# RuanJohn/Mava

Hardware: AMD Instinct MI355X
Metric: env-steps/sec (whole node), ff_mappo RWARE tiny-4ag (higher is better)
Workload: dtype f32 via 2 x f16 split operands on the MFMA (3 products, f32 accumulate); 1 GPU; ff_mappo RWARE tiny-4ag-shaped synthetic obs, 4096 envs/GPU (update_batch_size=1 x num_envs=4096), rollout_length=128, ppo_epochs=4, num_minibatches=2, agents=4, obs=70/264, actions=5, one step = one PPO update = 524288 env-steps per GPU; parallelism=dp1

## Files before the change

### include/mava_hip.h

```cpp
#ifndef MAVA_HIP_H
#define MAVA_HIP_H

#include <stddef.h>
#include <stdint.h>

#ifdef __cplusplus
extern "C" {
#endif

typedef struct ihipStream_t* mava_stream_t;

const char* mava_last_error(void);
int mava_abi_version(void);

typedef struct mava_ctx mava_ctx;
enum {
  MAVA_CTX_MATMUL_MODE = 0,
  MAVA_CTX_CRITIC_AGGREGATION = 1,
  MAVA_CTX_GAE_VARIANT = 2,
  MAVA_CTX_POLICY_VARIANT = 3,
  MAVA_CTX_H2_LAUNCHES = 4,
  MAVA_CTX_TRAIN_VARIANT = 5,
  MAVA_CTX_W8_LAUNCHES = 6,
  MAVA_CTX_W1_SPLIT_FRESH = 7,
// ... 4 lines not shown
  MAVA_CTX_W8_AHEAD_LAUNCHES = 12
};
int mava_ctx_create(mava_ctx** out);
int mava_ctx_destroy(mava_ctx* ctx);
int mava_ctx_set(mava_ctx* ctx, int key, long value);
int mava_ctx_get(const mava_ctx* ctx, int key, long* value);

int mava_gae_f32(const mava_ctx* ctx, const float* reward, const float* value, const uint8_t* done,
                 const float* last_val, const uint8_t* last_done, int T, int N, float gamma,
                 float lambda, float* adv, float* tgt, mava_stream_t s);

int mava_permutation_i32(long n, uint64_t seed, uint64_t counter, int32_t* out, mava_stream_t s);
int mava_permutation_batched_i32(long n, uint64_t seed, uint64_t counter, int n_perm, int32_t* out, long out_stride,
                                 mava_stream_t s);

int mava_clip_adam(float* p, const float* g, float* m, float* v, int32_t* count,
                   const int* seg_off, const float* seg_lr, int n_seg, float grad_scale,
                   float max_norm, int decay, int steps_per_update, int num_updates, float b1,
                   float b2, float eps, const float* loss_sums, float vf_coef, float ent_coef,
                   float* metrics_out, mava_stream_t s);

size_t mava_ppo_finish_workspace_bytes(int Pa, int Pc);
int mava_ppo_finish_f32(mava_ctx* ctx, const float* slab_a, long stride_a, const float* slab_c, long stride_c, int n_slab,
                        int Pa, int Pc, float* g, float* p, float* m, float* v, int32_t* count, float lr_a, float lr_c,
                        float grad_scale, float max_norm, int decay, int steps_per_update, int num_updates, float b1,
                        float b2, float eps, float vf_coef, float ent_coef, float* metrics_out, int critic_din,
                        void* workspace, size_t workspace_bytes, mava_stream_t s);

int mava_slab_reduce_f32(const float* slab, int n_slab, long slab_stride, int n, int accumulate,
                         float* out, mava_stream_t s);

int mava_slab_reduce2_f32(const float* slab, int n_slab, long slab_stride, int n_main,
                          float* out_main, int n_tail, float* out_tail, int accumulate,
                          mava_stream_t s);

int mava_mlp_param_count(int din, int n_out);

int mava_mlp_forward_f32(const mava_ctx* ctx, const float* params, int din, int n_out, const float* x, int x_share,
                         int rows, float* out, mava_stream_t s);

int mava_policy_step_f32(const mava_ctx* ctx, const float* actor_params, int actor_din, int n_actions,
                         const float* agents_view, const uint8_t* action_mask,
                         const float* critic_params, int critic_din, const float* critic_input,
                         int critic_share, int critic_rows, int value_broadcast, int rows,
                         uint64_t seed, uint32_t step, const uint32_t* step_base, uint32_t row_offset, int greedy,
                         const int32_t* forced_action, int32_t* action, float* log_prob,
                         float* value, float* logits, mava_stream_t s);


int mava_adv_stats_blocks(void);

int mava_adv_stats_f64(const float* advantages, const int32_t* idx, long idx_base, int Rb, int A,
                       double* partials, mava_stream_t s);
int mava_adv_stats_batched_f64(const float* advantages, const int32_t* idx, long idx_stride, int Rb, int A,
                               int n_batch, double* partials, mava_stream_t s);

int mava_ppo_actor_grad_f32(mava_ctx* ctx, const float* params, int din, int n_actions, const float* agents_view,
                            const uint8_t* action_mask, const int32_t* action, const float* old_log_prob,
                            const float* advantages, const double* adv_stats, const int32_t* idx, long idx_base, int Rb,
                            int A, float clip_eps, float ent_coef, float* slab, long slab_stride, int n_slab,
                            const uint16_t* input16, const uint32_t* input16_valid, int input16_ld, mava_stream_t s);

int mava_policy_step_continuous_f32(const mava_ctx* ctx, const float* actor_params, int actor_din, int action_dim, float min_scale,
                                    const float* agents_view, const float* critic_params, int critic_din,
                                    const float* critic_input, int critic_share, int critic_rows,
                                    int value_broadcast, int rows, uint64_t seed, uint32_t step,
                                    const uint32_t* step_base, uint32_t row_offset, int greedy,
                                    const float* forced_action, float* action, float* log_prob, float* value,
                                    float* mean, mava_stream_t s);
int mava_ppo_actor_grad_continuous_f32(const float* params, int din, int action_dim, float min_scale, const float* agents_view,
                                       const float* action, const float* old_log_prob, const float* advantages,
                                       const double* adv_stats, const int32_t* idx, long idx_base, int Rb, int A,
                                       float clip_eps, float ent_coef, uint64_t seed, uint32_t ent_step,
                                       uint32_t row_offset, float* slab, long slab_stride, int n_slab,
                                       mava_stream_t s);

int mava_ppo_critic_grad_f32(mava_ctx* ctx, const float* params, int din, const float* critic_input, int x_share,
                             const float* old_value, const float* targets, const int32_t* idx,
                             long idx_base, int Rb, int A, float clip_eps, float vf_coef,
                             float* slab, long slab_stride, int n_slab, const uint16_t* input16,
                             const uint32_t* input16_valid, int input16_ld, mava_stream_t s);


int mava_synth_rware_step(int E, int A, int O, int n_actions, int gs_tiles, int state_dim, int time_limit,
                          uint64_t seed, uint32_t t, const uint32_t* t_base, uint32_t env_offset, int is_reset,
                          int32_t* step_count, float* run_return, int32_t* run_length,
                          float* ep_return, int32_t* ep_length, float* agents_view,
                          float* global_state, uint8_t* action_mask, int32_t* obs_step_count,
                          float* reward, uint8_t* done, float* info_return, int32_t* info_length,
                          uint8_t* info_terminal, const int32_t* action, int reward_mode, mava_stream_t s);

int mava_lbf_step(int E, int A, int F, int G, int fov, int max_agent_level, int force_coop, int individual_rewards,
                  int time_limit, uint64_t seed, uint32_t t, const uint32_t* t_base, uint32_t env_offset, int is_reset,
                  int32_t* agent_pos, int32_t* agent_level, int32_t* food_pos, int32_t* food_level, uint8_t* food_alive,
                  float* total_food_level, int32_t* step_count, float* run_return, int32_t* run_length, float* ep_return,
                  int32_t* ep_length, float* agents_view, float* global_state, uint8_t* action_mask,
                  int32_t* obs_step_count, float* reward, uint8_t* done, float* info_return, int32_t* info_length,
                  uint8_t* info_terminal, const int32_t* action, float* real_view, uint8_t* real_mask, uint8_t* terminated,
                  mava_stream_t s);

int mava_rware_step(int E, int A, int S, int R, int H, int W, int sensor_range, int time_limit, int collision_terminates,
                    const uint32_t* highway_rows, const int32_t* shelf_home, uint64_t seed, uint32_t t,
                    const uint32_t* t_base, uint32_t env_offset, int is_reset, int32_t* agent_pos, int32_t* agent_dir,
                    int32_t* agent_carry, int32_t* shelf_pos, int32_t* request_queue, int32_t* step_count,
                    float* run_return, int32_t* run_length, float* ep_return, int32_t* ep_length, float* agents_view,
                    float* global_state, uint8_t* action_mask, int32_t* obs_step_count, float* reward, uint8_t* done,
                    float* info_return, int32_t* info_length, uint8_t* info_terminal, const int32_t* action,
                    float* real_view, uint8_t* real_mask, uint8_t* terminated, mava_stream_t s);

int mava_connector_step(int E, int A, int G, int time_limit, uint64_t seed, uint32_t t, const uint32_t* t_base,
                        uint32_t env_offset, int is_reset, int32_t* head, int32_t* target, uint8_t* connected,
                        uint8_t* grid, int32_t* step_count, float* run_return, int32_t* run_length, float* ep_return,
                        int32_t* ep_length, float* agents_view, float* global_state, uint8_t* action_mask,
                        int32_t* obs_step_count, float* reward, uint8_t* done, float* info_return, int32_t* info_length,
                        uint8_t* info_terminal, const int32_t* action, float* real_view, uint8_t* real_mask,
                        uint8_t* terminated, mava_stream_t s);

int mava_cleaner_step(int E, int A, int R, int C, int time_limit, uint64_t seed, uint32_t t, const uint32_t* t_base,
                      uint32_t env_offset, int is_reset, int32_t* pos, uint8_t* grid, int32_t* step_count,
                      float* run_return, int32_t* run_length, float* ep_return, int32_t* ep_length, float* agents_view,
                      float* global_state, uint8_t* action_mask, int32_t* obs_step_count, float* reward, uint8_t* done,
                      float* info_return, int32_t* info_length, uint8_t* info_terminal, uint8_t* info_won,
                      const int32_t* action, float* real_view, uint8_t* real_mask, uint8_t* terminated, mava_stream_t s);

int mava_smax_step(int E, int A, int Ne, uint64_t ally_types, uint64_t enemy_types, int time_limit, int see_enemy_actions,
                   int walls_cause_death, uint64_t seed, uint32_t t, const uint32_t* t_base, uint32_t env_offset,
                   int is_reset, float* pos, float* health, int32_t* cd, int32_t* last_action, int32_t* step_count,
                   float* run_return, int32_t* run_length, float* ep_return, int32_t* ep_length, float* agents_view,
                   float* global_state, uint8_t* action_mask, int32_t* obs_step_count, float* reward, uint8_t* done,
                   float* info_return, int32_t* info_length, uint8_t* info_terminal, uint8_t* info_won,
                   const int32_t* action, float* real_view, uint8_t* real_mask, uint8_t* terminated, mava_stream_t s);

int mava_spread_step(int E, int A, int add_agent_id, int time_limit, uint64_t seed, uint32_t t, const uint32_t* t_base,
                     uint32_t env_offset, int is_reset, float* agent_pos, float* landmark_pos, int32_t* step_count,
                     float* run_return, int32_t* run_length, float* ep_return, int32_t* ep_length, float* agents_view,
                     float* global_state, uint8_t* action_mask, int32_t* obs_step_count, float* reward, uint8_t* done,
                     float* info_return, int32_t* info_length, uint8_t* info_terminal, const float* action,
                     float* real_view, uint8_t* real_mask, uint8_t* terminated, float* real_state, mava_stream_t s);

int mava_rollout_ff_f32(const float* actor_params, int n_actions, const float* critic_params, int critic_shared,
                        int E, int A, int O, int T, int time_limit, uint64_t policy_seed, uint64_t env_seed,
                        uint32_t t0, uint32_t row_offset, uint32_t env_offset, int reward_mode,
                        int32_t* step_count, float* run_return, int32_t* run_length, float* ep_return,
                        int32_t* ep_length, float* agents_view, float* global_state, uint8_t* action_mask,
                        int32_t* obs_step_count, int32_t* action, float* value, float* reward, float* log_prob,
                        uint8_t* done, float* last_val, float* info_return, int32_t* info_length,
                        uint8_t* info_terminal, float* adv, float* tgt, float gamma, float gae_lambda,
                        float* last_reward, uint8_t* last_done, int32_t* step_counter, uint16_t* state16,
                        uint32_t* state16_valid, uint16_t* view16, uint32_t* view16_valid, mava_stream_t s);
int mava_rollout_carry(int T, int E, int A, int obs_dim, long gs_dim, int n_actions, float* agents_view,
                       float* global_state, uint8_t* action_mask, int32_t* step_count, mava_stream_t s);


int mava_rec_dense_f32(const mava_ctx* ctx, const float* x, int x_rowmajor, const int32_t* idx, int Rm, int E, int A,
                       int x_share, int x_ld, int accumulate, const float* w, int ldw, const float* bias,
                       const float* gate, float* y, int y_ld, int K, int N, int rows, int relu, mava_stream_t s);

int mava_rec_xty_f32(const mava_ctx* ctx, const float* x, int x_rowmajor, const int32_t* idx, int Rm, int E, int A,
                     int x_share, int x_ld, const float* y, int y_ld, const float* y_tail, int y_split, int y_tail_ld, int K, int N,
                     int rows, int want_bias, float out_scale, float* slab, long slab_stride, int n_slab, mava_stream_t s);
int mava_rec_gather_t32_f32(const float* x, const int32_t* idx, int Rm, int E, int A, int x_share, int x_ld, int K,
                            int rows, int k_pad, float* out, mava_stream_t s);

int mava_gru_scan_fwd_f32(const mava_ctx* ctx, int T, int Rm, int E, int A, const int32_t* idx, const uint8_t* done,
                          const float* h0, int h0_t32, const float* wh, const float* bhn,
                          const float* gi, float* hs, float* hprev, float* saved, mava_stream_t s);

int mava_gru_scan_bwd_f32(const mava_ctx* ctx, int T, int Rm, int E, int A, const int32_t* idx, const uint8_t* done,
                          const float* wh, const float* saved, const float* hprev, const float* dh_out,
                          float* dgi, float* dgh, int dgh_n_only, mava_stream_t s);

int mava_seq_actor_loss_f32(int T, int Rm, int E, int A, int n_actions, const int32_t* idx,
                            const float* logits, const uint8_t* mask, const int32_t* action,
                            const float* old_log_prob, const float* advantages, const double* adv_stats,
                            int n_stats, float clip_eps, float ent_coef, float grad_scale, float* dlogits,
                            float* loss_partials, int n_blocks, mava_stream_t s);
int mava_seq_actor_loss_continuous_f32(int T, int Rm, int E, int A, int action_dim, float min_scale, const int32_t* idx,
                                       const float* mean, const float* log_std, const float* log_std_rows,
                                       const float* action, const float* old_log_prob, const float* advantages,
                                       const double* adv_stats, int n_stats, float clip_eps, float ent_coef, uint64_t seed,
                                       uint32_t ent_step, uint32_t row_offset, float grad_scale, float* dmean,
                                       float* dlog_std_rows, float* loss_partials, float* dscale_partials, int n_blocks,
                                       mava_stream_t s);
int mava_seq_sample_continuous_f32(int rows, int action_dim, float min_scale, const float* mean, const float* log_std,
                                   const float* log_std_rows, uint64_t seed,
                                   uint32_t step, uint32_t row_offset, int greedy, float* action, float* log_prob,
                                   mava_stream_t s);
int mava_seq_critic_loss_f32(int T, int Rm, int E, int A, int agents_per_row, const int32_t* idx, const float* values,
                             const float* old_value, const float* targets, float clip_eps, float vf_coef,
                             float grad_scale, float* dvalues, float* loss_partials, int n_blocks, mava_stream_t s);

int mava_rec_out_f32(int T, int Rm, int E, int A, int n_out, int agents_per_row, const int32_t* idx, const float* hs,
                     const float* params_post_head, const uint8_t* mask, const int32_t* action, const float* f0,
                     const float* f1, const double* adv_stats, int n_stats, float clip_eps, float coef, float grad_scale,
                     int is_actor, float* dh, float* slab, long slab_stride, int n_slab, mava_stream_t s);

int mava_seq_sample_f32(int rows, int n_actions, const float* logits, const uint8_t* mask, uint64_t seed,
                        uint32_t step, uint32_t row_offset, int greedy, int32_t* action, float* log_prob,
                        mava_stream_t s);

int mava_rec_step_f32(const float* actor_params, int actor_din, int n_actions, const float* agents_view,
                      const uint8_t* action_mask, const uint8_t* done_a, const float* h_actor_in,
                      float* h_actor_out, int rows_a, uint64_t seed, uint32_t step, uint32_t row_offset,
                      int greedy, int32_t* action, float* log_prob, const float* critic_params, int critic_din,
                      const float* critic_input, int critic_share, const uint8_t* done_c, int done_c_stride,
                      const float* h_critic_in, float* h_critic_out, int rows_c, int value_broadcast,
                      float* value, mava_stream_t s);
int mava_rec_step_continuous_f32(const float* actor_params, int actor_din, int action_dim, float min_scale, const float* agents_view,
                                 const uint8_t* done_a, const float* h_actor_in, float* h_actor_out, int rows_a,
                                 uint64_t seed, uint32_t step, uint32_t row_offset, int greedy, float* action,
                                 float* log_prob, const float* critic_params, int critic_din,
                                 const float* critic_input, int critic_share, const uint8_t* done_c, int done_c_stride,
                                 const float* h_critic_in, float* h_critic_out, int rows_c, int value_broadcast,
                                 float* value, mava_stream_t s);

long mava_rec_step_pack_bytes(int din);
int mava_rec_step_pack_f32(const float* params, int din, void* pack, mava_stream_t s);
int mava_rec_step_packed_f32(const void* pack_a, const void* pack_c, const float* actor_params, int actor_din,
                             int n_actions, float min_scale, const float* agents_view, const uint8_t* action_mask, const uint8_t* done_a,
                             const float* h_actor_in, float* h_actor_out, int rows_a, uint64_t seed, uint32_t step,
                             uint32_t row_offset, int greedy, int32_t* action, float* action_f, float* log_prob,
                             const float* critic_params, int critic_din, const float* critic_input, int critic_share,
                             const uint8_t* done_c, int done_c_stride, const float* h_critic_in, float* h_critic_out,
                             int rows_c, int value_broadcast, float* value, mava_stream_t s);

int mava_rec_q_step_f32(const float* params, int din, int n_actions, const float* agents_view, const uint8_t* action_mask,
                        const uint8_t* done, const float* h_in, float* h_out, int rows, float eps, uint64_t seed, uint32_t step,
                        uint32_t row_offset, int32_t* action, float* q_out, mava_stream_t s);
int mava_replay_add_f32(int E, int A, int O, int n_actions, int capacity, int slot, const float* obs, const uint8_t* action_mask,
                        const int32_t* action, const float* reward, const uint8_t* terminal, const uint8_t* term_or_trunc,
                        const float* next_obs, const uint8_t* next_mask, float* b_obs, uint8_t* b_mask, int32_t* b_action,
                        float* b_reward, uint8_t* b_terminal, uint8_t* b_term_or_trunc, float* b_next_obs,
// ... 126 lines not shown
```

### mava_amd/_lib.py

```python
from __future__ import annotations

import ctypes as C
import os
from typing import Optional

import torch

_HERE = os.path.dirname(os.path.abspath(__file__))
LIB_PATH = os.environ.get("MAVA_LIB_PATH") or os.path.join(_HERE, "libmavahip.so")

_lib: Optional[C.CDLL] = None


class MavaHipError(RuntimeError):
    pass


vp = C.c_void_p
i32 = C.c_int
u32 = C.c_uint32
u64 = C.c_uint64
f32 = C.c_float
lng = C.c_long

_SIGNATURES = {
    "mava_abi_version": [],
    "mava_ctx_create": [vp],
    "mava_ctx_destroy": [vp],
    "mava_ctx_set": [vp, i32, lng],
    "mava_ctx_get": [vp, i32, vp],
    "mava_gae_f32": [vp, vp, vp, vp, vp, vp, i32, i32, f32, f32, vp, vp, vp],
    "mava_permutation_i32": [lng, u64, u64, vp, vp],
    "mava_permutation_batched_i32": [lng, u64, u64, i32, vp, lng, vp],
    "mava_clip_adam": [vp, vp, vp, vp, vp, C.POINTER(i32), C.POINTER(f32), i32, f32, f32, i32, i32, i32,
                       f32, f32, f32, vp, f32, f32, vp, vp],
    "mava_slab_reduce_f32": [vp, i32, lng, i32, i32, vp, vp],
    "mava_ppo_finish_workspace_bytes": [i32, i32],
    "mava_ppo_finish_f32": [vp, vp, lng, vp, lng, i32, i32, i32, vp, vp, vp, vp, vp, f32, f32, f32, f32, i32, i32, i32, f32, f32, f32,
                            f32, f32, vp, i32, vp, C.c_size_t, vp],
    "mava_slab_reduce2_f32": [vp, i32, lng, i32, vp, i32, vp, i32, vp],
    "mava_mlp_param_count": [i32, i32],
    "mava_mlp_forward_f32": [vp, vp, i32, i32, vp, i32, i32, vp, vp],
    "mava_policy_step_f32": [vp, vp, i32, i32, vp, vp, vp, i32, vp, i32, i32, i32, i32, u64, u32, vp, u32, i32,
                             vp, vp, vp, vp, vp, vp],
    "mava_policy_step_continuous_f32": [vp, vp, i32, i32, f32, vp, vp, i32, vp, i32, i32, i32, i32, u64, u32, vp, u32, i32, vp, vp, vp, vp, vp, vp],
    "mava_ppo_actor_grad_continuous_f32": [vp, i32, i32, f32, vp, vp, vp, vp, vp, vp, lng, i32, i32, f32, f32, u64, u32, u32, vp, lng, i32, vp],
    "mava_seq_actor_loss_continuous_f32": [i32, i32, i32, i32, i32, f32, vp, vp, vp, vp, vp, vp, vp, vp, i32, f32, f32, u64, u32, u32, f32, vp, vp, vp, vp, i32, vp],
    "mava_seq_sample_continuous_f32": [i32, i32, f32, vp, vp, vp, u64, u32, u32, i32, vp, vp, vp],
    "mava_adv_stats_blocks": [],
    "mava_adv_stats_f64": [vp, vp, lng, i32, i32, vp, vp],
    "mava_adv_stats_batched_f64": [vp, vp, lng, i32, i32, i32, vp, vp],
    "mava_ppo_actor_grad_f32": [vp, vp, i32, i32, vp, vp, vp, vp, vp, vp, vp, lng, i32, i32, f32, f32, vp, lng, i32,
                                vp, vp, i32, vp],
    "mava_ppo_critic_grad_f32": [vp, vp, i32, vp, i32, vp, vp, vp, lng, i32, i32, f32, f32, vp, lng, i32, vp, vp, i32, vp],
    "mava_synth_rware_step": [i32, i32, i32, i32, i32, i32, i32, u64, u32, vp, u32, i32] + [vp] * 14 + [vp, i32, vp],
    "mava_lbf_step": [i32] * 9 + [u64, u32, vp, u32, i32] + [vp] * 24 + [vp],
    "mava_rware_step": [i32] * 9 + [vp, vp, u64, u32, vp, u32, i32] + [vp] * 23 + [vp],
    "mava_connector_step": [i32] * 4 + [u64, u32, vp, u32, i32] + [vp] * 22 + [vp],
    "mava_cleaner_step": [i32] * 5 + [u64, u32, vp, u32, i32] + [vp] * 21 + [vp],
    "mava_smax_step": [i32] * 3 + [u64, u64] + [i32] * 3 + [u64, u32, vp, u32, i32] + [vp] * 23 + [vp],
    "mava_spread_step": [i32] * 4 + [u64, u32, vp, u32, i32] + [vp] * 21 + [vp],
    "mava_rec_q_step_f32": [vp, i32, i32, vp, vp, vp, vp, vp, i32, f32, u64, u32, u32, vp, vp, vp],
    "mava_replay_add_f32": [i32] * 6 + [vp] * 16 + [vp],
    "mava_replay_sample_f32": [i32] * 5 + [u32, i32, i32, i32, u64, u32] + [vp] * 17 + [vp],
    "mava_q_td_loss_f32": [i32, i32, i32, i32] + [vp] * 7 + [f32, f32, vp, vp, i32, vp],
    "mava_target_update_f32": [lng, vp, vp, f32, i32, vp],
    "mava_qmix_state_t32_f32": [i32] * 6 + [vp] * 4 + [vp],
    "mava_qmix_td_f32": [i32] * 7 + [vp] * 15 + [f32, f32] + [vp] * 6 + [i32, vp],
    "mava_sac_replay_add_f32": [i32] * 7 + [vp] * 14 + [vp],
    "mava_sac_replay_sample_f32": [i32] * 5 + [u32, i32, i32, u64, u32] + [vp] * 15 + [vp],
    "mava_sac_sample_f32": [i32, i32, i32, f32, vp, vp, u64, u32, u32, vp, vp, vp, vp],
    "mava_sac_concat_f32": [i32] * 7 + [vp] * 4 + [i32, vp],
    "mava_sac_q_loss_f32": [i32] * 3 + [vp] * 8 + [f32, f32] + [vp] * 4 + [i32, vp],
    "mava_sac_actor_grad_f32": [i32] * 4 + [f32] + [vp] * 9 + [i32, i32, i32, f32, f32] + [vp] * 3 + [i32, vp],
    "mava_sac_alpha_loss_f32": [i32, i32, vp, vp, f32, vp, vp, vp],
    "mava_rollout_ff_f32": [vp, i32, vp, i32, i32, i32, i32, i32, i32, u64, u64, u32, u32, u32, i32] + [vp] * 18
                           + [vp, vp, f32, f32] + [vp] * 7 + [vp],
    "mava_rollout_carry": [i32, i32, i32, i32, lng, i32, vp, vp, vp, vp, vp],
    "mava_rec_dense_f32": [vp, vp, i32, vp, i32, i32, i32, i32, i32, i32, vp, i32, vp, vp, vp, i32, i32, i32, i32, i32, vp],
    "mava_rec_xty_f32": [vp, vp, i32, vp, i32, i32, i32, i32, i32, vp, i32, vp, i32, i32, i32, i32, i32, i32, f32, vp, lng, i32, vp],
    "mava_rec_gather_t32_f32": [vp, vp, i32, i32, i32, i32, i32, i32, i32, i32, vp, vp],
    "mava_gru_scan_fwd_f32": [vp, i32, i32, i32, i32, vp, vp, vp, i32, vp, vp, vp, vp, vp, vp, vp],
    "mava_t32_gru_mask_f32": [vp, vp, vp, i32, i32, i32, lng, vp, vp],
    "mava_t32_gru_gates_f32": [vp, vp, vp, vp, i32, lng, vp, vp, vp, vp, vp, i32, i32, vp],
    "mava_t32_gru_gates_bwd_f32": [vp, vp, vp, vp, vp, vp, vp, i32, i32, i32, lng, vp, vp, vp, vp],
    "mava_gru_scan_bwd_f32": [vp, i32, i32, i32, i32, vp, vp, vp, vp, vp, vp, vp, vp, i32, vp],
    "mava_seq_actor_loss_f32": [i32, i32, i32, i32, i32, vp, vp, vp, vp, vp, vp, vp, i32, f32, f32, f32, vp, vp, i32, vp],
    "mava_rec_step_continuous_f32": [vp, i32, i32, f32, vp, vp, vp, vp, i32, u64, u32, u32, i32, vp, vp, vp, i32, vp, i32, vp, i32, vp, vp, i32, i32, vp, vp],
    "mava_rec_step_f32": [vp, i32, i32, vp, vp, vp, vp, vp, i32, u64, u32, u32, i32, vp, vp, vp, i32, vp, i32, vp, i32, vp, vp,
                          i32, i32, vp, vp],
    "mava_seq_critic_loss_f32": [i32, i32, i32, i32, i32, vp, vp, vp, vp, f32, f32, f32, vp, vp, i32, vp],
    "mava_rec_out_f32": [i32, i32, i32, i32, i32, i32, vp, vp, vp, vp, vp, vp, vp, vp, i32, f32, f32, f32, i32, vp, vp, lng, i32, vp],
    "mava_rec_step_pack_bytes": [i32],
    "mava_t32_norm_act_f32": [vp, i32, lng, i32, vp, i32, vp, vp, vp, vp],
    "mava_t32_norm_act_bwd_f32": [vp, vp, i32, lng, i32, vp, vp, i32, vp, vp, vp],
    "mava_t32_colsum_f32": [vp, i32, lng, f32, vp, lng, i32, vp],
    "mava_t32_im2col_f32": [vp, i32, lng, i32, i32, i32, i32, i32, vp, vp],
    "mava_t32_col2im_f32": [vp, i32, lng, i32, i32, i32, i32, i32, vp, vp],
    "mava_t32_flatten_f32": [vp, lng, i32, i32, i32, vp, vp],
    "mava_comm_unique_id": [vp],
    "mava_comm_create": [vp, i32, i32, vp],
    "mava_allreduce_sum_f32": [vp, vp, C.c_size_t, vp],
    "mava_broadcast_f32": [vp, vp, C.c_size_t, i32, vp],
    "mava_comm_destroy": [vp],
    "mava_rec_step_pack_f32": [vp, i32, vp, vp],
    "mava_rec_step_packed_f32": [vp, vp, vp, i32, i32, f32, vp, vp, vp, vp, vp, i32, u64, u32, u32, i32, vp, vp, vp, vp, i32, vp, i32, vp, i32, vp, vp, i32, i32, vp, vp],
    "mava_seq_sample_f32": [i32, i32, vp, vp, u64, u32, u32, i32, vp, vp, vp],
    "mava_t32_convert_f32": [vp, i32, i32, i32, vp, vp],
    "mava_mat_attn_fwd_f32": [vp, vp, vp, lng, i32, i32, i32, i32, i32, vp, vp, i32, vp],
    "mava_mat_attn_bwd_f32": [vp, vp, vp, vp, lng, i32, i32, i32, i32, i32, vp, vp, vp, i32, vp],
    "mava_mat_ln_fwd_f32": [vp, vp, vp, vp, i32, lng, lng, vp, vp, vp, i32, vp],
    "mava_mat_ln_bwd_f32": [vp, vp, vp, vp, i32, lng, lng, f32, vp, vp, lng, i32, vp],
    "mava_mat_gelu_f32": [vp, lng, vp, vp],
    "mava_mat_gelu_bwd_f32": [vp, vp, lng, vp, vp],
    "mava_mat_shift_onehot_f32": [vp, vp, i32, i32, i32, i32, lng, i32, vp, vp],
    "mava_mat_sample_f32": [i32, i32, i32, i32, vp, vp, u64, u32, u32, i32, vp, vp, vp],
    "mava_mat_loss_f32": [i32, i32, i32, lng, vp, vp, vp, vp, vp, vp, vp, vp, vp, vp, i32, f32, f32, f32, f32, vp, vp, vp, i32, vp],
    "mava_transformer_param_count": [i32, i32, i32, i32],
    "mava_transformer_act_workspace_bytes": [i32, i32, i32, i32, i32],
    "mava_transformer_act_f32": [vp, vp, vp, i32, i32, i32, i32, i32, i32, i32, u64, u32, u32, i32, vp, vp, vp, vp, C.c_size_t, i32, vp],
    "mava_transformer_shift_action_f32": [vp, vp, i32, i32, i32, i32, lng, i32, vp, vp],
    "mava_transformer_sample_continuous_f32": [i32, i32, i32, i32, f32, vp, vp, u64, u32, u32, i32, vp, vp, vp],
    "mava_transformer_loss_continuous_f32": [i32, i32, i32, f32, lng, vp, vp, vp, vp, vp, vp, vp, vp, vp, vp, i32, f32, f32, f32, u64, u32,
                                             u32, f32, vp, vp, vp, vp, i32, vp],
    "mava_transformer_param_count_continuous": [i32, i32, i32, i32],
    "mava_transformer_act_continuous_f32": [vp, vp, i32, i32, i32, i32, i32, i32, i32, f32, u64, u32, u32, i32, vp, vp, vp, vp, C.c_size_t,
                                            i32, vp],
}
_RESTYPES = {"mava_last_error": C.c_char_p, "mava_rec_step_pack_bytes": C.c_long, "mava_ppo_finish_workspace_bytes": C.c_size_t,
             "mava_transformer_param_count": C.c_long, "mava_transformer_act_workspace_bytes": C.c_size_t,
             "mava_transformer_param_count_continuous": C.c_long}


def declared_symbols():
    return sorted(set(_SIGNATURES) | set(_RESTYPES))


def lib() -> C.CDLL:
    global _lib
    if _lib is None:
        if not os.path.exists(LIB_PATH):
            raise MavaHipError(
                f"{LIB_PATH} is missing: build it with `python -m mava_amd.build` "
                "(hipcc --offload-arch=gfx950). There is no CPU fallback."
            )
        _lib = C.CDLL(LIB_PATH)
        _lib.mava_last_error.restype = C.c_char_p
        _lib.mava_last_error.argtypes = []
        for name, args in _SIGNATURES.items():
            fn = getattr(_lib, name)
            fn.argtypes = args
            fn.restype = _RESTYPES.get(name, C.c_int)
    return _lib


class Ctx:

    MATMUL_MODE, CRITIC_AGGREGATION, GAE_VARIANT, POLICY_VARIANT, H2_LAUNCHES, TRAIN_VARIANT, W8_LAUNCHES, W1_SPLIT_FRESH = 0, 1, 2, 3, 4, 5, 6, 7
    EXACT_TILES = 8
    X16_LAUNCHES = 9
# ... 77 lines not shown
```

### mava_amd/csrc/ppo_train.hip

```cpp
#include "mlp_core.h"
#include "ppo_train_task.h"
#include "ctx.h"
#include "tanh_normal.h"

namespace {

constexpr int STATS_BLOCKS = 128;
constexpr int LDT = 33;


#ifdef MAVA_STAMPS
#define STAMP_DECL unsigned long long st_prev = __builtin_readcyclecounter(), st_acc[16] = {0, 0, 0, 0, 0, 0, 0, 0, 0, 0, 0, 0, 0, 0, 0, 0};
#define STAMP(i)                                                   \
  do {                                                             \
    const unsigned long long st_now = __builtin_readcyclecounter(); \
    st_acc[i] += st_now - st_prev;                                 \
    st_prev = st_now;                                              \
  } while (0)
#else
#define STAMP_DECL
#define STAMP(i)
#endif

struct TrainLdsLayout {
// ... 748 lines not shown
      l += __shfl_down(l, o, 64);
    }
    if (lane == 0) { red[2 * w] = v; red[2 * w + 1] = l; }
    __syncthreads();
    if (tid == 0) {
      slab[oB3] = ((red[0] + red[2]) + red[4]) + red[6];
      slab[P] = ((red[1] + red[3]) + red[5]) + red[7];
      slab[P + 1] = 0.0f;
    }
  }
}

int pick_xv(const float* x, int din) {
  const uintptr_t a = (uintptr_t)x;
  return (din % 4 == 0 && a % 16 == 0 && din >= 96) ? 4 : 1;
}

template <int NO, int KT1, bool ACTOR, int XV, bool CONT>
int launch_train(const TrainTask& tk, int n_slab, hipStream_t s) {
  const TrainLdsLayout L = make_layout<NO>(KT1);
  const size_t lb = (size_t)L.end * sizeof(float);
  MAVA_ARG_CHECK(lb <= 163840, 8,
                 "ppo_train: %zu bytes of LDS needed (n_out pad %d, input width %d) exceed the 160 KiB of a CU",
                 lb, NO, tk.din);
  static bool attr_set = false;
  if (!attr_set) {
    MAVA_HIP_CHECK(hipFuncSetAttribute((const void*)ppo_train_kernel<NO, KT1, ACTOR, XV, CONT>,
                                       hipFuncAttributeMaxDynamicSharedMemorySize, (int)lb));
    attr_set = true;
  }
  g_train_last_instance = train_instance_id(1, ACTOR, CONT, false, NO, KT1, XV);
  hipLaunchKernelGGL((ppo_train_kernel<NO, KT1, ACTOR, XV, CONT>), dim3(n_slab), dim3(256), lb, s, tk, L);
  MAVA_LAUNCH_CHECK();
  return MAVA_OK;
}

template <int NO, int KT1, bool ACTOR, bool CONT>
int launch_xv(const TrainTask& tk, int n_slab, hipStream_t s) {
  if (KT1 >= 4 && tk.xv == 4) return launch_train<NO, KT1, ACTOR, (KT1 >= 4 ? 4 : 1), CONT>(tk, n_slab, s);
  return launch_train<NO, KT1, ACTOR, 1, CONT>(tk, n_slab, s);
}

template <int NO, bool ACTOR, bool CONT = false>
int dispatch_kt(const TrainTask& tk, int n_slab, hipStream_t s) {
  const int kt = tk.din / 32 + 1;
#ifdef MAVA_FAST_BUILD
  if (kt == 3) return launch_xv<NO, 3, ACTOR, CONT>(tk, n_slab, s);
  if (kt == 9) return launch_xv<NO, 9, ACTOR, CONT>(tk, n_slab, s);
  mava_set_error("fast build: input width %d not instantiated", tk.din);
  return MAVA_EARG(9);
#else
  switch (kt) {
    case 1: return launch_xv<NO, 1, ACTOR, CONT>(tk, n_slab, s);
    case 2: return launch_xv<NO, 2, ACTOR, CONT>(tk, n_slab, s);
    case 3: return launch_xv<NO, 3, ACTOR, CONT>(tk, n_slab, s);
    case 4: return launch_xv<NO, 4, ACTOR, CONT>(tk, n_slab, s);
    case 5: case 6: return launch_xv<NO, 6, ACTOR, CONT>(tk, n_slab, s);
    case 7: case 8: case 9: return launch_xv<NO, 9, ACTOR, CONT>(tk, n_slab, s);
    default:
      mava_set_error("ppo_train: input width %d > 287 is not instantiated", tk.din);
      return MAVA_EARG(9);
  }
#endif
}

}

#ifdef MAVA_STAMPS
static unsigned long long* g_stamps = nullptr;
extern "C" int mava_debug_set_stamps(unsigned long long* p) {
  g_stamps = p;
  return MAVA_OK;
}
#else
static constexpr unsigned long long* g_stamps = nullptr;
#endif


extern "C" int mava_adv_stats_blocks(void) { return STATS_BLOCKS; }

int g_train_last_instance = 0;
extern "C" int mava_debug_train_last_instance(void) { return g_train_last_instance; }

extern "C" int mava_adv_stats_f64(const float* adv, const int32_t* idx, long idx_base, int Rb, int A,
                                  double* partials, hipStream_t s) {
  MAVA_ARG_CHECK(Rb >= 1 && A >= 1, 0, "mava_adv_stats_f64: Rb=%d A=%d", Rb, A);
  MAVA_ARG_CHECK(adv && partials, 1, "mava_adv_stats_f64: null pointer argument");
  hipLaunchKernelGGL(adv_stats_kernel, dim3(STATS_BLOCKS), dim3(256), 0, s, adv, idx, idx_base, Rb, A,
                     partials, 0L);
  MAVA_LAUNCH_CHECK();
  return MAVA_OK;
}

extern "C" int mava_adv_stats_batched_f64(const float* adv, const int32_t* idx, long idx_stride, int Rb, int A,
                                          int n_batch, double* partials, hipStream_t s) {
  MAVA_ARG_CHECK(Rb >= 1 && A >= 1 && n_batch >= 1 && n_batch <= 65535 && idx_stride >= 0, 0,
                 "mava_adv_stats_batched_f64: Rb=%d A=%d n_batch=%d idx_stride=%ld", Rb, A, n_batch, idx_stride);
  MAVA_ARG_CHECK(adv && idx && partials, 1, "mava_adv_stats_batched_f64: null pointer argument");
  hipLaunchKernelGGL(adv_stats_kernel, dim3(STATS_BLOCKS, n_batch), dim3(256), 0, s, adv, idx, 0L, Rb, A, partials,
                     idx_stride);
  MAVA_LAUNCH_CHECK();
  return MAVA_OK;
}

extern "C" int mava_ppo_actor_grad_f32(mava_ctx* ctx, const float* params, int din, int n_actions, const float* agents_view,
                                       const uint8_t* action_mask, const int32_t* action, const float* old_log_prob,
                                       const float* advantages, const double* adv_stats, const int32_t* idx, long idx_base,
                                       int Rb, int A, float clip_eps, float ent_coef, float* slab, long slab_stride,
                                       int n_slab, const uint16_t* input16, const uint32_t* input16_valid, int input16_ld,
                                       hipStream_t s) {
  MAVA_ARG_CHECK(din >= 1 && n_actions >= 1 && n_actions <= 32, 0,
                 "mava_ppo_actor_grad_f32: din=%d n_actions=%d unsupported", din, n_actions);
  MAVA_ARG_CHECK(Rb >= 1 && A >= 1 && n_slab >= 1 && n_slab <= 1024 && (long)Rb * A < (1L << 31), 1,
                 "mava_ppo_actor_grad_f32: Rb=%d A=%d n_slab=%d", Rb, A, n_slab);
  MAVA_ARG_CHECK(slab_stride >= mlp_param_count(din, n_actions) + 2, 2,
                 "mava_ppo_actor_grad_f32: slab_stride too small");
  MAVA_ARG_CHECK(params && agents_view && action && old_log_prob && advantages && adv_stats && slab, 3,
                 "mava_ppo_actor_grad_f32: null pointer argument");
  MAVA_ARG_CHECK((input16 == nullptr) == (input16_valid == nullptr) && input16_ld >= 0, 3,
                 "mava_ppo_actor_grad_f32: input16 and input16_valid go together, input16_ld=%d", input16_ld);
  TrainTask tk = {};
  tk.params = params; tk.x = agents_view; tk.din = din; tk.no = n_actions; tk.xshare = 1; tk.agg = 1;
  tk.xv = pick_xv(agents_view, din); tk.A = A; tk.idx = idx; tk.idx_base = idx_base; tk.Rb = Rb;
  tk.mask = action_mask; tk.action = action; tk.old_logp = old_log_prob; tk.adv = advantages;
  tk.stats = adv_stats; tk.clip_eps = clip_eps; tk.ent_coef = ent_coef; tk.slab = slab;
  tk.slab_stride = slab_stride;
  tk.stamps = g_stamps;
  tk.x16 = reinterpret_cast<const _Float16*>(input16); tk.x16_valid = input16_valid; tk.x16_ld = input16_ld;
  if (mava_ctx_matmul_mode(ctx) == 1) {
    const int rc = mava_train_h2_launch(ctx, tk, n_slab, true, s);
    if (rc <= 0) return rc;
  }
  if (n_actions <= 8) return dispatch_kt<8, true>(tk, n_slab, s);
  if (n_actions <= 16) return dispatch_kt<16, true>(tk, n_slab, s);
  return dispatch_kt<32, true>(tk, n_slab, s);
}

extern "C" int mava_ppo_actor_grad_continuous_f32(const float* params, int din, int action_dim, float min_scale,
                                                  const float* agents_view, const float* action,
                                                  const float* old_log_prob, const float* advantages,
                                                  const double* adv_stats, const int32_t* idx, long idx_base, int Rb,
                                                  int A, float clip_eps, float ent_coef, uint64_t seed,
                                                  uint32_t ent_step, uint32_t row_offset, float* slab,
                                                  long slab_stride, int n_slab, hipStream_t s) {
  MAVA_ARG_CHECK(din >= 1 && action_dim >= 1 && action_dim <= 16, 0,
                 "mava_ppo_actor_grad_continuous_f32: din=%d action_dim=%d unsupported (action_dim <= 16)", din,
                 action_dim);
  MAVA_ARG_CHECK(Rb >= 1 && A >= 1 && n_slab >= 1 && n_slab <= 1024 && (long)Rb * A < (1L << 31), 1,
                 "mava_ppo_actor_grad_continuous_f32: Rb=%d A=%d n_slab=%d", Rb, A, n_slab);
  MAVA_ARG_CHECK(slab_stride >= mlp_param_count(din, action_dim) + action_dim + 2, 2,
                 "mava_ppo_actor_grad_continuous_f32: slab_stride too small");
  MAVA_ARG_CHECK(params && agents_view && action && old_log_prob && advantages && adv_stats && slab, 3,
                 "mava_ppo_actor_grad_continuous_f32: null pointer argument");
  TrainTask tk = {};
  tk.params = params; tk.x = agents_view; tk.din = din; tk.no = action_dim; tk.xshare = 1; tk.agg = 1;
  tk.xv = pick_xv(agents_view, din); tk.A = A; tk.idx = idx; tk.idx_base = idx_base; tk.Rb = Rb;
  tk.action_f = action; tk.old_logp = old_log_prob; tk.adv = advantages;
  tk.stats = adv_stats; tk.clip_eps = clip_eps; tk.ent_coef = ent_coef; tk.slab = slab;
  tk.slab_stride = slab_stride;
  tk.seed_lo = (uint32_t)seed; tk.seed_hi = (uint32_t)(seed >> 32); tk.ent_step = ent_step; tk.row_offset = row_offset;
  tk.min_scale = min_scale;
  tk.stamps = g_stamps;
  if (action_dim <= 8) return dispatch_kt<8, true, true>(tk, n_slab, s);
  return dispatch_kt<16, true, true>(tk, n_slab, s);
}

extern "C" int mava_ppo_critic_grad_f32(mava_ctx* ctx, const float* params, int din, const float* critic_input, int x_share,
                                        const float* old_value, const float* targets, const int32_t* idx, long idx_base,
                                        int Rb, int A, float clip_eps, float vf_coef, float* slab, long slab_stride,
                                        int n_slab, const uint16_t* input16, const uint32_t* input16_valid, int input16_ld,
                                        hipStream_t s) {
  MAVA_ARG_CHECK(din >= 1 && x_share >= 1, 0, "mava_ppo_critic_grad_f32: din=%d x_share=%d", din, x_share);
  MAVA_ARG_CHECK(Rb >= 1 && A >= 1 && n_slab >= 1 && n_slab <= 1024 && (long)Rb * A < (1L << 31), 1,
                 "mava_ppo_critic_grad_f32: Rb=%d A=%d n_slab=%d", Rb, A, n_slab);
  MAVA_ARG_CHECK(slab_stride >= mlp_param_count(din, 1) + 2, 2,
                 "mava_ppo_critic_grad_f32: slab_stride too small");
  MAVA_ARG_CHECK(params && critic_input && old_value && targets && slab, 3,
                 "mava_ppo_critic_grad_f32: null pointer argument");
  MAVA_ARG_CHECK((input16 == nullptr) == (input16_valid == nullptr) && input16_ld >= 0, 3,
                 "mava_ppo_critic_grad_f32: input16 and input16_valid go together, input16_ld=%d", input16_ld);
  TrainTask tk = {};
  tk.params = params; tk.x = critic_input; tk.din = din; tk.no = 1; tk.xshare = x_share; tk.agg = 1;
  if (mava_ctx_critic_aggregation(ctx) && A > 1 && A <= 8 && x_share == A) {
    tk.agg = A;
    tk.xshare = 1;
  }
  tk.xv = pick_xv(critic_input, din); tk.A = A; tk.idx = idx; tk.idx_base = idx_base; tk.Rb = Rb;
  tk.old_value = old_value; tk.targets = targets; tk.clip_eps = clip_eps; tk.vf_coef = vf_coef;
  tk.slab = slab; tk.slab_stride = slab_stride;
  tk.stamps = g_stamps;
  tk.x16 = reinterpret_cast<const _Float16*>(input16); tk.x16_valid = input16_valid; tk.x16_ld = input16_ld;
  int rc = 1;
  if (mava_ctx_matmul_mode(ctx) == 1) rc = mava_train_h2_launch(ctx, tk, n_slab, false, s);
  if (ctx != nullptr) ctx->w1_fresh[1] = 0;
  if (rc <= 0) return rc;
  return dispatch_kt<1, false>(tk, n_slab, s);
}
```

### mava_amd/csrc/ppo_train_h2.hip

```cpp
#include "h2_core.h"
#include "ppo_train_task.h"
#include "ctx.h"

#include <type_traits>

#ifndef MAVA_GW_DEPTH
#define MAVA_GW_DEPTH 0
#endif
#define GW_DEPTH MAVA_GW_DEPTH
#ifndef MAVA_GW_DEPTH_WIDE
#define MAVA_GW_DEPTH_WIDE 0
#endif
#ifndef MAVA_P1_EARLY_HALVES
#define MAVA_P1_EARLY_HALVES 2
#endif
#ifndef MAVA_P1_EARLY_RING
#define MAVA_P1_EARLY_RING 3
#endif

namespace {

using namespace h2;

constexpr int STATS_BLOCKS = 128;
// ... 1004 lines not shown
#pragma unroll
    for (int q = 0; q < 16; ++q) {
      const int o = (q & 3) + 8 * (q >> 2) + 4 * h;
      if (o < no) slab[oW3 + (32 * w + r) * no + o] = gW3[q] * invR;
    }
    float v = ab3;
#pragma unroll
    for (int m = NO; m < 64; m <<= 1) v += __shfl_xor(v, m, 64);
    if (lane < NO) red[w * NO + lane] = v;
    for (int o = 32; o > 0; o >>= 1) {
      loss_a += __shfl_down(loss_a, o, 64);
      loss_b += __shfl_down(loss_b, o, 64);
    }
    if (lane == 0) { red[4 * NO + 2 * w] = loss_a; red[4 * NO + 2 * w + 1] = loss_b; }
    __syncthreads();
    if (tid < no) slab[oB3 + tid] = (((red[tid] + red[NO + tid]) + red[2 * NO + tid]) + red[3 * NO + tid]) * invR;
    if (tid == 0) {
      slab[Pn] = ((red[4 * NO] + red[4 * NO + 2]) + red[4 * NO + 4]) + red[4 * NO + 6];
      slab[Pn + 1] = ((red[4 * NO + 1] + red[4 * NO + 3]) + red[4 * NO + 5]) + red[4 * NO + 7];
    }
  } else {
#pragma unroll
    for (int q = 0; q < 16; ++q) {
      float v = aW3r[q];
#pragma unroll
      for (int m = 1; m < 32; m <<= 1) v += __shfl_xor(v, m, 64);
      if (r == 0) slab[oW3 + 32 * w + (q & 3) + 8 * (q >> 2) + 4 * h] = v * invR;
    }
    float v = ab3, l = loss_a;
    for (int o = 32; o > 0; o >>= 1) {
      v += __shfl_down(v, o, 64);
      l += __shfl_down(l, o, 64);
    }
    if (lane == 0) { red[2 * w] = v; red[2 * w + 1] = l; }
    __syncthreads();
    if (tid == 0) {
      slab[oB3] = (((red[0] + red[2]) + red[4]) + red[6]) * invR;
      slab[Pn] = ((red[1] + red[3]) + red[5]) + red[7];
      slab[Pn + 1] = 0.0f;
    }
  }
}

template <int NO, int S1, bool ACTOR, bool WIDE, int XV>
__global__ __launch_bounds__(WIDE ? 512 : 256, WIDE ? 2 : 1) void ppo_train_h2_kernel(TrainTask tk, H2Layout L,
                                                                                     const uint4* __restrict__ w1p) {
  extern __shared__ __attribute__((aligned(16))) u8 lds[];
  if constexpr (WIDE) {
    constexpr bool X16_CAPABLE = !ACTOR && XV == 4;
    bool x16 = false;
    if constexpr (X16_CAPABLE) {
      if (tk.x16_valid != nullptr) x16 = __builtin_amdgcn_readfirstlane((int)*tk.x16_valid) == 1;
    }
    if (X16_CAPABLE && x16) {
      if constexpr (X16_CAPABLE) {
        if (threadIdx.x < 256) {
          h2_body<NO, S1, ACTOR, WIDE, XV, 1, true>(tk, L, w1p, lds);
        } else {
          h2_body<NO, S1, ACTOR, WIDE, XV, 2, true>(tk, L, w1p, lds);
        }
      }
    } else if (threadIdx.x < 256) {
      h2_body<NO, S1, ACTOR, WIDE, XV, 1>(tk, L, w1p, lds);
    } else {
      h2_body<NO, S1, ACTOR, WIDE, XV, 2>(tk, L, w1p, lds);
    }
  } else {
    h2_body<NO, S1, ACTOR, WIDE, XV, 0>(tk, L, w1p, lds);
  }
}

int ctx_counters(mava_ctx* ctx, hipStream_t s) {
  if (ctx->exact_tiles == nullptr) {
    void* word = nullptr;
    MAVA_HIP_CHECK(hipMalloc(&word, 5 * sizeof(unsigned long long)));
    ctx->exact_tiles = static_cast<unsigned long long*>(word);
    MAVA_HIP_CHECK(hipMemsetAsync(word, 0, 5 * sizeof(unsigned long long), s));
  }
  return MAVA_OK;
}

template <int NO, int S1, bool ACTOR, bool WIDE, int XV>
int launch_h2(mava_ctx* ctx, const TrainTask& tk, int n_slab, hipStream_t s) {
  const H2Layout L = make_h2_layout<NO, S1, WIDE>(ACTOR);
  MAVA_ARG_CHECK(L.end <= 163840, 8, "ppo_train_h2: %d bytes of LDS exceed the 160 KiB of a CU", L.end);
  static bool attr_set = false;
  if (!attr_set) {
    MAVA_HIP_CHECK(hipFuncSetAttribute((const void*)ppo_train_h2_kernel<NO, S1, ACTOR, WIDE, XV>,
                                       hipFuncAttributeMaxDynamicSharedMemorySize, L.end));
    attr_set = true;
  }
  const uint4* w1p = nullptr;
  if (WIDE) {
    void*& slot = ctx->w1_split[ACTOR ? 0 : 1];
    if (slot == nullptr) MAVA_HIP_CHECK(hipMalloc(&slot, W1_SPLIT_BYTES));
    uint4* const buf = static_cast<uint4*>(slot);
    const int kind = ACTOR ? 0 : 1;
    int& fresh = ctx->w1_fresh[kind];
    const bool keyed = ctx->w1_key_params[kind] == tk.params && ctx->w1_key_din[kind] == tk.din && ctx->w1_key_steps[kind] == S1;
    if (!(fresh && keyed)) {
      hipLaunchKernelGGL((pack_w1_kernel<S1>), dim3(1), dim3(256), 0, s, tk.params, tk.din, buf, ACTOR ? 1.0f : W_SCALE_CRITIC);
      MAVA_LAUNCH_CHECK();
    }
    fresh = 0;
    w1p = buf;
    const int rc = ctx_counters(ctx, s);
    if (rc != MAVA_OK) return rc;
  }
  TrainTask tkl = tk;
  tkl.exact_tiles = WIDE ? ctx->exact_tiles : nullptr;
  const bool x16_ok = WIDE && !ACTOR && XV == 4 && tk.x16 != nullptr && tk.x16_valid != nullptr && tk.din % 8 == 0 &&
                      (uintptr_t)tk.x16 % 16 == 0 && tk.force_xlo == 0 && (tk.x16_ld == 0 || tk.x16_ld == tk.din);
  if (!x16_ok) { tkl.x16 = nullptr; tkl.x16_valid = nullptr; }
  tkl.x16_launches = x16_ok ? ctx->exact_tiles + 1 : nullptr;
  g_train_last_instance = train_instance_id(2, ACTOR, false, WIDE, NO, S1, XV);
  hipLaunchKernelGGL((ppo_train_h2_kernel<NO, S1, ACTOR, WIDE, XV>), dim3(n_slab), dim3(WIDE ? 512 : 256), L.end, s, tkl, L,
                     w1p);
  MAVA_LAUNCH_CHECK();
  return MAVA_OK;
}

template <int NO, int S1, bool ACTOR, bool WIDE>
int dispatch_xv(mava_ctx* ctx, const TrainTask& tk, int n_slab, hipStream_t s) {
  const uintptr_t a = (uintptr_t)tk.x;
  if constexpr (WIDE) {
    if (tk.din % 4 == 0 && a % 16 == 0) return launch_h2<NO, S1, ACTOR, WIDE, 4>(ctx, tk, n_slab, s);
  } else {
    if (tk.din % 2 == 0 && a % 8 == 0) return launch_h2<NO, S1, ACTOR, WIDE, 2>(ctx, tk, n_slab, s);
  }
  return launch_h2<NO, S1, ACTOR, WIDE, 1>(ctx, tk, n_slab, s);
}

template <int NO, bool ACTOR>
int dispatch_s1(mava_ctx* ctx, const TrainTask& tk, int n_slab, hipStream_t s) {
  const int s1 = (tk.din + 1 + 15) / 16;
  switch (s1) {
#ifndef MAVA_FAST_BUILD
    case 1: return dispatch_xv<NO, 1, ACTOR, false>(ctx, tk, n_slab, s);
    case 2: return dispatch_xv<NO, 2, ACTOR, false>(ctx, tk, n_slab, s);
    case 3: return dispatch_xv<NO, 3, ACTOR, false>(ctx, tk, n_slab, s);
    case 4: return dispatch_xv<NO, 4, ACTOR, false>(ctx, tk, n_slab, s);
    case 6: return dispatch_xv<NO, 6, ACTOR, false>(ctx, tk, n_slab, s);
    case 7: case 8: case 9: case 10: case 11: case 12: return dispatch_xv<NO, 12, ACTOR, true>(ctx, tk, n_slab, s);
#endif
    case 5: return dispatch_xv<NO, 5, ACTOR, false>(ctx, tk, n_slab, s);
    case 13: case 14: case 15: case 16: case 17: case 18: return dispatch_xv<NO, 18, ACTOR, true>(ctx, tk, n_slab, s);
    default: return 1;
  }
}

}

static int h2_dispatch(mava_ctx* ctx, const TrainTask& tk, int n_slab, bool actor, hipStream_t s) {
  if (actor) {
    if (tk.action_f != nullptr) return 1;
    if (tk.no <= 8) return dispatch_s1<8, true>(ctx, tk, n_slab, s);
#ifndef MAVA_FAST_BUILD
    if (tk.no <= 16) return dispatch_s1<16, true>(ctx, tk, n_slab, s);
    return dispatch_s1<32, true>(ctx, tk, n_slab, s);
#else
    return 1;
#endif
  }
  return dispatch_s1<1, false>(ctx, tk, n_slab, s);
}

int mava_train_h2_launch(mava_ctx* ctx, const TrainTask& tk_in, int n_slab, bool actor, hipStream_t s) {
  TrainTask tk = tk_in;
  tk.force_xlo = (ctx->train_variant & 2) != 0;
  tk.no_defer = (ctx->train_variant & 4) != 0;
  tk.no_ahead = (ctx->train_variant & 8) != 0;
  if ((ctx->train_variant & 1) == 0) {
    if (tk.x16 != nullptr && tk.x16_valid != nullptr) {
      const int rcc = ctx_counters(ctx, s);
      if (rcc != MAVA_OK) return rcc;
      tk.x16_launches = ctx->exact_tiles + 2;
      tk.defer_launches = ctx->exact_tiles + 3;
      tk.ahead_launches = ctx->exact_tiles + 4;
    }
    const int rc8 = mava_train_w8_launch(tk, n_slab, actor, s);
    if (rc8 <= 0) {
      if (rc8 == 0) { ++ctx->h2_launches; ++ctx->w8_launches; }
      return rc8;
    }
  }
  const int rc = h2_dispatch(ctx, tk, n_slab, actor, s);
  if (rc == 0) ++ctx->h2_launches;
  return rc;
}
```

### mava_amd/csrc/ppo_train_task.h

```cpp
#pragma once
#include <stdint.h>

#include "common.h"

struct TrainTask {
  const float* params;
  const float* x;
  int din, no, xshare, xv;
  int A;
  int agg;
  const int32_t* idx;
  long idx_base;
  int Rb;
  const uint8_t* mask;
  const int32_t* action;
  const float* action_f;
  uint32_t seed_lo, seed_hi, ent_step, row_offset;
  float min_scale;
  const float* old_logp;
  const float* adv;
  const double* stats;
  const float* old_value;
  const float* targets;
  float clip_eps, ent_coef, vf_coef;
  float* slab;
  long slab_stride;
  unsigned long long* stamps;
  int force_xlo;
  unsigned long long* exact_tiles;
  const _Float16* x16;
  const uint32_t* x16_valid;
  unsigned long long* x16_launches;
  int x16_ld;
  int no_defer;
  unsigned long long* defer_launches;
  int no_ahead;
  unsigned long long* ahead_launches;
};

struct mava_ctx;
int mava_train_w8_launch(const TrainTask& tk, int n_slab, bool actor, hipStream_t s);
int mava_train_h2_launch(mava_ctx* ctx, const TrainTask& tk, int n_slab, bool actor, hipStream_t s);

extern int g_train_last_instance;
constexpr int train_instance_id(int family, bool actor, bool cont, bool wide, int no, int k, int xv) {
  return family * 1000000 + ((actor ? 1 : 0) + (cont ? 2 : 0) + (wide ? 4 : 0)) * 100000 + no * 1000 + k * 10 + xv;
}
```

### mava_amd/csrc/ppo_train_w8.hip

```cpp
#include "h2_core.h"
#include "ppo_train_task.h"
#include "ctx.h"

namespace {

using namespace h2;
typedef float f32x4 __attribute__((ext_vector_type(4)));

constexpr int STATS_BLOCKS = 128;
#ifndef MAVA_W8_GWD
#define MAVA_W8_GWD 1
#endif
constexpr int GWD = MAVA_W8_GWD;
#ifndef MAVA_W8_DEFER
#define MAVA_W8_DEFER 1
#endif
constexpr int W8_DEFER = MAVA_W8_DEFER;
static_assert(W8_DEFER >= 0 && W8_DEFER <= 2, "MAVA_W8_DEFER is 0, 1 or 2");
#ifndef MAVA_W8_AHEAD_ROLES
#define MAVA_W8_AHEAD_ROLES 1
#endif
#ifndef MAVA_W8_AHEAD_POS
#define MAVA_W8_AHEAD_POS 0
#endif
// ... 744 lines not shown
    float x = ab3;
#pragma unroll
    for (int m = NO; m < 64; m <<= 1) x += __shfl_xor(x, m, 64);
    if (l < NO) red[v * NO + l] = x;
    for (int o = 32; o > 0; o >>= 1) {
      loss_a += __shfl_down(loss_a, o, 64);
      loss_b += __shfl_down(loss_b, o, 64);
    }
    if (l == 0) { red[8 * NO + 2 * v] = loss_a; red[8 * NO + 2 * v + 1] = loss_b; }
  }
  __syncthreads();
  constexpr int LW = LOSS_THREADS / 64;
  if (tid < no) {
    float x = 0.0f;
#pragma unroll
    for (int u = 0; u < LW; ++u) x += red[u * NO + tid];
    slab[oB3 + tid] = x * invR;
  }
  if (tid == 0) {
    float a = 0.0f, b = 0.0f;
#pragma unroll
    for (int u = 0; u < LW; ++u) { a += red[8 * NO + 2 * u]; b += red[8 * NO + 2 * u + 1]; }
    slab[Pn] = a;
    slab[Pn + 1] = b;
  }
}

constexpr int w8_w2r(int no, int s1, int xv) {
#ifdef MAVA_W8_W2R
  return MAVA_W8_W2R;
#else
  return (no == 8) ? ((s1 <= 2) ? 2 : ((s1 == 3 && xv == 2) ? 2 : 0)) : ((s1 <= 2) ? 2 : 0);
#endif
}
template <int NO, int S1, int XV, int W2R, bool ACTOR>
__global__ __launch_bounds__(512, 2) void ppo_train_w8_kernel(TrainTask tk, W8Layout L) {
  extern __shared__ __attribute__((aligned(16))) u8 lds[];
  constexpr bool X16_CAPABLE = XV == 2;
  if constexpr (NO == 8) {
    constexpr bool DEFER_CAPABLE = X16_CAPABLE && W8_DEFER != 0;
    bool defer = false;
    if constexpr (DEFER_CAPABLE) {
      if (tk.x16_valid != nullptr && tk.no_defer == 0) defer = __builtin_amdgcn_readfirstlane((int)*tk.x16_valid) == 1;
    }
    constexpr bool AHEAD_CAPABLE = DEFER_CAPABLE && ACTOR && W8_AHEAD_ROLES != 0;
    if (DEFER_CAPABLE && defer && AHEAD_CAPABLE && tk.no_ahead == 0) {
      if constexpr (AHEAD_CAPABLE) {
        if (threadIdx.x < 256) w8_body<NO, S1, XV, W2R, ACTOR, 1, false, W8_DEFER, (W8_AHEAD_ROLES & 2) != 0>(tk, L, lds);
        else w8_body<NO, S1, XV, W2R, ACTOR, 2, true, 2, (W8_AHEAD_ROLES & 1) != 0>(tk, L, lds);
      }
    } else if (DEFER_CAPABLE && defer) {
      if constexpr (DEFER_CAPABLE) {
        if (threadIdx.x < 256) w8_body<NO, S1, XV, W2R, ACTOR, 1, false, W8_DEFER>(tk, L, lds);
        else w8_body<NO, S1, XV, W2R, ACTOR, 2, true, 2>(tk, L, lds);
      }
    } else if (threadIdx.x < 256) {
      w8_body<NO, S1, XV, W2R, ACTOR, 1>(tk, L, lds);
    } else {
      bool x16 = false;
      if constexpr (X16_CAPABLE) {
        if (tk.x16_valid != nullptr) x16 = __builtin_amdgcn_readfirstlane((int)*tk.x16_valid) == 1;
      }
      if (X16_CAPABLE && x16) {
        if constexpr (X16_CAPABLE) w8_body<NO, S1, XV, W2R, ACTOR, 2, true>(tk, L, lds);
      } else {
        w8_body<NO, S1, XV, W2R, ACTOR, 2>(tk, L, lds);
      }
    }
  } else {
    bool x16 = false;
    if constexpr (X16_CAPABLE) {
      if (tk.x16_valid != nullptr) x16 = __builtin_amdgcn_readfirstlane((int)*tk.x16_valid) == 1;
    }
    if (X16_CAPABLE && x16) {
      if constexpr (X16_CAPABLE) w8_body<NO, S1, XV, W2R, ACTOR, 0, true>(tk, L, lds);
    } else {
      w8_body<NO, S1, XV, W2R, ACTOR, 0>(tk, L, lds);
    }
  }
}

template <int NO, int S1, int XV, bool ACTOR>
int launch_w8(const TrainTask& tk, int n_slab, hipStream_t s) {
  const W8Layout L = make_w8_layout();
  MAVA_ARG_CHECK(L.end <= 163840, 8, "ppo_train_w8: %d bytes of LDS exceed the 160 KiB of a CU", L.end);
  static bool attr_set = false;
  if (!attr_set) {
    MAVA_HIP_CHECK(hipFuncSetAttribute((const void*)ppo_train_w8_kernel<NO, S1, XV, w8_w2r(NO, S1, XV), ACTOR>, hipFuncAttributeMaxDynamicSharedMemorySize,
                                       L.end));
    attr_set = true;
  }
  TrainTask tkl = tk;
  const int ld16 = tk.x16_ld != 0 ? tk.x16_ld : tk.din;
  const bool x16_ok = XV == 2 && tk.x16 != nullptr && tk.x16_valid != nullptr && ld16 % 8 == 0 && ld16 >= tk.din &&
                      (uintptr_t)tk.x16 % 16 == 0 && tk.force_xlo == 0 && tk.xshare == 1 && tk.agg <= 1;
  tkl.x16_ld = ld16;
  if (!x16_ok) { tkl.x16 = nullptr; tkl.x16_valid = nullptr; tkl.x16_launches = nullptr; tkl.defer_launches = nullptr; tkl.ahead_launches = nullptr; }
  g_train_last_instance = train_instance_id(3, ACTOR, false, false, NO, S1, XV);
  hipLaunchKernelGGL((ppo_train_w8_kernel<NO, S1, XV, w8_w2r(NO, S1, XV), ACTOR>), dim3(n_slab), dim3(512), L.end, s, tkl, L);
  MAVA_LAUNCH_CHECK();
  return MAVA_OK;
}

template <int NO, int S1, bool ACTOR>
int dispatch_w8_xv(const TrainTask& tk, int n_slab, hipStream_t s) {
  if (tk.din % 2 == 0 && ((uintptr_t)tk.x) % 8 == 0) return launch_w8<NO, S1, 2, ACTOR>(tk, n_slab, s);
  if constexpr (S1 == 4) return 1;
  else return launch_w8<NO, S1, 1, ACTOR>(tk, n_slab, s);
}

template <int NO, bool ACTOR>
int dispatch_w8(const TrainTask& tk, int n_slab, hipStream_t s) {
  const int s1 = (tk.din + 1 + 31) / 32;
  switch (s1) {
#ifndef MAVA_FAST_BUILD
    case 1: return dispatch_w8_xv<NO, 1, ACTOR>(tk, n_slab, s);
    case 2: return dispatch_w8_xv<NO, 2, ACTOR>(tk, n_slab, s);
    case 4: return dispatch_w8_xv<NO, 4, ACTOR>(tk, n_slab, s);
#endif
    case 3: return dispatch_w8_xv<NO, 3, ACTOR>(tk, n_slab, s);
    default: return 1;
  }
}

}

int mava_train_w8_launch(const TrainTask& tk, int n_slab, bool actor, hipStream_t s) {
  if (tk.action_f != nullptr || tk.din + 1 > 128) return 1;
  if (!actor) {
    if (tk.agg > 1 || tk.no != 1) return 1;
    return dispatch_w8<8, false>(tk, n_slab, s);
  }
  if (tk.no <= 8) return dispatch_w8<8, true>(tk, n_slab, s);
#ifndef MAVA_FAST_BUILD
  if (tk.no <= 16) return dispatch_w8<16, true>(tk, n_slab, s);
#endif
  return 1;
}
```

### mava_amd/csrc/rollout_h2.hip

```cpp
#include "h2_core.h"

#ifdef MAVA_STAMPS
#define RSTAMP_DECL unsigned long long rs_prev = __builtin_readcyclecounter(), rs_acc[8] = {0, 0, 0, 0, 0, 0, 0, 0};
#define RSTAMP(i)                                                   \
  do {                                                              \
    __builtin_amdgcn_sched_barrier(0);                              \
    const unsigned long long rs_now = __builtin_readcyclecounter(); \
    rs_acc[i] += rs_now - rs_prev;                                  \
    rs_prev = rs_now;                                               \
    __builtin_amdgcn_sched_barrier(0);                              \
  } while (0)
static __device__ unsigned long long g_rollout_stamps[16];
#else
#define RSTAMP_DECL
#define RSTAMP(i)
#endif

namespace {
using namespace h2;
typedef _Float16 half2v __attribute__((ext_vector_type(2)));

constexpr uint32_t ENV_STREAM = 0x454E5653u;
constexpr uint32_t POLICY_STREAM = 0x504f4c49u;

struct RolloutArgs {
  const float* pa;
  const float* pc;
  int E, A, O, no, T, time_limit;
  uint32_t pseed_lo, pseed_hi, eseed_lo, eseed_hi;
  uint32_t t0;
  uint32_t row_offset;
  uint32_t env_offset;
  int reward_mode;
  int32_t* step_count;
  float* run_return; int32_t* run_length; float* ep_return; int32_t* ep_length;
  float* agents_view;
  float* global_state;
  uint8_t* action_mask;
  int32_t* obs_step_count;
  int32_t* action; float* value; float* reward; float* log_prob; uint8_t* done;
  float* last_val;
  float* info_return; int32_t* info_length; uint8_t* info_terminal;
  float* adv; float* tgt;
  float gamma, lam;
  float* last_reward; uint8_t* last_done; int32_t* step_counter;
  _Float16* state16; uint32_t* state16_valid;
  _Float16* view16; uint32_t* view16_valid;
  int v16_nc; uint32_t v16_nc_m;
};

#define MAVA_AS4 __attribute__((address_space(4)))
__device__ __forceinline__ const MAVA_AS4 RolloutArgs& args_here() {
  const MAVA_AS4 RolloutArgs* p = (const MAVA_AS4 RolloutArgs*)__builtin_amdgcn_kernarg_segment_ptr();
  asm volatile("" : "+s"(p));
  return *p;
}

__device__ __forceinline__ uint32_t div_small(uint32_t x, uint32_t m) { return __umul24(x, m) >> 16; }

struct RolloutLds {
  int xa, xa_row, xa_plane, xc, xc_row, xc_plane, h1, wl, ypa, ypc, act, mask, small, gum, xlf, end;
};
constexpr int W1_REG_STEPS = 12;

template <int NO, int S1A, int S1C, bool SHARED>
constexpr RolloutLds make_rollout_lds() {
  constexpr int KTA = (S1A + 1) / 2, KTC = (S1C + 1) / 2;
  RolloutLds L{};
  L.xa = 0;
  L.xa_row = 2 * 32 * KTA + 16;
  L.xa_plane = 32 * L.xa_row;
  L.xc = L.xa + 2 * 2 * L.xa_plane;
  L.xc_row = 2 * 32 * KTC + 16;
  L.xc_plane = ((S1C > W1_REG_STEPS) ? 16 : 32) * L.xc_row;
  L.h1 = L.xc + (SHARED ? 2 * L.xc_plane : 0);
  L.wl = L.h1 + (SHARED ? 3 : 4) * IMG_BYTES;
  L.ypa = L.wl + ((S1C > W1_REG_STEPS) ? (S1C - W1_REG_STEPS) * 4 * 64 * 32 : 0);
  L.ypc = L.ypa + 2 * 4 * 32 * (NO + 1) * 4;
  L.act = L.ypc + 2 * 4 * 32 * 4;
  L.mask = L.act + 64 * 4;
  L.small = L.mask + 64 * 32;
  L.gum = L.small + (128 + 32 + 128 + 4 + 128) * 4;
  L.gum = (L.gum + 15) & ~15;
  L.xlf = L.gum + 64 * NO * 4;
  L.end = L.xlf + 16;
  L.end = (L.end + 15) & ~15;
  return L;
}

template <int NO, int S1A, int S1C, bool SHARED, int ROLE>
__device__ __forceinline__ void rollout_body(const RolloutArgs& a, u8* lds) {
  constexpr bool ACT_ROLE = ROLE == 0;
  constexpr RolloutLds L = make_rollout_lds<NO, S1A, S1C, SHARED>();
  const int t512 = threadIdx.x;
  const int tid = t512 & 255, lane = tid & 63, w = tid >> 6, h = lane >> 5, r = lane & 31;
  const int A = a.A, O = a.O, no = a.no, W = A + O, E = a.E;
  const int EB = 64 / A;
  const int e0 = blockIdx.x * EB;
  const int din_a = W, din_c = SHARED ? A * O : W;
  constexpr int NTC = SHARED ? 1 : 2;
  float* const B2a = reinterpret_cast<float*>(lds + L.small);
  float* const B3a = B2a + 128;
  float* const B2c = B3a + 32;
  float* const B3c = B2c + 128;
  float* const W3c = B3c + 4;
  int* const ACT = reinterpret_cast<int*>(lds + L.act);
  u8* const MASK = lds + L.mask;
  float* const GUM = reinterpret_cast<float*>(lds + L.gum);
  unsigned* const XLF = reinterpret_cast<unsigned*>(lds + L.xlf);
  float* const YPA = reinterpret_cast<float*>(lds + L.ypa);
  float* const YPC = reinterpret_cast<float*>(lds + L.ypc);
  constexpr int xa_row = L.xa_row, xa_plane = L.xa_plane, xc_row = L.xc_row, xc_plane = L.xc_plane;

  for (int i = t512 * 16; i < L.end; i += 512 * 16) *reinterpret_cast<uint4*>(lds + i) = make_uint4(0, 0, 0, 0);
  __syncthreads();
  const int oW2a = mlp_off_w2(din_a), oW3a = mlp_off_w3(din_a), oW2c = mlp_off_w2(din_c), oW3c = mlp_off_w3(din_c);
  if (ACT_ROLE) {
    if (tid < 128) B2a[tid] = a.pa[mlp_off_b2(din_a) + tid];
    if (tid < no) B3a[tid] = a.pa[mlp_off_b3(din_a, no) + tid];
  } else {
    if (tid < 128) {
      B2c[tid] = a.pc[mlp_off_b2(din_c) + tid];
      W3c[tid] = a.pc[oW3c + tid];
    }
    if (tid == 0) B3c[0] = a.pc[mlp_off_b3(din_c, 1)];
  }
  constexpr int S1R = ACT_ROLE ? S1A : S1C;
  constexpr int S1REG = (S1R > W1_REG_STEPS) ? W1_REG_STEPS : S1R;
  constexpr int XC_ROWS = (S1C > W1_REG_STEPS) ? 16 : 32;
  uint4* const WL = reinterpret_cast<uint4*>(lds + L.wl) + 2 * (w * 64 + lane);
  const float* const PR = ACT_ROLE ? a.pa : a.pc;
  const int din_r = ACT_ROLE ? din_a : din_c, oW2r = ACT_ROLE ? oW2a : oW2c;
// ... 212 lines not shown
          return read_row_frag(lds + L.h1 + ((ACT_ROLE ? 0 : 2) + t) * IMG_BYTES, IMG_PLANE, rowB + 32 * s);
        };
        Frag bn[NT];
#pragma unroll
        for (int t = 0; t < NT; ++t) bn[t] = h_frag(0, t);
#pragma unroll
        for (int s = 0; s < 8; ++s) {
          Frag b[NT];
#pragma unroll
          for (int t = 0; t < NT; ++t) b[t] = bn[t];
          if (s + 1 < 8) {
#pragma unroll
            for (int t = 0; t < NT; ++t) bn[t] = h_frag(s + 1, t);
          }
#pragma unroll
          for (int t = 0; t < NT; ++t) z[t] = mfma3(W2r[s], b[t], z[t]);
          __builtin_amdgcn_sched_barrier(0);
        }
      }
      if (ACT_ROLE) {
#pragma unroll
        for (int t = 0; t < NT; ++t) {
          half4 ph[4], pl[4];
#pragma unroll
          for (int g = 0; g < 4; ++g)
#pragma unroll
            for (int e = 0; e < 4; ++e) {
              _Float16 x0, x1;
              split1(fmaxf(z[t][4 * g + e], 0.0f), x0, x1);
              ph[g][e] = x0;
              pl[g][e] = x1;
            }
          f32x16 y;
#pragma unroll
          for (int q = 0; q < 16; ++q) y[q] = 0.0f;
#pragma unroll
          for (int s = 0; s < 2; ++s) {
            Frag b;
            b.hi = __builtin_shufflevector(ph[2 * s], ph[2 * s + 1], 0, 1, 2, 3, 4, 5, 6, 7);
            b.lo = __builtin_shufflevector(pl[2 * s], pl[2 * s + 1], 0, 1, 2, 3, 4, 5, 6, 7);
            y = mfma3(W3h[s], b, y);
          }
#pragma unroll
          for (int q = 0; q < 16; ++q) {
            const int o = (q & 3) + 8 * (q >> 2) + 4 * h;
            if ((q & 3) + 8 * (q >> 2) < NO) {
              if (o < NO) YPA[((t * 4 + w) * 32 + r) * (NO + 1) + o] = y[q] * W3_UNSCALE;
            }
          }
        }
      } else {
#pragma unroll
        for (int t = 0; t < NT; ++t) {
          float4 w3g[4];
#pragma unroll
          for (int g = 0; g < 4; ++g) w3g[g] = *reinterpret_cast<const float4*>(W3c + 32 * w + 4 * h + 8 * g);
          float part = 0.0f;
#pragma unroll
          for (int q = 0; q < 16; ++q) {
            const float4 tv = w3g[q >> 2];
            const float w3 = (q & 3) == 0 ? tv.x : (q & 3) == 1 ? tv.y : (q & 3) == 2 ? tv.z : tv.w;
            part = fmaf(fmaxf(z[t][q], 0.0f), w3, part);
          }
          part += __shfl_xor(part, 32, 64);
          if (h == 0) YPC[(t * 4 + w) * 32 + r] = part;
        }
      }
    }
    RSTAMP(2);
    __syncthreads();
    RSTAMP(3);
  };
  auto value_of = [&](int crow) -> float {
    const float* yp = YPC + (crow >> 5) * 4 * 32 + (crow & 31);
    return (((yp[0] + yp[32]) + yp[64]) + yp[96]) + B3c[0];
  };

  const int rows_ok = min(64, (E - e0) * A), envs_ok = min(EB, E - e0);
  const int AO = A * O;
  const uint32_t no_m = 65536u / (uint32_t)no + 1u, nch_m = 65536u / nch + 1u;
  const int tid_w = tid, wo_q = (W >> 1) > 0 ? (W >> 1) : 1, gs_q = (AO >> 2) > 0 ? (AO >> 2) : 1;
  const int wo_dr = 256 / wo_q, gs_dr = 256 / gs_q;
  const uint32_t wo_m = 65536u / (uint32_t)wo_q + 1u, gs_m = 65536u / (uint32_t)gs_q + 1u;
  auto write_gs = [&](long slot, bool f32_too) {
    const auto& a = args_here();
    int tid = tid_w;
    asm volatile("" : "+v"(tid));
    if (SHARED && a.global_state != nullptr) {
      float* dst = a.global_state + (slot * E + e0) * (long)AO;
      if ((AO & 3) == 0) {
        const bool h16 = a.state16 != nullptr;
        uint4* const dst16 = h16 ? reinterpret_cast<uint4*>(a.state16 + (slot * E + e0) * (long)AO) : nullptr;
        const int Q = AO >> 2, d_r = gs_dr, d_f = 256 - d_r * Q;
        int le = (int)div_small((uint32_t)tid, gs_m), k = tid - le * Q;
        for (int j = tid; j < EB * Q; j += 256) {
          if (le < envs_ok) {
            if (f32_too) {
              const half4 v = *reinterpret_cast<const half4*>(lds + L.xc + le * xc_row + 8 * k);
              reinterpret_cast<float4*>(dst)[j] = make_float4((float)v[0], (float)v[1], (float)v[2], (float)v[3]);
            }
            if (h16 && (k & 1) == 0) dst16[j >> 1] = *reinterpret_cast<const uint4*>(lds + L.xc + le * xc_row + 8 * k);
          }
          le += d_r; k += d_f;
          if (k >= Q) { k -= Q; ++le; }
        }
      } else if (f32_too) {
        const int d_r = 256 / AO, d_f = 256 - d_r * AO;
        int le = tid / AO, k = tid - le * AO;
        for (int j = tid; j < EB * AO; j += 256) {
          if (le < envs_ok) dst[j] = (float)*reinterpret_cast<const _Float16*>(lds + L.xc + le * xc_row + 2 * k);
          le += d_r; k += d_f;
          if (k >= AO) { k -= AO; ++le; }
        }
      }
    }
  };
  auto write_view16 = [&](long slot) {
    const auto& a = args_here();
    if (a.view16 != nullptr) {
      int tid = tid_w;
      asm volatile("" : "+v"(tid));
      const int NC = a.v16_nc;
      uint4* const dst16 = reinterpret_cast<uint4*>(a.view16) + (slot * EA + (long)e0 * A) * NC;
      for (int j = tid; j < rows_ok * NC; j += 256) {
        const int row = (int)div_small((uint32_t)j, a.v16_nc_m), c = j - row * NC;
        dst16[j] = *reinterpret_cast<const uint4*>(lds + L.xa + (row >> 5) * 2 * xa_plane + (row & 31) * xa_row + 16 * c);
      }
    }
  };
  auto write_out = [&](long slot, bool part_gs) {
    const auto& a = args_here();
    int tid = tid_w;
    asm volatile("" : "+v"(tid));
    if (!part_gs) {
      float* dst = a.agents_view + (slot * EA + (long)e0 * A) * W;
      if ((W & 1) == 0) {
        const int W2 = W >> 1, d_r = wo_dr, d_f = 256 - d_r * W2;
        int row = (int)div_small((uint32_t)tid, wo_m), f = tid - row * W2;
        for (int j = tid; j < 64 * W2; j += 256) {
          if (row < rows_ok) {
            const u8* xa = lds + L.xa + (row >> 5) * 2 * xa_plane + (row & 31) * xa_row;
            const half2v v = *reinterpret_cast<const half2v*>(xa + 4 * f);
            reinterpret_cast<float2*>(dst)[j] = make_float2((float)v[0], (float)v[1]);
          }
          row += d_r; f += d_f;
          if (f >= W2) { f -= W2; ++row; }
        }
      } else {
        const int d_r = 256 / W, d_f = 256 - d_r * W;
        int row = tid / W, f = tid - row * W;
        for (int j = tid; j < 64 * W; j += 256) {
          if (row < rows_ok) {
            const u8* xa = lds + L.xa + (row >> 5) * 2 * xa_plane + (row & 31) * xa_row;
            dst[j] = (float)*reinterpret_cast<const _Float16*>(xa + 2 * f);
          }
          row += d_r; f += d_f;
          if (f >= W) { f -= W; ++row; }
        }
      }
    }
    if (!part_gs) write_view16(slot);
    if (part_gs) write_gs(slot, true);
    if (!part_gs) {
      uint8_t* dst = a.action_mask + (slot * EA + (long)e0 * A) * no;
      for (int j = tid; j < rows_ok * no; j += 256) {
        const int row = (int)div_small((uint32_t)j, no_m), o = j - row * no;
        dst[j] = MASK[row * 32 + o];
      }
    }
  };

  const int T_steps = a.T;
  const uint32_t t0 = a.t0;
  if (SHARED && ACT_ROLE && a.state16 != nullptr) write_gs(0L, false);
  if (!ACT_ROLE) write_view16(0L);
  for (int t = 0; t < T_steps; ++t) {
    const uint32_t step = t0 + (uint32_t)t;
    forward(true, true, step);
    x_lo = 0;
    asm volatile("" : "+s"(x_lo));
    const auto& a = args_here();
    if (ACT_ROLE) {
      constexpr int RPP = 256 / NO;
#pragma unroll
      for (int pass = 0; pass < 64 / RPP; ++pass) {
        const int row = pass * RPP + tid / NO, o = tid & (NO - 1);
        const float* yp = YPA + (((row >> 5) * 4) * 32 + (row & 31)) * (NO + 1) + o;
        const float y = (((yp[0] + yp[32 * (NO + 1)]) + yp[2 * 32 * (NO + 1)]) + yp[3 * 32 * (NO + 1)]) + B3a[o];
        const bool legal = (o < no) && (MASK[row * 32 + o] != 0);
        const float z = legal ? y : -FLT_MAX;
        auto fmax_op = [](float p, float q) { return fmaxf(p, q); };
        auto add_op = [](float p, float q) { return p + q; };
        const float mx = group_allreduce<NO>(z, fmax_op);
        const float se = group_allreduce<NO>(expf(z - mx), add_op);
        const float logp = (mx == -FLT_MAX) ? ((o < no) ? -logf((float)no) : -FLT_MAX) : z - (mx + logf(se));
        float sc = (o < no) ? (z + GUM[row * NO + o]) : -FLT_MAX;
        if (!(sc > -FLT_MAX)) sc = -FLT_MAX;
        int best = o;
#pragma unroll
        for (int m = 1; m < NO; m <<= 1) {
          const float so = __shfl_xor(sc, m, 64);
          const int bo = __shfl_xor(best, m, 64);
          const bool take = (so > sc) || (so == sc && bo < best);
          sc = take ? so : sc;
          best = take ? bo : best;
        }
        const float lp = group_allreduce<NO>((o == best) ? logp : 0.0f, add_op);
        const int e = e0 + (row >> lgA);
        if (o == 0) {
          ACT[row] = best;
          if (e < E) {
            const long k = (long)t * EA + (long)e0 * A + row;
            a.action[k] = best;
            a.log_prob[k] = lp;
          }
        }
      }
    } else {
      if (tid < 64 && (e0 + (tid >> lgA)) < E) {
        a.value[(long)t * EA + (long)e0 * A + tid] = value_of(SHARED ? (tid >> lgA) : tid);
      }
      if (t > 0) write_out((long)t, false);
    }
    if (ACT_ROLE && t > 0) write_out((long)t, true);
    RSTAMP(4);
    __syncthreads();
    RSTAMP(5);
    {
      const auto& a = args_here();
      const uint32_t tn = step + 1;
      const long slot = (long)(t + 1);
      const uint32_t n_view = (uint32_t)(64 * nch);
      for (uint32_t i = ACT_ROLE ? (uint32_t)tid : n_view; i < n_view; i += 256) {
        const uint32_t row = div_small(i, nch_m), c = i - row * nch;
        const uint32_t le = row >> lgA, ag = row - (le << lgA), e = e0 + le;
        if ((int)e >= E) continue;
        const uint32_t ent = (a.env_offset + e) * A + ag;
        const Philox4 rv = philox4x32_10(ent, tn, c, ENV_STREAM, a.eseed_lo, a.eseed_hi);
        const uint32_t wds[4] = {rv.x, rv.y, rv.z, rv.w};
        const uint32_t f0 = 2 + 16 * c;
        const int n = (int)min(16u, (uint32_t)O - f0);
        u8* xa = lds + L.xa + (row >> 5) * 2 * xa_plane + (row & 31) * xa_row;
        u8* xc = lds + L.xc + le * xc_row + 2 * (ag * O);
        const bool pk_a = (n == 16) && (((uint32_t)A + f0) & 1u) == 0;
        const bool pk_c = (n == 16) && ((ag * (uint32_t)O + f0) & 1u) == 0;
        uint32_t pr[8];
#pragma unroll
        for (int q = 0; q < 16; q += 2) {
          const uint32_t b0 = (((wds[q >> 2] >> (8 * (q & 3))) & 0xFFu) < 51u) ? 0x3C00u : 0u;
          const uint32_t b1 = (((wds[(q + 1) >> 2] >> (8 * ((q + 1) & 3))) & 0xFFu) < 51u) ? 0x3C00u : 0u;
          pr[q >> 1] = b0 | (b1 << 16);
        }
        if (pk_a) {
#pragma unroll
          for (int q = 0; q < 8; ++q) *reinterpret_cast<uint32_t*>(xa + 2 * (A + f0) + 4 * q) = pr[q];
        } else {
#pragma unroll
          for (int q = 0; q < 16; ++q) {
            if (q < n) *reinterpret_cast<uint16_t*>(xa + 2 * (A + f0 + q)) = (uint16_t)(pr[q >> 1] >> (16 * (q & 1)));
          }
        }
        if (SHARED) {
          if (pk_c) {
#pragma unroll
            for (int q = 0; q < 8; ++q) *reinterpret_cast<uint32_t*>(xc + 2 * f0 + 4 * q) = pr[q];
          } else {
#pragma unroll
            for (int q = 0; q < 16; ++q) {
              if (q < n) *reinterpret_cast<uint16_t*>(xc + 2 * (f0 + q)) = (uint16_t)(pr[q >> 1] >> (16 * (q & 1)));
            }
          }
        }
      }
      if (!ACT_ROLE && tid >= 64 && tid < 128) {
        const uint32_t row = (uint32_t)(tid - 64);
        const uint32_t le = row >> lgA, ag = row - (le << lgA), e = e0 + le;
        if ((int)e < E) {
          const uint32_t ent = (a.env_offset + e) * A + ag;
          u8* xa = lds + L.xa + (row >> 5) * 2 * xa_plane + (row & 31) * xa_row;
          u8* xc = lds + L.xc + le * xc_row + 2 * (ag * O);
          const Philox4 cm = philox4x32_10(ent, tn, 0xFFFFu, ENV_STREAM, a.eseed_lo, a.eseed_hi);
          const float c0 = (float)(cm.x % 10u), c1 = (float)(cm.y % 10u);
          *reinterpret_cast<_Float16*>(xa + 2 * A) = (_Float16)c0;
          *reinterpret_cast<_Float16*>(xa + 2 * (A + 1)) = (_Float16)c1;
          if (SHARED) {
            *reinterpret_cast<_Float16*>(xc) = (_Float16)c0;
            *reinterpret_cast<_Float16*>(xc + 2) = (_Float16)c1;
          }
          const bool m1 = !((cm.z & 0xFFu) < 51u);
          for (int o = 0; o < no; ++o) MASK[row * 32 + o] = (o == 1 && no > 1) ? (m1 ? 1 : 0) : 1;
        }
      }
      if (bk_on) {
        const uint32_t env_id = a.env_offset + (uint32_t)(e0 + bk_le);
        const Philox4 ev = philox4x32_10(env_id, tn, 0u, ENV_STREAM ^ 1u, a.eseed_lo, a.eseed_hi);
        float rew = (u01_open(ev.x) < 0.02f) ? 1.0f : 0.0f;
        if (a.reward_mode == 1) {
          int hits = 0;
          for (int a2 = 0; a2 < A; ++a2) {
            const Philox4 pc2 = philox4x32_10(env_id * A + a2, tn - 1u, 0xFFFFu, ENV_STREAM, a.eseed_lo, a.eseed_hi);
            hits += (ACT[bk_le * A + a2] == (int)((pc2.x % 10u) % (uint32_t)no)) ? 1 : 0;
          }
          rew = (float)hits / (float)A;
        }
        const int sc_new = sc_reg + 1;
        const bool term = (sc_new >= a.time_limit) || (u01_open(ev.y) < 0.002f);
        const int sc_obs = term ? 0 : sc_new;
        sc_reg = sc_obs;
        a.obs_step_count[slot * EA + bk_k] = sc_obs;
        a.reward[(long)t * EA + bk_k] = rew;
        a.done[(long)t * EA + bk_k] = term ? 1 : 0;
        if (bk_ag == 0) {
          const float new_ret = rr_reg + rew;
          const int new_len = rl_reg + 1;
          er_reg = term ? new_ret : er_reg;
          el_reg = term ? new_len : el_reg;
          rr_reg = term ? 0.0f : new_ret;
          rl_reg = term ? 0 : new_len;
          const long ie = (long)t * E + e0 + bk_le;
          a.info_return[ie] = er_reg;
          a.info_length[ie] = el_reg;
          a.info_terminal[ie] = term ? 1 : 0;
        }
      }
    }
    RSTAMP(6);
    __syncthreads();
    RSTAMP(7);
  }
#ifdef MAVA_STAMPS
  if (blockIdx.x == 0 && tid == 0)
    for (int i = 0; i < 8; ++i) g_rollout_stamps[(ACT_ROLE ? 0 : 8) + i] = rs_acc[i];
#endif
  write_out((long)T_steps, ACT_ROLE);
  forward(!ACT_ROLE, false, 0u);
  {
  const auto& a = args_here();
  float lv = 0.0f;
  if (bk_on) {
    lv = value_of(SHARED ? (tid >> lgA) : tid);
    a.last_val[bk_k] = lv;
    a.step_count[bk_k] = sc_reg;
    if (bk_ag == 0) {
      a.run_return[e0 + bk_le] = rr_reg; a.run_length[e0 + bk_le] = rl_reg;
      a.ep_return[e0 + bk_le] = er_reg; a.ep_length[e0 + bk_le] = el_reg;
    }
    if (a.last_reward != nullptr) {
      const long k = (long)(a.T - 1) * EA + bk_k;
      a.last_reward[bk_k] = a.reward[k];
      a.last_done[bk_k] = a.done[k];
    }
  }
  if (a.adv != nullptr) {
    const int T = a.T;
    const int TC = min(T, (L.ypa / (64 * 9)) & ~7);
    float* const RW = reinterpret_cast<float*>(lds);
    float* const VV = RW + TC * 64;
    u8* const DD = reinterpret_cast<u8*>(VV + TC * 64);
    const long col0 = (long)e0 * A;
    const float gl = a.gamma * a.lam;
    float g = 0.0f, nv = lv;
    for (int tb = T; tb > 0; tb -= TC) {
      const int t_lo = max(tb - TC, 0), n = (tb - t_lo) * 64;
      __syncthreads();
      for (int i0 = t512; i0 < n; i0 += 512 * 8) {
        float rw[8], vv[8];
        uint8_t dd[8];
#pragma unroll
        for (int i = 0; i < 8; ++i) {
          const int j = min(i0 + 512 * i, n - 1);
          const long k = (long)(t_lo + (j >> 6)) * EA + col0 + min(j & 63, rows_ok - 1);
          rw[i] = a.reward[k]; vv[i] = a.value[k]; dd[i] = a.done[k];
        }
#pragma unroll
        for (int i = 0; i < 8; ++i) {
          const int j = i0 + 512 * i;
          if (j < n) { RW[j] = rw[i]; VV[j] = vv[i]; DD[j] = dd[i]; }
        }
      }
      __syncthreads();
      if (bk_on) {
#pragma unroll 8
        for (int t = tb - 1; t >= t_lo; --t) {
          const int j = (t - t_lo) * 64 + tid;
          const float rw = RW[j], vv = VV[j];
          const float nd = DD[j] ? 0.0f : 1.0f;
          const float delta = rw + a.gamma * nv * nd - vv;
          g = delta + gl * nd * g;
          RW[j] = g;
          VV[j] = g + vv;
          nv = vv;
        }
      }
      __syncthreads();
      for (int j = t512; j < n; j += 512) {
        if ((j & 63) < rows_ok) {
          const long k = (long)(t_lo + (j >> 6)) * EA + col0 + (j & 63);
          a.adv[k] = RW[j];
          a.tgt[k] = VV[j];
        }
      }
    }
  }
  if (!ACT_ROLE && blockIdx.x == 0 && tid == 0 && a.step_counter != nullptr) *a.step_counter += a.T;
  }
}

template <int NO, int S1A, int S1C, bool SHARED>
__global__ __launch_bounds__(512, 2) void rollout_h2_kernel(RolloutArgs a) {
  extern __shared__ __attribute__((aligned(16))) u8 lds[];
  if (threadIdx.x < 256) {
    rollout_body<NO, S1A, S1C, SHARED, 0>(a, lds);
  } else {
    rollout_body<NO, S1A, S1C, SHARED, 1>(a, lds);
  }
}

int g_rollout_last_instance = 0;

template <int NO, int S1A, int S1C, bool SHARED>
int launch_rollout(const RolloutArgs& a, hipStream_t s) {
  g_rollout_last_instance = NO * 100000 + S1A * 1000 + S1C * 10 + (SHARED ? 1 : 0);
  constexpr RolloutLds L = make_rollout_lds<NO, S1A, S1C, SHARED>();
  MAVA_ARG_CHECK(L.end <= 163840, 8, "mava_rollout_ff_f32: %d bytes of LDS exceed the 160 KiB of a CU", L.end);
  const int lds_bytes = L.end > 83968 ? L.end : 83968;
  static bool attr_set = false;
  if (!attr_set) {
    MAVA_HIP_CHECK(hipFuncSetAttribute((const void*)rollout_h2_kernel<NO, S1A, S1C, SHARED>,
                                       hipFuncAttributeMaxDynamicSharedMemorySize, lds_bytes));
    attr_set = true;
  }
  const int EB = 64 / a.A;
  hipLaunchKernelGGL((rollout_h2_kernel<NO, S1A, S1C, SHARED>), dim3(mava_cdiv(a.E, EB)), dim3(512), lds_bytes, s, a);
  MAVA_LAUNCH_CHECK();
  return MAVA_OK;
}

}

#ifdef MAVA_STAMPS
extern "C" int mava_debug_get_rollout_stamps(unsigned long long* out16) {
  return -(int)hipMemcpyFromSymbol(out16, HIP_SYMBOL(g_rollout_stamps), 16 * sizeof(unsigned long long));
}
#endif

extern "C" int mava_debug_rollout_last_instance(void) { return g_rollout_last_instance; }

extern "C" int mava_rollout_ff_f32(const float* actor_params, int n_actions, const float* critic_params, int critic_shared,
                                   int E, int A, int O, int T, int time_limit, uint64_t policy_seed, uint64_t env_seed,
                                   uint32_t t0, uint32_t row_offset, uint32_t env_offset, int reward_mode,
                                   int32_t* step_count, float* run_return, int32_t* run_length, float* ep_return,
                                   int32_t* ep_length, float* agents_view, float* global_state, uint8_t* action_mask,
                                   int32_t* obs_step_count, int32_t* action, float* value, float* reward, float* log_prob,
                                   uint8_t* done, float* last_val, float* info_return, int32_t* info_length,
                                   uint8_t* info_terminal, float* adv, float* tgt, float gamma, float gae_lambda,
                                   float* last_reward, uint8_t* last_done, int32_t* step_counter, uint16_t* state16,
                                   uint32_t* state16_valid, uint16_t* view16, uint32_t* view16_valid, hipStream_t s) {
  MAVA_ARG_CHECK(E >= 1 && A >= 1 && O >= 2 && T >= 1 && n_actions >= 1 && time_limit >= 1, 0,
                 "mava_rollout_ff_f32: bad shape E=%d A=%d O=%d T=%d nA=%d", E, A, O, T, n_actions);
  MAVA_ARG_CHECK(actor_params && critic_params && step_count && run_return && run_length && ep_return && ep_length &&
                     agents_view && action_mask && obs_step_count && action && value && reward && log_prob && done &&
                     last_val && info_return && info_length && info_terminal && (!critic_shared || global_state),
                 1, "mava_rollout_ff_f32: null pointer argument");
  if (64 % A != 0 || n_actions > 8) return 1;
  if (critic_shared && A < 2) return 1;
  const int s1a = (A + O + 1 + 15) / 16, s1c = critic_shared ? (A * O + 1 + 15) / 16 : s1a;
  RolloutArgs a = {};
  a.pa = actor_params; a.pc = critic_params; a.E = E; a.A = A; a.O = O; a.no = n_actions; a.T = T; a.time_limit = time_limit;
  a.pseed_lo = (uint32_t)policy_seed; a.pseed_hi = (uint32_t)(policy_seed >> 32);
  a.eseed_lo = (uint32_t)env_seed; a.eseed_hi = (uint32_t)(env_seed >> 32);
  a.t0 = t0; a.row_offset = row_offset; a.env_offset = env_offset; a.reward_mode = reward_mode;
  a.step_count = step_count; a.run_return = run_return; a.run_length = run_length; a.ep_return = ep_return;
  a.ep_length = ep_length; a.agents_view = agents_view; a.global_state = critic_shared ? global_state : nullptr;
  a.action_mask = action_mask; a.obs_step_count = obs_step_count; a.action = action; a.value = value; a.reward = reward;
  a.log_prob = log_prob; a.done = done; a.last_val = last_val; a.info_return = info_return; a.info_length = info_length;
  a.info_terminal = info_terminal;
  MAVA_ARG_CHECK((adv == nullptr) == (tgt == nullptr), 1, "mava_rollout_ff_f32: adv and tgt go together");
  a.adv = adv; a.tgt = tgt; a.gamma = gamma; a.lam = gae_lambda;
  MAVA_ARG_CHECK((last_reward == nullptr) == (last_done == nullptr) && (last_reward != nullptr || step_counter == nullptr), 1,
                 "mava_rollout_ff_f32: last_reward, last_done (and step_counter) go together");
  a.last_reward = last_reward; a.last_done = last_done; a.step_counter = step_counter;
  MAVA_ARG_CHECK((state16 == nullptr) == (state16_valid == nullptr), 1, "mava_rollout_ff_f32: state16 and state16_valid go together");
  MAVA_ARG_CHECK(state16 == nullptr || (critic_shared && (A * O) % 8 == 0 && (uintptr_t)state16 % 16 == 0), 2,
                 "mava_rollout_ff_f32: state16 needs the shared critic, A*O %% 8 == 0 (A*O=%d) and 16-byte alignment", A * O);
  a.state16 = reinterpret_cast<_Float16*>(state16); a.state16_valid = state16_valid;
  MAVA_ARG_CHECK((view16 == nullptr) == (view16_valid == nullptr), 1, "mava_rollout_ff_f32: view16 and view16_valid go together");
  MAVA_ARG_CHECK(view16 == nullptr || (uintptr_t)view16 % 16 == 0, 2, "mava_rollout_ff_f32: view16 needs 16-byte alignment");
  a.view16 = reinterpret_cast<_Float16*>(view16); a.view16_valid = view16_valid;
  a.v16_nc = (A + O + 8) / 8; a.v16_nc_m = 65536u / (uint32_t)a.v16_nc + 1u;
  if (critic_shared) {
    if (s1a == 5 && s1c == 17 && A >= 4) return launch_rollout<8, 5, 17, true>(a, s);
#ifndef MAVA_FAST_BUILD
    if (s1a <= 2 && s1c <= 2) return launch_rollout<8, 2, 2, true>(a, s);
    if (s1a <= 2 && s1c <= 4) return launch_rollout<8, 2, 4, true>(a, s);
    if (s1a <= 5 && s1c <= 9) return launch_rollout<8, 5, 9, true>(a, s);
#endif
    return 1;
  }
  if (s1a == 5) return launch_rollout<8, 5, 5, false>(a, s);
#ifndef MAVA_FAST_BUILD
  if (s1a <= 2) return launch_rollout<8, 2, 2, false>(a, s);
#endif
  return 1;
}

namespace {
struct CarryArgs {
  uint8_t* base[4];
  long slot_bytes[4];
  int T;
};
template <typename V>
__device__ __forceinline__ void carry_copy(uint8_t* dst, const uint8_t* src, long bytes) {
  const long nv = bytes / (long)sizeof(V), stride = (long)gridDim.x * blockDim.x;
  const long i0 = (long)blockIdx.x * blockDim.x + threadIdx.x;
  for (long i = i0; i < nv; i += stride) reinterpret_cast<V*>(dst)[i] = reinterpret_cast<const V*>(src)[i];
  for (long i = nv * (long)sizeof(V) + i0; i < bytes; i += stride) dst[i] = src[i];
}
__global__ __launch_bounds__(256) void rollout_carry_kernel(CarryArgs c) {
  uint8_t* const dst = c.base[blockIdx.y];
  const long bytes = c.slot_bytes[blockIdx.y];
  if (dst == nullptr || bytes <= 0) return;
  const uint8_t* const src = dst + (long)c.T * bytes;
  const uintptr_t al = reinterpret_cast<uintptr_t>(dst) | reinterpret_cast<uintptr_t>(src);
  if ((al & 15) == 0) carry_copy<uint4>(dst, src, bytes);
  else if ((al & 3) == 0) carry_copy<uint32_t>(dst, src, bytes);
  else carry_copy<uint8_t>(dst, src, bytes);
}
}

extern "C" int mava_rollout_carry(int T, int E, int A, int obs_dim, long gs_dim, int n_actions, float* agents_view,
                                  float* global_state, uint8_t* action_mask, int32_t* step_count, hipStream_t s) {
  MAVA_ARG_CHECK(T >= 1 && E >= 1 && A >= 1 && obs_dim >= 1 && gs_dim >= 0 && n_actions >= 1, 0,
                 "mava_rollout_carry: bad shape T=%d E=%d A=%d obs_dim=%d gs_dim=%ld nA=%d", T, E, A, obs_dim, gs_dim, n_actions);
  MAVA_ARG_CHECK(agents_view && action_mask && step_count && (gs_dim == 0 || global_state), 1,
                 "mava_rollout_carry: null pointer argument");
  CarryArgs c = {};
  c.T = T;
  c.base[0] = reinterpret_cast<uint8_t*>(agents_view); c.slot_bytes[0] = (long)E * A * obs_dim * 4;
  c.base[1] = gs_dim ? reinterpret_cast<uint8_t*>(global_state) : nullptr; c.slot_bytes[1] = (long)E * gs_dim * 4;
  c.base[2] = action_mask; c.slot_bytes[2] = (long)E * A * n_actions;
  c.base[3] = reinterpret_cast<uint8_t*>(step_count); c.slot_bytes[3] = (long)E * A * 4;
  long most = 0;
  for (int i = 0; i < 4; ++i) most = c.slot_bytes[i] > most ? c.slot_bytes[i] : most;
  const long blocks = mava_cdiv(most, 256L * 16 * 4);
  hipLaunchKernelGGL(rollout_carry_kernel, dim3((unsigned)(blocks < 1 ? 1 : blocks > 2048 ? 2048 : blocks), 4), dim3(256), 0, s, c);
  MAVA_LAUNCH_CHECK();
  return MAVA_OK;
}
```

### mava_amd/learner.py

```python
from __future__ import annotations

import math
import contextlib
import os
from typing import Any, Dict, List, Optional, Tuple

import torch

from . import ops, parallel, ppo_learner
from .networks import FeedForwardActor, FeedForwardValueNet, MLPTorso
from .ppo_learner import PPOLearner
from .types import LearnerState, TimeStep


class FFLearner(PPOLearner):
    def __init__(self, env, config, centralised_critic: bool, device: Optional[torch.device] = None):
        super().__init__(env, config, centralised_critic, device,
                         ctx_kwargs={"critic_aggregation": os.environ.get("MAVA_CRITIC_AGGREGATION", "1") != "0"})
        s, env0, action_head = config.system, self.reps[0].env, self.action_head

        net = config.network
        from . import generic_networks as gn

        self.generic = (not gn.is_default_mlp(net.actor_network.pre_torso) or not gn.is_default_mlp(net.critic_network.pre_torso)
                        or (self.continuous and not action_head.independent_std))
        if self.generic:
            if (self.E * env0.num_agents) % 32 or ((self.T * self.E // self.M) * env0.num_agents) % 32:
                raise ValueError("the general network path needs num_envs * num_agents and the agent rows of a minibatch to be "
                                 "multiples of 32")
            obs_shape = getattr(env0, "obs_shape", None)
            state_shape = getattr(env0, "state_shape", None) if centralised_critic else obs_shape
            self.actor_network = gn.GenericActor(gn.torso_from_config(net.actor_network.pre_torso), action_head, self.Oa, obs_shape)
            self.critic_network = gn.GenericCritic(gn.torso_from_config(net.critic_network.pre_torso), centralised_critic, self.Oc,
                                                   state_shape)
        else:
            a_torso = MLPTorso(**{k: v for k, v in net.actor_network.pre_torso.items() if k != "_target_"})
            c_torso = MLPTorso(**{k: v for k, v in net.critic_network.pre_torso.items() if k != "_target_"})
            self.actor_network = FeedForwardActor(a_torso, action_head, self.Oa)
            self.critic_network = FeedForwardValueNet(c_torso, centralised_critic, self.Oc)
        self.Pa, self.Pc = self.actor_network.num_params, self.critic_network.num_params
        self._alloc_params([(self.actor_network, s.actor_lr), (self.critic_network, s.critic_lr)])

        d = self.device
        self.Rb = self.T * self.E // self.M
        self.n_slab = self._slab_count((self.Rb * self.A + 31) // 32)
        self.slab_a = torch.zeros((self.n_slab, self.Pa + 2), device=d)
        self.slab_c = torch.zeros((self.n_slab, self.Pc + 2), device=d)
        self.step_dev = torch.zeros(1, dtype=torch.int32, device=d)
        mode = os.environ.get("MAVA_GRAPH_ROLLOUT", "1")
        self.graph_rollout = (mode == "force" or (mode != "0" and self.world == 1)) and not self.generic
        self._graphs: Dict[int, Any] = {}
        self._graph_seen: set = set()
        self.ctx.set(self.ctx.TRAIN_VARIANT, int(os.environ.get("MAVA_TRAIN_VARIANT", "0")))
        for net_ in (self.actor_network, self.critic_network):
            net_.ctx = self.ctx
        self.fused_rollout = (self.matmul_mode == "f16x2" and not self.continuous and not self.generic
                              and os.environ.get("MAVA_FUSED_ROLLOUT", "1") != "0"
                              and bool(getattr(env0, "supports_fused_rollout", False))
                              and int(getattr(env0, "synth_state_dim", 0)) == 0
                              and (not centralised_critic or (env0.gs_tiles == 1 and env0.global_state_shared)))
        self.x16 = (self.fused_rollout and centralised_critic and self.Oc % 8 == 0 and os.environ.get("MAVA_X16", "1") != "0")
        for rep in self.reps:
            rep.state16 = torch.zeros((self.T + 1, self.E, 1, self.Oc), dtype=torch.float16, device=d) if self.x16 else None
            rep.state16_valid = torch.zeros((1,), dtype=torch.int32, device=d) if self.x16 else None
        self.view16 = (self.fused_rollout and not self.continuous and self.matmul_mode == "f16x2" and self.Oa + 1 <= 128
                       and os.environ.get("MAVA_X16", "1") != "0" and os.environ.get("MAVA_X16_ACTOR", "1") != "0")
        rp = 8 * ((self.Oa + 8) // 8)
        for rep in self.reps:
            rep.view16 = torch.zeros((self.T + 1, self.E, self.A, rp), dtype=torch.float16, device=d) if self.view16 else None
            rep.view16_valid = torch.zeros((1,), dtype=torch.int32, device=d) if self.view16 else None
        self.fused_tail = (self.world == 1 and not self.generic and os.environ.get("MAVA_FUSED_TAIL", "1") != "0")
        self._finish_ws = ops.ppo_finish_workspace(self.Pa, self.Pc, d) if self.fused_tail else None
        self._finish_ws_mr = (ops.ppo_finish_workspace(self.Pa, self.Pc, d)
                              if (not self.fused_tail and not self.generic and os.environ.get("MAVA_FUSED_TAIL", "1") != "0") else None)
        if self.fused_tail and self.U > 1:
            self.slab_a = torch.zeros((self.U * self.n_slab, self.Pa + 2), device=d)
            self.slab_c = torch.zeros((self.U * self.n_slab, self.Pc + 2), device=d)

    def _refuse(self, env, config) -> None:
        if (self.T * self.E) % self.M:
            raise ValueError("rollout_length * num_envs must be divisible by num_minibatches (ff_mappo.py:277-279)")

    def _timed(self, name: str, fn, *args, **kwargs):
        if self.timers is None:
            return fn(*args, **kwargs)
        a, b = torch.cuda.Event(enable_timing=True), torch.cuda.Event(enable_timing=True)
        a.record()
        out = fn(*args, **kwargs)
        b.record()
        self.timers.setdefault(name, []).append((a, b))
        return out

    def reset_envs(self) -> None:
        super().reset_envs()
        self.step_dev.zero_()

    def _timestep(self, slot: int) -> TimeStep:
        stack, obs = self._stack, self._observation(slot)
        done = stack(lambda r: r.last_done[:, 0]).bool()
        step_type = torch.where(done, 2, 1).to(torch.int8)
        reward = stack(lambda r: r.last_reward)
        n = max(self.n_upd - 1, 0)
        extras = {"episode_metrics": {
            "episode_return": stack(lambda r: r.info_return[n, -1]),
            "episode_length": stack(lambda r: r.info_length[n, -1]),
            "is_terminal_step": stack(lambda r: r.info_terminal[n, -1]).bool()}}
        return TimeStep(step_type, reward, 1.0 - stack(lambda r: r.last_done).float(), obs, extras)

    def learner_state(self) -> LearnerState:
        env_state = self._env_state()
        env_state["running_count_episode_return"] = self._stack(lambda r: r.state.run_return)
        env_state["running_count_episode_length"] = self._stack(lambda r: r.state.run_length)
        return LearnerState(self._params_tree(), self._opt_tree(), self._key(), env_state, self._timestep(0))

    def _adopted(self) -> None:
        self.ctx.set(self.ctx.W1_SPLIT_FRESH, 0)

    def _rollout(self, n: int) -> None:
        if self.fused_rollout and self._rollout_fused(n):
            self.t_global += self.T
            return
        if not self.graph_rollout or self.timers is not None:
            self._rollout_body()
            self._bootstrap_and_gae()
        else:
            key = self.seed
            graph = self._graphs.get(key)
            if graph is None and key in self._graph_seen:
                graph = torch.cuda.CUDAGraph()
                with torch.cuda.graph(graph, capture_error_mode="thread_local"):
                    self._rollout_body()
                    self._bootstrap_and_gae()
                self._graphs[key] = graph
            if graph is None:
                self._graph_seen.add(key)
                self._rollout_body()
                self._bootstrap_and_gae()
            else:
                graph.replay()
        for rep in self.reps:
            rep.info_return[n].copy_(rep.cur_return)
            rep.info_length[n].copy_(rep.cur_length)
            rep.info_terminal[n].copy_(rep.cur_terminal)
        self.t_global += self.T

    def _rollout_fused(self, n: int) -> bool:
        s = self.config.system
        pa, pc = self.p[: self.Pa], self.p[self.Pa :]
        EA = self.E * self.A
        main = torch.cuda.current_stream() if self.device.type == "cuda" else None
        side = self.U > 1 and self.timers is None and main is not None and os.environ.get("MAVA_ROLLOUT_STREAMS", "1") != "0"
        if side and not hasattr(self, "_roll_streams"):
            from .streams import overlapping_stream

            self._roll_streams = [overlapping_stream(self.device) for _ in range(self.U - 1)]
            if any(st is None for st in self._roll_streams):
                self._roll_streams = []
        side = side and len(self._roll_streams) == self.U - 1
        if side:
            for st in self._roll_streams:
                st.wait_stream(main)
        for u, rep in enumerate(self.reps):
            env = rep.env
            with (torch.cuda.stream(self._roll_streams[u - 1]) if (side and u > 0) else contextlib.nullcontext()):
              ok = self._timed(
                "rollout_fused", ops.rollout_ff, pa, pc, n_actions=self.nA, critic_shared=self.centralised, E=self.E,
                A=self.A, O=env.raw_obs_dim, T=self.T, time_limit=env.time_limit, policy_seed=self.seed,
                env_seed=env.seed, t0=self.t_global, row_offset=(self.rank * self.U + u) * EA, env_offset=env.env_offset,
                reward_mode=1 if env.reward_mode == "match" else 0, env_state=rep.state, agents_view=rep.agents_view,
                global_state=rep.global_state, action_mask=rep.action_mask, obs_step_count=rep.step_count,
                action=rep.action, value=rep.value, reward=rep.reward, log_prob=rep.log_prob, done=rep.done,
                last_val=rep.last_val, info_return=rep.info_return[n], info_length=rep.info_length[n],
                info_terminal=rep.info_terminal[n], adv=rep.adv, tgt=rep.tgt, gamma=float(s.gamma),
                gae_lambda=float(s.gae_lambda), last_reward=rep.last_reward, last_done=rep.last_done,
                step_counter=self.step_dev if u == 0 else None,
                state16=rep.state16, state16_valid=rep.state16_valid, view16=rep.view16, view16_valid=rep.view16_valid)
              if not ok:
                assert u == 0
                self.fused_rollout = self.x16 = self.view16 = False
                for r in self.reps:
                    r.state16 = r.state16_valid = r.view16 = r.view16_valid = None
                return False
        if side:
            for st in self._roll_streams:
                main.wait_stream(st)
        return True

    def _rollout_body(self) -> None:
        pa, pc = self.p[: self.Pa], self.p[self.Pa :]
        EA = self.E * self.A
        for t in range(self.T):
            step = t
            for u, rep in enumerate(self.reps):
                av = rep.agents_view[t].view(EA, self.Oa)
                if self.centralised:
                    cx = rep.global_state[t].view(-1, self.Oc)
                else:
                    cx = av
                shared = self.critic_share == self.A and self.A > 1
                common = dict(critic_share=1 if shared else self.critic_share, critic_rows=self.E if shared else EA,
                              value_broadcast=self.A if shared else 1, seed=self.seed, step=step,
                              step_base=self.step_dev, row_offset=(self.rank * self.U + u) * EA, ctx=self.ctx)
                if self.generic:
                    self._timed("policy_step", self._generic_act, u, rep, t, step)
                elif self.continuous:
                    self._timed("policy_step", ops.policy_step_continuous, pa, pc, av, cx, action_dim=self.nA, min_scale=self.min_scale,
                                out=(rep.action[t].view(EA, self.nA), rep.log_prob[t].view(EA), rep.value[t].view(EA)),
                                **common)
                else:
                    self._timed("policy_step", ops.policy_step, pa, pc, av, rep.action_mask[t].view(EA, self.nA), cx,
                                n_actions=self.nA,
                                out=(rep.action[t].view(EA), rep.log_prob[t].view(EA), rep.value[t].view(EA)), **common)
                last = t == self.T - 1
                self._timed("env_step", rep.env.step_into, rep.state, step + 1, rep.obs_slot(t + 1), rep.reward[t], rep.done[t],
                            rep.cur_return[t], rep.cur_length[t], rep.cur_terminal[t], t_base=self.step_dev,
                            action=rep.action[t] if self._env_reads_action else None)
                if last:
                    rep.last_reward.copy_(rep.reward[t])
                    rep.last_done.copy_(rep.done[t])
        self.step_dev.add_(self.T)

    def _bootstrap_and_gae(self) -> None:
        s = self.config.system
        pc = self.p[self.Pa :]
        EA = self.E * self.A
        for rep in self.reps:
            cx = rep.global_state[self.T].view(-1, self.Oc) if self.centralised else rep.agents_view[self.T].view(EA, self.Oa)
            if self.generic:
                v = self.critic_network.net.forward(pc, self._gws_roll[1], cx.view(1, self.E, -1, self.Oc), self.critic_share, None, EA,
                                                    self.E, self.A)[0]
                rep.last_val.view(EA).copy_(v)
            else:
                ops.mlp_forward(pc, self.Oc, 1, cx, rows=EA, x_share=self.critic_share, out=rep.last_val.view(EA, 1), ctx=self.ctx)
            self._timed("gae", ops.gae, rep.reward.view(self.T, EA), rep.value.view(self.T, EA), rep.done.view(self.T, EA),
                        rep.last_val.view(EA), float(s.gamma), float(s.gae_lambda),
                        out=(rep.adv.view(self.T, EA), rep.tgt.view(self.T, EA)), ctx=self.ctx)

    def _minibatch(self, n: int, k: int, mb: int, perm: Optional[torch.Tensor]) -> None:
        s = self.config.system
        T, E, A = self.T, self.E, self.A
        TEA = T * E * A
        pa, pc = self.p[: self.Pa], self.p[self.Pa :]
        idx = None if perm is None else perm[mb * self.Rb : (mb + 1) * self.Rb]
        base = mb * self.Rb
        if self.generic:
            return self._minibatch_generic(n, k, mb, idx if idx is not None else torch.arange(base, base + self.Rb, dtype=torch.int32,
                                                                                             device=self.device))
        ns = self.n_slab
        per_rep = self.fused_tail and self.U > 1
        for u, rep in enumerate(self.reps):
            slab_a = self.slab_a[u * ns : (u + 1) * ns] if per_rep else self.slab_a
            av = rep.agents_view[:T].view(TEA, self.Oa)
            if getattr(self, "_stats_batched", False) and perm is self._perm_bufs[k]:
                stats = self._stats_all[u, k * self.M + mb]
            else:
                stats = ops.adv_stats(rep.adv.view(TEA), idx, base, self.Rb, A, out=self.stats)
            if self.continuous:
                self._timed("actor_grad", ops.ppo_actor_grad_continuous, pa, av, rep.action.view(TEA, self.nA),
                            rep.log_prob.view(TEA), rep.adv.view(TEA), stats, idx, base, self.Rb, A, self.nA,
                            float(s.clip_eps), float(s.ent_coef), self.seed, self.ent_step,
                            (self.rank * self.U + u) * TEA, slab_a, min_scale=self.min_scale)
            else:
                self._timed("actor_grad", ops.ppo_actor_grad, pa, av, rep.action_mask[:T].view(TEA, self.nA),
                            rep.action.view(TEA), rep.log_prob.view(TEA), rep.adv.view(TEA), stats, idx, base,
                            self.Rb, A, self.nA, float(s.clip_eps), float(s.ent_coef), slab_a, ctx=self.ctx,
                            input16=rep.view16[:T].view(TEA, -1) if self.view16 else None,
                            input16_valid=rep.view16_valid if self.view16 else None)
            if not self.fused_tail:
                ops.slab_reduce2(self.slab_a, self.Pa, self.g[: self.Pa], 2, self.g[self.P : self.P + 2], accumulate=u > 0)
        w_actor = parallel.allreduce_sum_async(self.g[: self.Pa])
        for u, rep in enumerate(self.reps):
            av = rep.agents_view[:T].view(TEA, self.Oa)
            cx = rep.global_state[:T].view(-1, self.Oc) if self.centralised else av
            in16 = in16_valid = None
            if self.x16:
                in16, in16_valid = rep.state16[:T].view(-1, self.Oc), rep.state16_valid
            elif self.view16 and not self.centralised and self.critic_share == 1:
                in16, in16_valid = rep.view16[:T].view(TEA, -1), rep.view16_valid
            self._timed("critic_grad", ops.ppo_critic_grad, pc, cx, self.critic_share, rep.value.view(TEA), rep.tgt.view(TEA),
                        idx, base, self.Rb, A, float(s.clip_eps), float(s.vf_coef),
                        self.slab_c[u * ns : (u + 1) * ns] if per_rep else self.slab_c, ctx=self.ctx,
                        input16=in16, input16_valid=in16_valid)
            if not self.fused_tail:
                ops.slab_reduce2(self.slab_c, self.Pc, self.g[self.Pa : self.P], 1, self.g[self.P + 2 : self.P + 3], accumulate=u > 0)
        if self.fused_tail:
            self._ppo_finish("finish", n, k, mb, self.slab_a, self.slab_c, self._finish_ws)
            return
        w_rest = parallel.allreduce_sum_async(self.g[self.Pa :])
        for wk in (w_actor, w_rest):
            if wk is not None:
                wk.wait()
        if self._finish_ws_mr is not None:
            self._ppo_finish("clip_adam", n, k, mb, None, None, self._finish_ws_mr)
        else:
            self._timed("clip_adam", self._clip_adam, n, k, mb)

    def _ppo_finish(self, name: str, n: int, k: int, mb: int, slab_a, slab_c, workspace) -> None:
        self._timed(name, ops.ppo_finish, self.ctx, slab_a, slab_c, self.Pa, self.Pc, self.g, self.p, self.m, self.v, self.count,
                    self.seg_lr[0], self.seg_lr[1], critic_din=self.Oc, workspace=workspace, **self._adam_kwargs(n, k, mb))

    def _generic_setup(self) -> None:
        d = self.device
        EA, Rm = self.E * self.A, self.Rb * self.A
        a, c = self.actor_network.net, self.critic_network.net
        self._gws_roll = (a.workspace(EA, d, False), c.workspace(EA, d, False))
        self._gws = (a.workspace(Rm, d, True), c.workspace(Rm, d, True))
        self._g_scale = float(2 ** math.ceil(math.log2(Rm)))
        self._g_dscale = torch.zeros((self._gws[0].loss_partials.shape[0], max(self.nA, 1)), device=d)

    def _generic_act(self, u: int, rep, t: int, step: int) -> None:
        if not hasattr(self, "_gws_roll"):
            self._generic_setup()
        L, st = ops.lib(), ops.stream_ptr()
        pa, pc = self.p[: self.Pa], self.p[self.Pa :]
        E, A, EA = self.E, self.A, self.E * self.A
        an = self.actor_network
        outs = an.net.forward(pa, self._gws_roll[0], rep.agents_view[t : t + 1], 1, None, EA, E, A)
        seed, row_off = self.seed & (2**64 - 1), ((self.rank * self.U + u) * EA) & 0xFFFFFFFF
        gstep = (self.t_global + step) & 0xFFFFFFFF
        if self.continuous:
            ind = an.independent_std
            ops.check(L.mava_seq_sample_continuous_f32(EA, self.nA, self.min_scale, ops.ptr(outs[0]), ops.ptr(an.log_std(pa)) if ind else None,
                                                       None if ind else ops.ptr(outs[1]), seed, gstep, row_off, 0, ops.ptr(rep.action[t]),
                                                       ops.ptr(rep.log_prob[t]), st), "mava_seq_sample_continuous_f32")
        else:
            ops.check(L.mava_seq_sample_f32(EA, self.nA, ops.ptr(outs[0]), ops.ptr(rep.action_mask[t]), seed, gstep, row_off, 0,
                                            ops.ptr(rep.action[t]), ops.ptr(rep.log_prob[t]), st), "mava_seq_sample_f32")
        cx = rep.global_state[t : t + 1] if self.centralised else rep.agents_view[t : t + 1]
        v = self.critic_network.net.forward(pc, self._gws_roll[1], cx, self.critic_share, None, EA, E, A)[0]
        rep.value[t].view(EA).copy_(v)

    def _minibatch_generic(self, n: int, k: int, mb: int, idx: torch.Tensor) -> None:
        if not hasattr(self, "_gws"):
            self._generic_setup()
        s = self.config.system
        T, E, A = self.T, self.E, self.A
        TE, Rm = T * E, self.Rb * A
        L, st = ops.lib(), ops.stream_ptr()
        pa, pc = self.p[: self.Pa], self.p[self.Pa :]
        idx = idx.contiguous()
        wa, wc = self._gws
        an, cn, gs = self.actor_network, self.critic_network, self._g_scale
        nblk = wa.loss_partials.shape[0]
        for u, rep in enumerate(self.reps):
            acc = u > 0
            outs = an.net.forward(pa, wa, rep.agents_view[:T].view(1, TE, A, self.Oa), 1, idx, Rm, TE, A)
            ops.adv_stats(rep.adv.view(-1), idx, 0, self.Rb, A, out=self.stats)
            if self.continuous:
                ind = an.independent_std
                ops.check(L.mava_seq_actor_loss_continuous_f32(
                    1, Rm, TE, A, self.nA, self.min_scale, ops.ptr(idx), ops.ptr(outs[0]), ops.ptr(an.log_std(pa)) if ind else None,
                    None if ind else ops.ptr(outs[1]), ops.ptr(rep.action), ops.ptr(rep.log_prob), ops.ptr(rep.adv), ops.ptr(self.stats),
                    self.stats.shape[0], float(s.clip_eps), float(s.ent_coef), self.seed & (2**64 - 1), self.ent_step & 0xFFFFFFFF,
                    ((self.rank * self.U + u) * TE * A) & 0xFFFFFFFF, gs, ops.ptr(wa.dout[0]), None if ind else ops.ptr(wa.dout[1]),
                    ops.ptr(wa.loss_partials), ops.ptr(self._g_dscale), nblk, st), "mava_seq_actor_loss_continuous_f32")
                if ind:
                    ops.slab_reduce(self._g_dscale, self.nA, an.log_std(self.g[: self.Pa]), accumulate=acc)
            else:
                ops.check(L.mava_seq_actor_loss_f32(1, Rm, TE, A, self.nA, ops.ptr(idx), ops.ptr(outs[0]), ops.ptr(rep.action_mask[:T]),
                                                    ops.ptr(rep.action), ops.ptr(rep.log_prob), ops.ptr(rep.adv), ops.ptr(self.stats),
                                                    self.stats.shape[0], float(s.clip_eps), float(s.ent_coef), gs, ops.ptr(wa.dout[0]),
                                                    ops.ptr(wa.loss_partials), nblk, st), "mava_seq_actor_loss_f32")
            ops.slab_reduce(wa.loss_partials, 2, self.g[self.P : self.P + 2], accumulate=acc)
            an.net.backward(pa, wa, wa.dout[: len(an.net.heads)], self.g[: self.Pa], accumulate=acc, grad_scale=gs)
        w_actor = parallel.allreduce_sum_async(self.g[: self.Pa])
        for u, rep in enumerate(self.reps):
            acc = u > 0
            cx = (rep.global_state[:T].view(1, TE, -1, self.Oc) if self.centralised else rep.agents_view[:T].view(1, TE, A, self.Oa))
            v = cn.net.forward(pc, wc, cx, self.critic_share, idx, Rm, TE, A)[0]
            ops.check(L.mava_seq_critic_loss_f32(1, Rm, TE, A, 1, ops.ptr(idx), ops.ptr(v), ops.ptr(rep.value), ops.ptr(rep.tgt),
                                                 float(s.clip_eps), float(s.vf_coef), gs, ops.ptr(wc.dout[0]), ops.ptr(wc.loss_partials),
                                                 nblk, st), "mava_seq_critic_loss_f32")
            ops.slab_reduce(wc.loss_partials, 1, self.g[self.P + 2 : self.P + 3], accumulate=acc)
            cn.net.backward(pc, wc, [wc.dout[0]], self.g[self.Pa : self.P], accumulate=acc, grad_scale=gs)
        w_rest = parallel.allreduce_sum_async(self.g[self.Pa :])
        for wk in (w_actor, w_rest):
            if wk is not None:
                wk.wait()
        self._clip_adam(n, k, mb)

    def _permutations(self) -> List[torch.Tensor]:
        if not hasattr(self, "_perm_bufs"):
            self._perm_all = torch.empty((self.K, self.T * self.E), dtype=torch.int32, device=self.device)
            self._perm_bufs = [self._perm_all[k] for k in range(self.K)]
            self._stats_all = torch.empty((self.U, self.K * self.M, self.stats.shape[0], 2), dtype=torch.float64, device=self.device)
        for k0 in range(0, self.K, 16):
            ops.permutation_batched(self.T * self.E, self.seed, self.perm_count + k0, self._perm_all[k0 : k0 + 16])
        self.perm_count += self.K
        return self._perm_bufs

    def update(self, n: int, permutations: Optional[List[torch.Tensor]] = None) -> None:
        own = permutations is None
        if own:
            permutations = self._permutations()
        self.ctx.set(self.ctx.W1_SPLIT_FRESH, 0)
        self._rollout(n)
        self._stats_batched = own and not self.generic and self.T * self.E == self.M * self.Rb
        if self._stats_batched:
            for u, rep in enumerate(self.reps):
                ops.adv_stats_batched(rep.adv.view(-1), self._perm_all.view(-1), self.Rb, self.A, self.K * self.M,
                                      out=self._stats_all[u])
        for k in range(self.K):
            self._epoch(n, k, permutations[k])
        self._carry_observation()

    def _carry_observation(self) -> None:
        for rep in self.reps:
            ops.rollout_carry(rep.agents_view, rep.global_state, rep.action_mask, rep.step_count)


def learner_setup(env, keys, config, centralised_critic: bool, device=None):
    return ppo_learner.learner_setup(FFLearner, env, keys, config, centralised_critic, device=device)


def get_final_step_metrics(metrics: Dict[str, torch.Tensor]) -> Tuple[Dict[str, torch.Tensor], bool]:
    metrics = dict(metrics)
    is_final = metrics.pop("is_terminal_step").bool()
    has_final = bool(is_final.any())
    if not has_final:
        return {k: torch.zeros_like(v) for k, v in metrics.items()}, False
    return {k: v[is_final] for k, v in metrics.items()}, True
```

### mava_amd/ops.py

```python
from __future__ import annotations

import ctypes as C
from typing import Optional, Sequence, Tuple

import torch

from . import _lib
from ._lib import Ctx, check, ctx_ptr, lib, ptr, stream_ptr


def _req(t: torch.Tensor, dtype: torch.dtype, name: str, shape: Optional[Tuple[int, ...]] = None) -> None:
    if not isinstance(t, torch.Tensor):
        raise TypeError(f"{name}: expected a torch.Tensor")
    if not t.is_cuda:
        raise _lib.MavaHipError(f"{name}: tensor must live on the GPU (got {t.device}); there is no CPU path")
    if t.dtype != dtype:
        raise TypeError(f"{name}: expected dtype {dtype}, got {t.dtype}")
    if not t.is_contiguous():
        raise ValueError(f"{name}: tensor must be contiguous")
    if shape is not None and tuple(t.shape) != tuple(shape):
        raise ValueError(f"{name}: expected shape {tuple(shape)}, got {tuple(t.shape)}")


def _as_u8(t: torch.Tensor) -> torch.Tensor:
# ... 375 lines not shown
        raise ValueError("agents_view rows must be a multiple of A")
    TE = rows // A
    _req(params, torch.float32, "params")
    P = mlp_param_count(din, n_actions)
    if params.numel() != P:
        raise ValueError(f"params: expected {P} floats")
    if action_mask is not None:
        action_mask = _as_u8(action_mask)
        _req(action_mask, torch.uint8, "action_mask", (rows, n_actions))
    _req(action, torch.int32, "action")
    _req(old_log_prob, torch.float32, "old_log_prob")
    _req(advantages, torch.float32, "advantages")
    for n, t in (("action", action), ("old_log_prob", old_log_prob), ("advantages", advantages)):
        if t.numel() != rows:
            raise ValueError(f"{n}: expected {rows} elements, got {t.numel()}")
    _req(stats, torch.float64, "stats", (lib().mava_adv_stats_blocks(), 2))
    _check_idx(idx, idx_base, Rb, TE)
    if rows >= 2 ** 31:
        raise ValueError("trajectory too large: TE*A must be < 2^31 (32-bit row arithmetic in the kernel)")
    _req(slab, torch.float32, "slab")
    if slab.dim() != 2 or slab.shape[1] < P + 2:
        raise ValueError("slab must be (n_slab, >= P+2)")
    args = (ctx_ptr(ctx), ptr(params), din, n_actions, ptr(agents_view), ptr(action_mask), ptr(action), ptr(old_log_prob),
            ptr(advantages), ptr(stats), ptr(idx), idx_base, Rb, A, clip_eps, ent_coef, ptr(slab), slab.shape[1], slab.shape[0])
    check(lib().mava_ppo_actor_grad_f32(*args, ptr(input16), ptr(input16_valid), 0 if input16 is None else input16.shape[1],
                                        stream_ptr()), "mava_ppo_actor_grad_f32")


def ppo_critic_grad(params, critic_input, x_share: int, old_value, targets, idx, idx_base: int, Rb: int, A: int,
                    clip_eps: float, vf_coef: float, slab: torch.Tensor, ctx: Optional[Ctx] = None,
                    input16: Optional[torch.Tensor] = None, input16_valid: Optional[torch.Tensor] = None) -> None:
    _req(critic_input, torch.float32, "critic_input")
    din = critic_input.shape[1]
    if (input16 is None) != (input16_valid is None):
        raise ValueError("input16 and input16_valid go together")
    if input16 is not None:
        _req(input16, torch.float16, "input16")
        if tuple(input16.shape) != tuple(critic_input.shape) and not (
                x_share == 1 and input16.dim() == 2 and input16.shape[0] == critic_input.shape[0] and input16.shape[1] > din):
            raise ValueError(f"input16: expected {tuple(critic_input.shape)} (or (rows, RP > din) with x_share == 1), got {tuple(input16.shape)}")
        _req(input16_valid, torch.int32, "input16_valid", (1,))
    _req(params, torch.float32, "params")
    P = mlp_param_count(din, 1)
    if params.numel() != P:
        raise ValueError(f"params: expected {P} floats")
    _req(old_value, torch.float32, "old_value")
    _req(targets, torch.float32, "targets")
    rows = old_value.numel()
    if targets.numel() != rows or rows % A:
        raise ValueError("old_value/targets must hold TE*A elements")
    if (rows + x_share - 1) // x_share > critic_input.shape[0]:
        raise ValueError("critic_input has too few rows")
    _check_idx(idx, idx_base, Rb, rows // A)
    if rows >= 2 ** 31:
        raise ValueError("trajectory too large: TE*A must be < 2^31 (32-bit row arithmetic in the kernel)")
    _req(slab, torch.float32, "slab")
    if slab.dim() != 2 or slab.shape[1] < P + 2:
        raise ValueError("slab must be (n_slab, >= P+2)")
    args = (ctx_ptr(ctx), ptr(params), din, ptr(critic_input), x_share, ptr(old_value), ptr(targets), ptr(idx), idx_base, Rb, A,
            clip_eps, vf_coef, ptr(slab), slab.shape[1], slab.shape[0])
    check(lib().mava_ppo_critic_grad_f32(*args, ptr(input16), ptr(input16_valid), 0 if input16 is None else input16.shape[1],
                                         stream_ptr()), "mava_ppo_critic_grad_f32")


def slab_reduce2(slab: torch.Tensor, n_main: int, out_main: torch.Tensor, n_tail: int, out_tail: torch.Tensor,
                 accumulate: bool = False) -> None:
    _req(slab, torch.float32, "slab")
    _req(out_main, torch.float32, "out_main")
    _req(out_tail, torch.float32, "out_tail")
    if slab.dim() != 2 or slab.shape[1] < n_main + n_tail or out_main.numel() < n_main or out_tail.numel() < n_tail:
        raise ValueError("slab_reduce2: inconsistent sizes")
    check(
        lib().mava_slab_reduce2_f32(ptr(slab), slab.shape[0], slab.shape[1], n_main, ptr(out_main), n_tail, ptr(out_tail),
                                    int(accumulate), stream_ptr()),
        "mava_slab_reduce2_f32",
    )


def rollout_ff(actor_params, critic_params, *, n_actions: int, critic_shared: bool, E: int, A: int, O: int, T: int,
               time_limit: int, policy_seed: int, env_seed: int, t0: int, row_offset: int, env_offset: int,
               reward_mode: int, env_state, agents_view, global_state, action_mask, obs_step_count, action, value,
               reward, log_prob, done, last_val, info_return, info_length, info_terminal, adv=None, tgt=None,
               gamma: float = 0.99, gae_lambda: float = 0.95, last_reward=None, last_done=None, step_counter=None,
               state16=None, state16_valid=None, view16=None, view16_valid=None) -> bool:
    W = A + O
    _req(actor_params, torch.float32, "actor_params")
    _req(critic_params, torch.float32, "critic_params")
    if actor_params.numel() != mlp_param_count(W, n_actions):
        raise ValueError("actor_params: wrong size")
    if critic_params.numel() != mlp_param_count(A * O if critic_shared else W, 1):
        raise ValueError("critic_params: wrong size")
    _req(agents_view, torch.float32, "agents_view", (T + 1, E, A, W))
    if critic_shared:
        _req(global_state, torch.float32, "global_state", (T + 1, E, 1, A * O))
    _req(action_mask, torch.uint8, "action_mask", (T + 1, E, A, n_actions))
    _req(obs_step_count, torch.int32, "obs_step_count", (T + 1, E, A))
    _req(action, torch.int32, "action", (T, E, A))
    for name, t, dt in (("value", value, torch.float32), ("reward", reward, torch.float32),
                        ("log_prob", log_prob, torch.float32), ("done", done, torch.uint8)):
        _req(t, dt, name, (T, E, A))
    _req(last_val, torch.float32, "last_val", (E, A))
    if adv is not None or tgt is not None:
        _req(adv, torch.float32, "adv", (T, E, A))
        _req(tgt, torch.float32, "tgt", (T, E, A))
    _req(info_return, torch.float32, "info_return", (T, E))
    _req(info_length, torch.int32, "info_length", (T, E))
    _req(info_terminal, torch.uint8, "info_terminal", (T, E))
    _req(env_state.step_count, torch.int32, "step_count", (E, A))
    for name, t, dt in (("run_return", env_state.run_return, torch.float32), ("run_length", env_state.run_length, torch.int32),
                        ("ep_return", env_state.ep_return, torch.float32), ("ep_length", env_state.ep_length, torch.int32)):
        _req(t, dt, name, (E,))
    args = (
        ptr(actor_params), n_actions, ptr(critic_params), int(critic_shared), E, A, O, T, time_limit,
        policy_seed & 0xFFFFFFFFFFFFFFFF, env_seed & 0xFFFFFFFFFFFFFFFF, t0 & 0xFFFFFFFF, row_offset & 0xFFFFFFFF,
        env_offset & 0xFFFFFFFF, reward_mode, ptr(env_state.step_count), ptr(env_state.run_return),
        ptr(env_state.run_length), ptr(env_state.ep_return), ptr(env_state.ep_length), ptr(agents_view),
        ptr(global_state) if critic_shared else None, ptr(action_mask), ptr(obs_step_count), ptr(action), ptr(value),
        ptr(reward), ptr(log_prob), ptr(done), ptr(last_val), ptr(info_return), ptr(info_length), ptr(info_terminal),
        ptr(adv), ptr(tgt), gamma, gae_lambda)
    if (state16 is None) != (state16_valid is None):
        raise ValueError("state16 and state16_valid go together")
    if (view16 is None) != (view16_valid is None):
        raise ValueError("view16 and view16_valid go together")
    if state16 is not None:
        if not critic_shared or (A * O) % 8:
            raise ValueError("state16 needs the shared critic and A * O % 8 == 0")
        _req(state16, torch.float16, "state16", (T + 1, E, 1, A * O))
        _req(state16_valid, torch.int32, "state16_valid", (1,))
    if view16 is not None:
        _req(view16, torch.float16, "view16", (T + 1, E, A, 8 * ((W + 8) // 8)))
        _req(view16_valid, torch.int32, "view16_valid", (1,))
    if last_reward is not None or last_done is not None or step_counter is not None:
        _req(last_reward, torch.float32, "last_reward", (E, A))
        _req(last_done, torch.uint8, "last_done", (E, A))
        if step_counter is not None:
            _req(step_counter, torch.int32, "step_counter", (1,))
    rc = lib().mava_rollout_ff_f32(*args, ptr(last_reward), ptr(last_done), ptr(step_counter), ptr(state16), ptr(state16_valid),
                                   ptr(view16), ptr(view16_valid), stream_ptr())
    if rc == 1:
        return False
    check(rc, "mava_rollout_ff_f32")
    return True
```

### mava_amd/ppo_learner.py

```python
from __future__ import annotations

import os
from typing import Any, Dict, List, Optional, Sequence, Tuple

import torch

from . import ops, parallel
from .guards import check_f16_range
from .learner_common import bind_learn, matmul_ctx
from .networks import make_action_head
from .types import AdamState, ExperimentOutput, Observation, ObservationGlobalState, OptStates, Params
from .utils.tree import tree_to

NUM_CU = 256


class _Replica:

    def __init__(self, env, T: int, n_upd: int, device, continuous: bool = False):
        E, A = env.num_envs, env.num_agents
        self.env = env
        self.state = env.alloc_state()
        d = device
        self.agents_view = torch.empty((T + 1, E, A, env.obs_dim), device=d)
        self.global_state = torch.empty((T + 1, E, env.gs_tiles, env.state_dim), device=d)
        self.action_mask = torch.empty((T + 1, E, A, env.action_dim), dtype=torch.uint8, device=d)
        self.step_count = torch.empty((T + 1, E, A), dtype=torch.int32, device=d)
        self.action = (torch.empty((T, E, A, env.action_dim), device=d) if continuous
                       else torch.empty((T, E, A), dtype=torch.int32, device=d))
        self.value = torch.empty((T, E, A), device=d)
        self.reward = torch.empty((T, E, A), device=d)
        self.log_prob = torch.empty((T, E, A), device=d)
        self.done = torch.empty((T, E, A), dtype=torch.uint8, device=d)
        self.last_val = torch.empty((E, A), device=d)
        self.adv = torch.empty((T, E, A), device=d)
        self.tgt = torch.empty((T, E, A), device=d)
        self.info_return = torch.zeros((n_upd, T, E), device=d)
        self.info_length = torch.zeros((n_upd, T, E), dtype=torch.int32, device=d)
        self.info_terminal = torch.zeros((n_upd, T, E), dtype=torch.uint8, device=d)
        self.cur_return = torch.zeros((T, E), device=d)
        self.cur_length = torch.zeros((T, E), dtype=torch.int32, device=d)
        self.cur_terminal = torch.zeros((T, E), dtype=torch.uint8, device=d)
        self.last_reward = torch.zeros((E, A), device=d)
        self.last_done = torch.zeros((E, A), dtype=torch.uint8, device=d)

    def obs_slot(self, t: int) -> Dict[str, torch.Tensor]:
        return {"agents_view": self.agents_view[t], "global_state": self.global_state[t],
                "action_mask": self.action_mask[t], "step_count": self.step_count[t]}


class PPOLearner:
    def __init__(self, env, config, centralised_critic: bool, device: Optional[torch.device] = None, *, replica=_Replica,
                 replica_kwargs: Optional[Dict[str, Any]] = None, ctx_kwargs: Optional[Dict[str, Any]] = None):
        self.config = config
        self.centralised = centralised_critic
        self.rank, self.world = parallel.rank_world()
        s, arch = config.system, config.arch
        self.E, self.U, self.T = int(arch.num_envs), int(s.update_batch_size), int(s.rollout_length)
        self.K, self.M = int(s.ppo_epochs), int(s.num_minibatches)
        self._refuse(env, config)
        self.device = device if device is not None else torch.device("cuda", torch.cuda.current_device())
        self.n_upd = int(s.get("num_updates_per_eval", 1))
        if env.num_envs != self.E:
            raise ValueError(f"env.num_envs={env.num_envs} != arch.num_envs={self.E}")
        if centralised_critic and not getattr(env, "add_global_state", False):
            raise ValueError("Global state must be provided to the centralised critic.")
        self.matmul_mode, self.ctx = matmul_ctx(s, **(ctx_kwargs or {}))
        self.action_head = make_action_head(config.network.get("action_head", None), env.action_dim)
        self.continuous = type(self.action_head).__name__ == "ContinuousActionHead"
        self.min_scale = float(getattr(self.action_head, "min_scale", 1e-3))
        self._env_reads_action = not self.continuous or getattr(env, "continuous_actions", False)
        self.reps: List[Any] = []
        for u in range(self.U):
            rep_env = env.clone(env_offset=getattr(env, "env_offset", 0) + (self.rank * self.U + u) * self.E)
            self.reps.append(replica(rep_env, self.T, self.n_upd, self.device, continuous=self.continuous, **(replica_kwargs or {})))
        env0 = self.reps[0].env
        self.A, self.nA = env0.num_agents, env0.action_dim
        config.system.num_agents = self.A
        self.Oa = env0.obs_dim
        if centralised_critic:
            self.Oc = env0.state_dim
            self.critic_share = self.A if env0.global_state_shared else 1
        else:
            self.Oc, self.critic_share = self.Oa, 1
        self.rccl_cus = int(s.get("rccl_cus", None) if s.get("rccl_cus", None) is not None
                            else os.environ.get("MAVA_RCCL_CUS", "8" if self.world > 1 else "0"))
        d = self.device
        self.stats = torch.zeros((ops.lib().mava_adv_stats_blocks(), 2), dtype=torch.float64, device=d)
        self.train_metrics = torch.zeros((self.n_upd, self.K, self.M, 4), device=d)
        self.perm_rows = self.T * self.E
        self.perm_count = 0
        self.t_global = 0
        self.ent_step = 0
        self.seed = int(s.seed)
        self.timers: Optional[Dict[str, list]] = None
        self._learn_calls = 0

    def _refuse(self, env, config) -> None:
        pass

    def _slab_count(self, ntiles: int) -> int:
        return max(1, min(NUM_CU - max(0, min(self.rccl_cus, NUM_CU - 1)), ntiles))

    def _alloc_params(self, nets: Sequence[Tuple[Any, float]]) -> None:
        self.seg_off = [0]
        for net, _ in nets:
            self.seg_off.append(self.seg_off[-1] + net.num_params)
        self.segments = [(net, slice(lo, hi)) for (net, _), lo, hi in zip(nets, self.seg_off, self.seg_off[1:])]
        self.seg_lr = [float(lr) for _, lr in nets]
        self.P = self.seg_off[-1]
        d = self.device
        self.p, self.m, self.v = (torch.zeros(self.P, device=d) for _ in range(3))
        self.g = torch.zeros(self.P + 4, device=d)
        self.count = torch.zeros(2, dtype=torch.int32, device=d)

    def init_params(self, *seeds: int) -> None:
        for (net, sl), seed in zip(self.segments, seeds):
            self.p[sl].copy_(net.init_flat(seed))
        self.m.zero_()
        self.v.zero_()
        self.count.zero_()

    def reset_envs(self) -> None:
        for rep in self.reps:
            rep.env.step_into(rep.state, 0, rep.obs_slot(0), is_reset=True)
        self.t_global = self.ent_step = self.perm_count = 0

    def _trees(self, flat: torch.Tensor) -> List[Any]:
        return [net.tree(flat[sl], (1, self.U)) for net, sl in self.segments]

    def _adam_states(self) -> List[AdamState]:
        return [AdamState(self.count[i].expand(1, self.U), mu, nu)
                for i, (mu, nu) in enumerate(zip(self._trees(self.m), self._trees(self.v)))]

    def _params_tree(self):
        return Params(*self._trees(self.p))

    def _opt_tree(self):
        return OptStates(*self._adam_states())

    def _state_segments(self, state) -> List[Tuple[Any, AdamState]]:
        return [(state.params.actor_params, state.opt_states.actor_opt_state),
                (state.params.critic_params, state.opt_states.critic_opt_state)]

    def adopt(self, state) -> None:
        trees = self._state_segments(state)
        leaf = self.segments[0][0].first_leaf(trees[0][0])
        if isinstance(leaf, torch.Tensor) and leaf.data_ptr() == self.p.data_ptr():
            return
        to = lambda tree: tree_to(tree, self.p.device)
        for i, ((net, sl), (params, opt)) in enumerate(zip(self.segments, trees)):
            net.flat_from_tree(to(params), self.p[sl])
            net.flat_from_tree(to(opt.mu), self.m[sl])
            net.flat_from_tree(to(opt.nu), self.v[sl])
            self.count[i] = int(torch.as_tensor(opt.count).reshape(-1)[0])
        self._adopted()

    def _adopted(self) -> None:
        pass

    def _stack(self, f) -> torch.Tensor:
        return torch.stack([f(r) for r in self.reps], 0).unsqueeze(0)

    def _observation(self, slot: int = 0):
        av = self._stack(lambda r: r.agents_view[slot])
        mask = self._stack(lambda r: r.action_mask[slot]).bool()
        sc = self._stack(lambda r: r.step_count[slot])
        if not self.centralised:
            return Observation(av, mask, sc)
        gs = self._stack(lambda r: r.global_state[slot].expand(-1, self.A, -1) if r.env.gs_tiles == 1 else r.global_state[slot])
        return ObservationGlobalState(av, mask, gs, sc)

    def _key(self) -> torch.Tensor:
        return torch.tensor([[[self.seed, self.t_global]] * self.U], dtype=torch.int64)

    def _env_state(self) -> Dict[str, torch.Tensor]:
        return {"step_count": self._stack(lambda r: r.state.step_count), "episode_return": self._stack(lambda r: r.state.ep_return),
                "episode_length": self._stack(lambda r: r.state.ep_length)}

    def _adam_kwargs(self, n: int, k: int, mb: int) -> Dict[str, Any]:
        s = self.config.system
        return dict(grad_scale=1.0 / (self.U * self.world), max_norm=float(s.max_grad_norm), decay=bool(s.decay_learning_rates),
                    steps_per_update=self.K * self.M, num_updates=int(s.get("num_updates", 1) or 1), vf_coef=float(s.vf_coef),
                    ent_coef=float(s.ent_coef), metrics_out=self.train_metrics[n, k, mb])

    def _clip_adam(self, n: int, k: int, mb: int) -> None:
        ops.clip_adam(self.p, self.g, self.m, self.v, self.count, self.seg_off, self.seg_lr, loss_sums=self.g[self.P :],
                      **self._adam_kwargs(n, k, mb))

    def _epoch(self, n: int, k: int, perm) -> None:
        for mb in range(self.M):
            self._minibatch(n, k, mb, perm)
            self.ent_step += 1

    def _carry_observation(self) -> None:
        for rep in self.reps:
            for buf in (rep.agents_view, rep.global_state, rep.action_mask, rep.step_count):
                buf[0].copy_(buf[self.T])

    def update(self, n: int, permutations: Optional[List[torch.Tensor]] = None) -> None:
        self._rollout(n)
        self._bootstrap_and_gae()
        for k in range(self.K):
            if permutations is not None:
                perm = permutations[k]
            else:
                perm = ops.permutation(self.perm_rows, self.seed, self.perm_count)
                self.perm_count += 1
            self._epoch(n, k, perm)
        self._carry_observation()

    def _guard_tensors(self) -> Tuple[torch.Tensor, List[Optional[torch.Tensor]]]:
        return self.p, [t for r in self.reps for t in (r.agents_view[0], r.global_state[0] if self.centralised else None)]

    def learn(self, learner_state) -> ExperimentOutput:
        self.adopt(learner_state)
        if self.matmul_mode == "f16x2":
            params, obs = self._guard_tensors()
            check_f16_range(params, obs, self.train_metrics if self._learn_calls else None, type(self).__name__)
        self._learn_calls += 1
        for n in range(self.n_upd):
            self.update(n)
        episode_metrics = {
            "episode_return": torch.stack([r.info_return for r in self.reps], 1).unsqueeze(0),
            "episode_length": torch.stack([r.info_length for r in self.reps], 1).unsqueeze(0),
            "is_terminal_step": torch.stack([r.info_terminal for r in self.reps], 1).unsqueeze(0).bool(),
        }
        tm = self.train_metrics.unsqueeze(1).expand(self.n_upd, self.U, self.K, self.M, 4).unsqueeze(0)
        train_metrics = {"total_loss": tm[..., 0], "value_loss": tm[..., 1], "actor_loss": tm[..., 2], "entropy": tm[..., 3]}
        return ExperimentOutput(self.learner_state(), episode_metrics, train_metrics)


def learner_setup(cls, env, keys, config, *cls_args, device=None):
    key, *net_keys = (int(k) for k in keys)
    learner = cls(env, config, *cls_args, device)
    learner.seed = key
    learner.init_params(*net_keys[: len(learner.segments)])
    parallel.broadcast_(learner.p, src=0)
    learner.reset_envs()
    return bind_learn(learner), learner.actor_network, learner.learner_state()
```

Baseline: 89.05 million env-steps/s.

## Skip f32 observation writes in rollout when training reads f16 copies

Adds a rollout entry point with flags that skip writing the f32 agents_view and/or global_state buffers for intermediate steps. Only the f16 copies are written, and the f32 data is rebuilt on demand through a new expand kernel when something reads it. Query functions ask the train launchers whether they will consume the f16 inputs, so skipping only happens when it is safe. This aims to cut rollout write bandwidth, at the cost of a lazy materialisation path and more complex replica state.

Measured after the change: 90.68 million env-steps/s (median of 6 runs). 1.02x the previous value.

```diff
diff --git a/include/mava_hip.h b/include/mava_hip.h
--- a/include/mava_hip.h
+++ b/include/mava_hip.h
@@ -110,6 +110,11 @@
                              const uint32_t* input16_valid, int input16_ld, mava_stream_t s);
 
 
+int mava_ppo_actor_grad_reads_input16(const mava_ctx* ctx, int din, int n_actions, const float* agents_view, int A,
+                                      const uint16_t* input16, int input16_ld);
+int mava_ppo_critic_grad_reads_input16(const mava_ctx* ctx, int din, const float* critic_input, int x_share, int A,
+                                       const uint16_t* input16, int input16_ld);
+
 int mava_synth_rware_step(int E, int A, int O, int n_actions, int gs_tiles, int state_dim, int time_limit,
                           uint64_t seed, uint32_t t, const uint32_t* t_base, uint32_t env_offset, int is_reset,
                           int32_t* step_count, float* run_return, int32_t* run_length,
@@ -176,6 +181,22 @@
                         uint8_t* info_terminal, float* adv, float* tgt, float gamma, float gae_lambda,
                         float* last_reward, uint8_t* last_done, int32_t* step_counter, uint16_t* state16,
                         uint32_t* state16_valid, uint16_t* view16, uint32_t* view16_valid, mava_stream_t s);
+#define MAVA_ROLLOUT_SKIP_AGENTS_VIEW 1u
+#define MAVA_ROLLOUT_SKIP_GLOBAL_STATE 2u
+int mava_rollout_ff_flags_f32(const float* actor_params, int n_actions, const float* critic_params, int critic_shared,
+                              int E, int A, int O, int T, int time_limit, uint64_t policy_seed, uint64_t env_seed,
+                              uint32_t t0, uint32_t row_offset, uint32_t env_offset, int reward_mode,
+                              int32_t* step_count, float* run_return, int32_t* run_length, float* ep_return,
+                              int32_t* ep_length, float* agents_view, float* global_state, uint8_t* action_mask,
+                              int32_t* obs_step_count, int32_t* action, float* value, float* reward, float* log_prob,
+                              uint8_t* done, float* last_val, float* info_return, int32_t* info_length,
+                              uint8_t* info_terminal, float* adv, float* tgt, float gamma, float gae_lambda,
+                              float* last_reward, uint8_t* last_done, int32_t* step_counter, uint16_t* state16,
+                              uint32_t* state16_valid, uint16_t* view16, uint32_t* view16_valid, uint32_t flags,
+                              mava_stream_t s);
+int mava_rollout_expand_f32(int T, int E, int A, int O, float* agents_view, const uint16_t* view16,
+                            const uint32_t* view16_valid, float* global_state, const uint16_t* state16,
+                            const uint32_t* state16_valid, int force, mava_stream_t s);
 int mava_rollout_carry(int T, int E, int A, int obs_dim, long gs_dim, int n_actions, float* agents_view,
                        float* global_state, uint8_t* action_mask, int32_t* step_count, mava_stream_t s);
 
diff --git a/mava_amd/_lib.py b/mava_amd/_lib.py
--- a/mava_amd/_lib.py
+++ b/mava_amd/_lib.py
@@ -76,6 +76,11 @@
     "mava_sac_alpha_loss_f32": [i32, i32, vp, vp, f32, vp, vp, vp],
     "mava_rollout_ff_f32": [vp, i32, vp, i32, i32, i32, i32, i32, i32, u64, u64, u32, u32, u32, i32] + [vp] * 18
                            + [vp, vp, f32, f32] + [vp] * 7 + [vp],
+    "mava_rollout_ff_flags_f32": [vp, i32, vp, i32, i32, i32, i32, i32, i32, u64, u64, u32, u32, u32, i32] + [vp] * 18
+                                 + [vp, vp, f32, f32] + [vp] * 7 + [u32, vp],
+    "mava_rollout_expand_f32": [i32, i32, i32, i32, vp, vp, vp, vp, vp, vp, i32, vp],
+    "mava_ppo_actor_grad_reads_input16": [vp, i32, i32, vp, i32, vp, i32],
+    "mava_ppo_critic_grad_reads_input16": [vp, i32, vp, i32, i32, vp, i32],
     "mava_rollout_carry": [i32, i32, i32, i32, lng, i32, vp, vp, vp, vp, vp],
     "mava_rec_dense_f32": [vp, vp, i32, vp, i32, i32, i32, i32, i32, i32, vp, i32, vp, vp, vp, i32, i32, i32, i32, i32, vp],
     "mava_rec_xty_f32": [vp, vp, i32, vp, i32, i32, i32, i32, i32, vp, i32, vp, i32, i32, i32, i32, i32, i32, f32, vp, lng, i32, vp],
diff --git a/mava_amd/csrc/ppo_train.hip b/mava_amd/csrc/ppo_train.hip
--- a/mava_amd/csrc/ppo_train.hip
+++ b/mava_amd/csrc/ppo_train.hip
@@ -854,6 +854,39 @@
 int g_train_last_instance = 0;
 extern "C" int mava_debug_train_last_instance(void) { return g_train_last_instance; }
 
+thread_local int* g_x16_query = nullptr;
+
+static TrainTask actor_task(const float* agents_view, int din, int n_actions, int A, const uint16_t* input16,
+                            const uint32_t* input16_valid, int input16_ld) {
+  TrainTask tk = {};
+  tk.x = agents_view; tk.din = din; tk.no = n_actions; tk.xshare = 1; tk.agg = 1;
+  tk.xv = pick_xv(agents_view, din); tk.A = A;
+  tk.x16 = reinterpret_cast<const _Float16*>(input16); tk.x16_valid = input16_valid; tk.x16_ld = input16_ld;
+  return tk;
+}
+static TrainTask critic_task(const mava_ctx* ctx, const float* critic_input, int din, int x_share, int A, const uint16_t* input16,
+                             const uint32_t* input16_valid, int input16_ld) {
+  TrainTask tk = {};
+  tk.x = critic_input; tk.din = din; tk.no = 1; tk.xshare = x_share; tk.agg = 1;
+  if (mava_ctx_critic_aggregation(ctx) && A > 1 && A <= 8 && x_share == A) {
+    tk.agg = A;
+    tk.xshare = 1;
+  }
+  tk.xv = pick_xv(critic_input, din); tk.A = A;
+  tk.x16 = reinterpret_cast<const _Float16*>(input16); tk.x16_valid = input16_valid; tk.x16_ld = input16_ld;
+  return tk;
+}
+static int reads_x16(const mava_ctx* ctx, const TrainTask& tk, bool actor) {
+  int ans = 0;
+  if (mava_ctx_matmul_mode(ctx) == 1) {
+    g_x16_query = &ans;
+    const int rc = mava_train_h2_launch(const_cast<mava_ctx*>(ctx), tk, 1, actor, nullptr);
+    g_x16_query = nullptr;
+    if (rc < 0) return rc;
+  }
+  return ans;
+}
+
 extern "C" int mava_adv_stats_f64(const float* adv, const int32_t* idx, long idx_base, int Rb, int A,
                                   double* partials, hipStream_t s) {
   MAVA_ARG_CHECK(Rb >= 1 && A >= 1, 0, "mava_adv_stats_f64: Rb=%d A=%d", Rb, A);
@@ -891,14 +924,12 @@
                  "mava_ppo_actor_grad_f32: null pointer argument");
   MAVA_ARG_CHECK((input16 == nullptr) == (input16_valid == nullptr) && input16_ld >= 0, 3,
                  "mava_ppo_actor_grad_f32: input16 and input16_valid go together, input16_ld=%d", input16_ld);
-  TrainTask tk = {};
-  tk.params = params; tk.x = agents_view; tk.din = din; tk.no = n_actions; tk.xshare = 1; tk.agg = 1;
-  tk.xv = pick_xv(agents_view, din); tk.A = A; tk.idx = idx; tk.idx_base = idx_base; tk.Rb = Rb;
+  TrainTask tk = actor_task(agents_view, din, n_actions, A, input16, input16_valid, input16_ld);
+  tk.params = params; tk.idx = idx; tk.idx_base = idx_base; tk.Rb = Rb;
   tk.mask = action_mask; tk.action = action; tk.old_logp = old_log_prob; tk.adv = advantages;
   tk.stats = adv_stats; tk.clip_eps = clip_eps; tk.ent_coef = ent_coef; tk.slab = slab;
   tk.slab_stride = slab_stride;
   tk.stamps = g_stamps;
-  tk.x16 = reinterpret_cast<const _Float16*>(input16); tk.x16_valid = input16_valid; tk.x16_ld = input16_ld;
   if (mava_ctx_matmul_mode(ctx) == 1) {
     const int rc = mava_train_h2_launch(ctx, tk, n_slab, true, s);
     if (rc <= 0) return rc;
@@ -951,20 +982,32 @@
                  "mava_ppo_critic_grad_f32: null pointer argument");
   MAVA_ARG_CHECK((input16 == nullptr) == (input16_valid == nullptr) && input16_ld >= 0, 3,
                  "mava_ppo_critic_grad_f32: input16 and input16_valid go together, input16_ld=%d", input16_ld);
-  TrainTask tk = {};
-  tk.params = params; tk.x = critic_input; tk.din = din; tk.no = 1; tk.xshare = x_share; tk.agg = 1;
-  if (mava_ctx_critic_aggregation(ctx) && A > 1 && A <= 8 && x_share == A) {
-    tk.agg = A;
-    tk.xshare = 1;
-  }
-  tk.xv = pick_xv(critic_input, din); tk.A = A; tk.idx = idx; tk.idx_base = idx_base; tk.Rb = Rb;
+  TrainTask tk = critic_task(ctx, critic_input, din, x_share, A, input16, input16_valid, input16_ld);
+  tk.params = params; tk.idx = idx; tk.idx_base = idx_base; tk.Rb = Rb;
   tk.old_value = old_value; tk.targets = targets; tk.clip_eps = clip_eps; tk.vf_coef = vf_coef;
   tk.slab = slab; tk.slab_stride = slab_stride;
   tk.stamps = g_stamps;
-  tk.x16 = reinterpret_cast<const _Float16*>(input16); tk.x16_valid = input16_valid; tk.x16_ld = input16_ld;
   int rc = 1;
   if (mava_ctx_matmul_mode(ctx) == 1) rc = mava_train_h2_launch(ctx, tk, n_slab, false, s);
   if (ctx != nullptr) ctx->w1_fresh[1] = 0;
   if (rc <= 0) return rc;
   return dispatch_kt<1, false>(tk, n_slab, s);
 }
+
+extern "C" int mava_ppo_actor_grad_reads_input16(const mava_ctx* ctx, int din, int n_actions, const float* agents_view, int A,
+                                                 const uint16_t* input16, int input16_ld) {
+  MAVA_ARG_CHECK(din >= 1 && n_actions >= 1 && n_actions <= 32 && A >= 1 && input16_ld >= 0, 0,
+                 "mava_ppo_actor_grad_reads_input16: din=%d n_actions=%d A=%d input16_ld=%d", din, n_actions, A, input16_ld);
+  if (input16 == nullptr) return 0;
+  static const uint32_t word = 0;
+  return reads_x16(ctx, actor_task(agents_view, din, n_actions, A, input16, &word, input16_ld), true);
+}
+
+extern "C" int mava_ppo_critic_grad_reads_input16(const mava_ctx* ctx, int din, const float* critic_input, int x_share, int A,
+                                                  const uint16_t* input16, int input16_ld) {
+  MAVA_ARG_CHECK(din >= 1 && x_share >= 1 && A >= 1 && input16_ld >= 0, 0,
+                 "mava_ppo_critic_grad_reads_input16: din=%d x_share=%d A=%d input16_ld=%d", din, x_share, A, input16_ld);
+  if (input16 == nullptr) return 0;
+  static const uint32_t word = 0;
+  return reads_x16(ctx, critic_task(ctx, critic_input, din, x_share, A, input16, &word, input16_ld), false);
+}
diff --git a/mava_amd/csrc/ppo_train_h2.hip b/mava_amd/csrc/ppo_train_h2.hip
--- a/mava_amd/csrc/ppo_train_h2.hip
+++ b/mava_amd/csrc/ppo_train_h2.hip
@@ -1110,6 +1110,12 @@
 
 template <int NO, int S1, bool ACTOR, bool WIDE, int XV>
 int launch_h2(mava_ctx* ctx, const TrainTask& tk, int n_slab, hipStream_t s) {
+  const bool x16_ok = WIDE && !ACTOR && XV == 4 && tk.x16 != nullptr && tk.x16_valid != nullptr && tk.din % 8 == 0 &&
+                      (uintptr_t)tk.x16 % 16 == 0 && tk.force_xlo == 0 && (tk.x16_ld == 0 || tk.x16_ld == tk.din);
+  if (g_x16_query != nullptr) {
+    *g_x16_query = x16_ok ? 1 : 0;
+    return MAVA_OK;
+  }
   const H2Layout L = make_h2_layout<NO, S1, WIDE>(ACTOR);
   MAVA_ARG_CHECK(L.end <= 163840, 8, "ppo_train_h2: %d bytes of LDS exceed the 160 KiB of a CU", L.end);
   static bool attr_set = false;
@@ -1137,8 +1143,6 @@
   }
   TrainTask tkl = tk;
   tkl.exact_tiles = WIDE ? ctx->exact_tiles : nullptr;
-  const bool x16_ok = WIDE && !ACTOR && XV == 4 && tk.x16 != nullptr && tk.x16_valid != nullptr && tk.din % 8 == 0 &&
-                      (uintptr_t)tk.x16 % 16 == 0 && tk.force_xlo == 0 && (tk.x16_ld == 0 || tk.x16_ld == tk.din);
   if (!x16_ok) { tkl.x16 = nullptr; tkl.x16_valid = nullptr; }
   tkl.x16_launches = x16_ok ? ctx->exact_tiles + 1 : nullptr;
   g_train_last_instance = train_instance_id(2, ACTOR, false, WIDE, NO, S1, XV);
@@ -1199,7 +1203,7 @@
   tk.no_defer = (ctx->train_variant & 4) != 0;
   tk.no_ahead = (ctx->train_variant & 8) != 0;
   if ((ctx->train_variant & 1) == 0) {
-    if (tk.x16 != nullptr && tk.x16_valid != nullptr) {
+    if (tk.x16 != nullptr && tk.x16_valid != nullptr && g_x16_query == nullptr) {
       const int rcc = ctx_counters(ctx, s);
       if (rcc != MAVA_OK) return rcc;
       tk.x16_launches = ctx->exact_tiles + 2;
@@ -1208,11 +1212,11 @@
     }
     const int rc8 = mava_train_w8_launch(tk, n_slab, actor, s);
     if (rc8 <= 0) {
-      if (rc8 == 0) { ++ctx->h2_launches; ++ctx->w8_launches; }
+      if (rc8 == 0 && g_x16_query == nullptr) { ++ctx->h2_launches; ++ctx->w8_launches; }
       return rc8;
     }
   }
   const int rc = h2_dispatch(ctx, tk, n_slab, actor, s);
-  if (rc == 0) ++ctx->h2_launches;
+  if (rc == 0 && g_x16_query == nullptr) ++ctx->h2_launches;
   return rc;
 }
diff --git a/mava_amd/csrc/ppo_train_task.h b/mava_amd/csrc/ppo_train_task.h
--- a/mava_amd/csrc/ppo_train_task.h
+++ b/mava_amd/csrc/ppo_train_task.h
@@ -42,6 +42,8 @@
 int mava_train_w8_launch(const TrainTask& tk, int n_slab, bool actor, hipStream_t s);
 int mava_train_h2_launch(mava_ctx* ctx, const TrainTask& tk, int n_slab, bool actor, hipStream_t s);
 
+extern thread_local int* g_x16_query;
+
 extern int g_train_last_instance;
 constexpr int train_instance_id(int family, bool actor, bool cont, bool wide, int no, int k, int xv) {
   return family * 1000000 + ((actor ? 1 : 0) + (cont ? 2 : 0) + (wide ? 4 : 0)) * 100000 + no * 1000 + k * 10 + xv;
diff --git a/mava_amd/csrc/ppo_train_w8.hip b/mava_amd/csrc/ppo_train_w8.hip
--- a/mava_amd/csrc/ppo_train_w8.hip
+++ b/mava_amd/csrc/ppo_train_w8.hip
@@ -850,6 +850,13 @@
 
 template <int NO, int S1, int XV, bool ACTOR>
 int launch_w8(const TrainTask& tk, int n_slab, hipStream_t s) {
+  const int ld16 = tk.x16_ld != 0 ? tk.x16_ld : tk.din;
+  const bool x16_ok = XV == 2 && tk.x16 != nullptr && tk.x16_valid != nullptr && ld16 % 8 == 0 && ld16 >= tk.din &&
+                      (uintptr_t)tk.x16 % 16 == 0 && tk.force_xlo == 0 && tk.xshare == 1 && tk.agg <= 1;
+  if (g_x16_query != nullptr) {
+    *g_x16_query = x16_ok ? 1 : 0;
+    return MAVA_OK;
+  }
   const W8Layout L = make_w8_layout();
   MAVA_ARG_CHECK(L.end <= 163840, 8, "ppo_train_w8: %d bytes of LDS exceed the 160 KiB of a CU", L.end);
   static bool attr_set = false;
@@ -859,9 +866,6 @@
     attr_set = true;
   }
   TrainTask tkl = tk;
-  const int ld16 = tk.x16_ld != 0 ? tk.x16_ld : tk.din;
-  const bool x16_ok = XV == 2 && tk.x16 != nullptr && tk.x16_valid != nullptr && ld16 % 8 == 0 && ld16 >= tk.din &&
-                      (uintptr_t)tk.x16 % 16 == 0 && tk.force_xlo == 0 && tk.xshare == 1 && tk.agg <= 1;
   tkl.x16_ld = ld16;
   if (!x16_ok) { tkl.x16 = nullptr; tkl.x16_valid = nullptr; tkl.x16_launches = nullptr; tkl.defer_launches = nullptr; tkl.ahead_launches = nullptr; }
   g_train_last_instance = train_instance_id(3, ACTOR, false, false, NO, S1, XV);
diff --git a/mava_amd/csrc/rollout_h2.hip b/mava_amd/csrc/rollout_h2.hip
--- a/mava_amd/csrc/rollout_h2.hip
+++ b/mava_amd/csrc/rollout_h2.hip
@@ -47,7 +47,10 @@
   _Float16* state16; uint32_t* state16_valid;
   _Float16* view16; uint32_t* view16_valid;
   int v16_nc; uint32_t v16_nc_m;
+  uint32_t flags;
+  int s16_nc; uint32_t s16_nc_m;
 };
+constexpr uint32_t SKIP_VIEW = 1u, SKIP_STATE = 2u;
 
 #define MAVA_AS4 __attribute__((address_space(4)))
 __device__ __forceinline__ const MAVA_AS4 RolloutArgs& args_here() {
@@ -426,11 +429,18 @@
   const int tid_w = tid, wo_q = (W >> 1) > 0 ? (W >> 1) : 1, gs_q = (AO >> 2) > 0 ? (AO >> 2) : 1;
   const int wo_dr = 256 / wo_q, gs_dr = 256 / gs_q;
   const uint32_t wo_m = 65536u / (uint32_t)wo_q + 1u, gs_m = 65536u / (uint32_t)gs_q + 1u;
-  auto write_gs = [&](long slot, bool f32_too) {
+  auto write_gs = [&](long slot, bool f32_too, bool lean) {
     const auto& a = args_here();
     int tid = tid_w;
     asm volatile("" : "+v"(tid));
-    if (SHARED && a.global_state != nullptr) {
+    if (SHARED && lean) {
+      const int NC = a.s16_nc;
+      uint4* const dst16 = reinterpret_cast<uint4*>(a.state16 + (slot * E + e0) * (long)AO);
+      for (int j = tid; j < envs_ok * NC; j += 256) {
+        const int le = (int)div_small((uint32_t)j, a.s16_nc_m), c = j - le * NC;
+        dst16[j] = *reinterpret_cast<const uint4*>(lds + L.xc + le * xc_row + 16 * c);
+      }
+    } else if (SHARED && a.global_state != nullptr) {
       float* dst = a.global_state + (slot * E + e0) * (long)AO;
       if ((AO & 3) == 0) {
         const bool h16 = a.state16 != nullptr;
@@ -472,11 +482,12 @@
       }
     }
   };
-  auto write_out = [&](long slot, bool part_gs) {
+  auto write_out = [&](long slot, bool part_gs, bool last) {
     const auto& a = args_here();
+    const uint32_t skip = last ? 0u : a.flags;
     int tid = tid_w;
     asm volatile("" : "+v"(tid));
-    if (!part_gs) {
+    if (!part_gs && (skip & SKIP_VIEW) == 0) {
       float* dst = a.agents_view + (slot * EA + (long)e0 * A) * W;
       if ((W & 1) == 0) {
         const int W2 = W >> 1, d_r = wo_dr, d_f = 256 - d_r * W2;
@@ -504,7 +515,8 @@
       }
     }
     if (!part_gs) write_view16(slot);
-    if (part_gs) write_gs(slot, true);
+    if (part_gs && (skip & SKIP_STATE) == 0) write_gs(slot, true, false);
+    if (!part_gs && (skip & SKIP_STATE) != 0) write_gs(slot, true, true);
     if (!part_gs) {
       uint8_t* dst = a.action_mask + (slot * EA + (long)e0 * A) * no;
       for (int j = tid; j < rows_ok * no; j += 256) {
@@ -516,7 +528,7 @@
 
   const int T_steps = a.T;
   const uint32_t t0 = a.t0;
-  if (SHARED && ACT_ROLE && a.state16 != nullptr) write_gs(0L, false);
+  if (SHARED && ACT_ROLE && a.state16 != nullptr) write_gs(0L, false, false);
   if (!ACT_ROLE) write_view16(0L);
   for (int t = 0; t < T_steps; ++t) {
     const uint32_t step = t0 + (uint32_t)t;
@@ -564,9 +576,9 @@
       if (tid < 64 && (e0 + (tid >> lgA)) < E) {
         a.value[(long)t * EA + (long)e0 * A + tid] = value_of(SHARED ? (tid >> lgA) : tid);
       }
-      if (t > 0) write_out((long)t, false);
-    }
-    if (ACT_ROLE && t > 0) write_out((long)t, true);
+      if (t > 0) write_out((long)t, false, false);
+    }
+    if (ACT_ROLE && t > 0) write_out((long)t, true, false);
     RSTAMP(4);
     __syncthreads();
     RSTAMP(5);
@@ -676,7 +688,7 @@
   if (blockIdx.x == 0 && tid == 0)
     for (int i = 0; i < 8; ++i) g_rollout_stamps[(ACT_ROLE ? 0 : 8) + i] = rs_acc[i];
 #endif
-  write_out((long)T_steps, ACT_ROLE);
+  write_out((long)T_steps, ACT_ROLE, true);
   forward(!ACT_ROLE, false, 0u);
   {
   const auto& a = args_here();
@@ -790,16 +802,17 @@
 
 extern "C" int mava_debug_rollout_last_instance(void) { return g_rollout_last_instance; }
 
-extern "C" int mava_rollout_ff_f32(const float* actor_params, int n_actions, const float* critic_params, int critic_shared,
-                                   int E, int A, int O, int T, int time_limit, uint64_t policy_seed, uint64_t env_seed,
-                                   uint32_t t0, uint32_t row_offset, uint32_t env_offset, int reward_mode,
-                                   int32_t* step_count, float* run_return, int32_t* run_length, float* ep_return,
-                                   int32_t* ep_length, float* agents_view, float* global_state, uint8_t* action_mask,
-                                   int32_t* obs_step_count, int32_t* action, float* value, float* reward, float* log_prob,
-                                   uint8_t* done, float* last_val, float* info_return, int32_t* info_length,
-                                   uint8_t* info_terminal, float* adv, float* tgt, float gamma, float gae_lambda,
-                                   float* last_reward, uint8_t* last_done, int32_t* step_counter, uint16_t* state16,
-                                   uint32_t* state16_valid, uint16_t* view16, uint32_t* view16_valid, hipStream_t s) {
+extern "C" int mava_rollout_ff_flags_f32(const float* actor_params, int n_actions, const float* critic_params, int critic_shared,
+                                         int E, int A, int O, int T, int time_limit, uint64_t policy_seed, uint64_t env_seed,
+                                         uint32_t t0, uint32_t row_offset, uint32_t env_offset, int reward_mode,
+                                         int32_t* step_count, float* run_return, int32_t* run_length, float* ep_return,
+                                         int32_t* ep_length, float* agents_view, float* global_state, uint8_t* action_mask,
+                                         int32_t* obs_step_count, int32_t* action, float* value, float* reward, float* log_prob,
+                                         uint8_t* done, float* last_val, float* info_return, int32_t* info_length,
+                                         uint8_t* info_terminal, float* adv, float* tgt, float gamma, float gae_lambda,
+                                         float* last_reward, uint8_t* last_done, int32_t* step_counter, uint16_t* state16,
+                                         uint32_t* state16_valid, uint16_t* view16, uint32_t* view16_valid, uint32_t flags,
+                                         hipStream_t s) {
   MAVA_ARG_CHECK(E >= 1 && A >= 1 && O >= 2 && T >= 1 && n_actions >= 1 && time_limit >= 1, 0,
                  "mava_rollout_ff_f32: bad shape E=%d A=%d O=%d T=%d nA=%d", E, A, O, T, n_actions);
   MAVA_ARG_CHECK(actor_params && critic_params && step_count && run_return && run_length && ep_return && ep_length &&
@@ -832,6 +845,15 @@
   MAVA_ARG_CHECK(view16 == nullptr || (uintptr_t)view16 % 16 == 0, 2, "mava_rollout_ff_f32: view16 needs 16-byte alignment");
   a.view16 = reinterpret_cast<_Float16*>(view16); a.view16_valid = view16_valid;
   a.v16_nc = (A + O + 8) / 8; a.v16_nc_m = 65536u / (uint32_t)a.v16_nc + 1u;
+  MAVA_ARG_CHECK((flags & ~(SKIP_VIEW | SKIP_STATE)) == 0, 3, "mava_rollout_ff_flags_f32: unknown flags 0x%x", flags);
+  MAVA_ARG_CHECK((flags & SKIP_VIEW) == 0 || (view16 != nullptr && view16_valid != nullptr), 3,
+                 "mava_rollout_ff_flags_f32: MAVA_ROLLOUT_SKIP_AGENTS_VIEW needs view16 and view16_valid");
+  MAVA_ARG_CHECK((flags & SKIP_STATE) == 0 || (state16 != nullptr && state16_valid != nullptr), 3,
+                 "mava_rollout_ff_flags_f32: MAVA_ROLLOUT_SKIP_GLOBAL_STATE needs state16 and state16_valid");
+  a.flags = flags;
+  a.s16_nc = state16 != nullptr ? A * O / 8 : 1; a.s16_nc_m = 65536u / (uint32_t)a.s16_nc + 1u;
+  MAVA_ARG_CHECK((flags & SKIP_STATE) == 0 || (64 / A) * a.s16_nc * a.s16_nc < 65536, 3,
+                 "mava_rollout_ff_flags_f32: A*O=%d too wide for MAVA_ROLLOUT_SKIP_GLOBAL_STATE", A * O);
   if (critic_shared) {
     if (s1a == 5 && s1c == 17 && A >= 4) return launch_rollout<8, 5, 17, true>(a, s);
 #ifndef MAVA_FAST_BUILD
@@ -846,6 +868,107 @@
   if (s1a <= 2) return launch_rollout<8, 2, 2, false>(a, s);
 #endif
   return 1;
+}
+
+extern "C" int mava_rollout_ff_f32(const float* actor_params, int n_actions, const float* critic_params, int critic_shared,
+                                   int E, int A, int O, int T, int time_limit, uint64_t policy_seed, uint64_t env_seed,
+                                   uint32_t t0, uint32_t row_offset, uint32_t env_offset, int reward_mode,
+                                   int32_t* step_count, float* run_return, int32_t* run_length, float* ep_return,
+                                   int32_t* ep_length, float* agents_view, float* global_state, uint8_t* action_mask,
+                                   int32_t* obs_step_count, int32_t* action, float* value, float* reward, float* log_prob,
+                                   uint8_t* done, float* last_val, float* info_return, int32_t* info_length,
+                                   uint8_t* info_terminal, float* adv, float* tgt, float gamma, float gae_lambda,
+                                   float* last_reward, uint8_t* last_done, int32_t* step_counter, uint16_t* state16,
+                                   uint32_t* state16_valid, uint16_t* view16, uint32_t* view16_valid, hipStream_t s) {
+  return mava_rollout_ff_flags_f32(actor_params, n_actions, critic_params, critic_shared, E, A, O, T, time_limit, policy_seed, env_seed, t0, row_offset, env_offset, reward_mode, step_count, run_return, run_length, ep_return, ep_length, agents_view, global_state, action_mask, obs_step_count, action, value, reward, log_prob, done, last_val, info_return, info_length, info_terminal, adv, tgt, gamma, gae_lambda, last_reward, last_done, step_counter, state16, state16_valid, view16, view16_valid, 0u, s);
+}
+
+namespace {
+struct ExpandArgs {
+  const _Float16* src[2];
+  float* dst[2];
+  const uint32_t* word[2];
+  long rows[2];
+  int ld[2], w[2];
+  int force;
+};
+constexpr int EXPAND_ROWS = 64;
+constexpr int EXPAND_LD_MAX = 288;
+__global__ __launch_bounds__(256) void rollout_expand_kernel(ExpandArgs x) {
+  __shared__ __attribute__((aligned(16))) _Float16 tile[EXPAND_ROWS * EXPAND_LD_MAX];
+  const int k = blockIdx.y;
+  if (x.src[k] == nullptr) return;
+  if (x.force == 0 && __builtin_amdgcn_readfirstlane((int)*x.word[k]) == 1) return;
+  const int ld = x.ld[k], w = x.w[k], nc = ld >> 3;
+  const long rows = x.rows[k], tiles = (rows + EXPAND_ROWS - 1) / EXPAND_ROWS;
+  const bool wide = (reinterpret_cast<uintptr_t>(x.dst[k]) & 15) == 0;
+  for (long tl = blockIdx.x; tl < tiles; tl += gridDim.x) {
+    const long row0 = tl * EXPAND_ROWS;
+    const int nr = (int)(rows - row0 < EXPAND_ROWS ? rows - row0 : EXPAND_ROWS);
+    const uint4* const src = reinterpret_cast<const uint4*>(x.src[k] + row0 * ld);
+    for (int j = threadIdx.x; j < nr * nc; j += 256) reinterpret_cast<uint4*>(tile)[j] = src[j];
+    __syncthreads();
+    float* const dst = x.dst[k] + row0 * w;
+    const int n = nr * w;
+    if (wide) {
+      for (int q = threadIdx.x; 4 * q < n; q += 256) {
+        int r = (4 * q) / w, c = 4 * q - r * w;
+        float v[4];
+#pragma unroll
+        for (int i = 0; i < 4; ++i) {
+          v[i] = (4 * q + i < n) ? (float)tile[r * ld + c] : 0.0f;
+          if (++c == w) { c = 0; ++r; }
+        }
+        if (4 * q + 4 <= n) {
+          reinterpret_cast<float4*>(dst)[q] = make_float4(v[0], v[1], v[2], v[3]);
+        } else {
+          for (int i = 0; 4 * q + i < n; ++i) dst[4 * q + i] = v[i];
+        }
+      }
+    } else {
+      for (int e = threadIdx.x; e < n; e += 256) {
+        const int r = e / w, c = e - r * w;
+        dst[e] = (float)tile[r * ld + c];
+      }
+    }
+    __syncthreads();
+  }
+}
+}
+
+extern "C" int mava_rollout_expand_f32(int T, int E, int A, int O, float* agents_view, const uint16_t* view16,
+                                       const uint32_t* view16_valid, float* global_state, const uint16_t* state16,
+                                       const uint32_t* state16_valid, int force, hipStream_t s) {
+  MAVA_ARG_CHECK(T >= 1 && E >= 1 && A >= 1 && O >= 1, 0, "mava_rollout_expand_f32: bad shape T=%d E=%d A=%d O=%d", T, E, A, O);
+  MAVA_ARG_CHECK((agents_view == nullptr) == (view16 == nullptr) && (view16 == nullptr) == (view16_valid == nullptr), 1,
+                 "mava_rollout_expand_f32: agents_view, view16 and view16_valid go together");
+  MAVA_ARG_CHECK((global_state == nullptr) == (state16 == nullptr) && (state16 == nullptr) == (state16_valid == nullptr), 1,
+                 "mava_rollout_expand_f32: global_state, state16 and state16_valid go together");
+  MAVA_ARG_CHECK(view16 != nullptr || state16 != nullptr, 1, "mava_rollout_expand_f32: no record given");
+  MAVA_ARG_CHECK(((uintptr_t)view16 | (uintptr_t)state16) % 16 == 0, 2, "mava_rollout_expand_f32: the records need 16-byte alignment");
+  const int W = A + O, RP = 8 * ((W + 8) / 8), AO = A * O;
+  MAVA_ARG_CHECK(state16 == nullptr || AO % 8 == 0, 2, "mava_rollout_expand_f32: state16 needs A*O %% 8 == 0 (A*O=%d)", AO);
+  MAVA_ARG_CHECK((view16 == nullptr || RP <= EXPAND_LD_MAX) && (state16 == nullptr || AO <= EXPAND_LD_MAX), 2,
+                 "mava_rollout_expand_f32: record rows of more than %d halves are not supported", EXPAND_LD_MAX);
+  if (T < 2) return MAVA_OK;
+  ExpandArgs x = {};
+  x.force = force ? 1 : 0;
+  long most = 0;
+  if (view16 != nullptr) {
+    const long EA = (long)E * A;
+    x.src[0] = reinterpret_cast<const _Float16*>(view16) + EA * RP; x.dst[0] = agents_view + EA * W; x.word[0] = view16_valid;
+    x.rows[0] = (long)(T - 1) * EA; x.ld[0] = RP; x.w[0] = W;
+    most = x.rows[0];
+  }
+  if (state16 != nullptr) {
+    x.src[1] = reinterpret_cast<const _Float16*>(state16) + (long)E * AO; x.dst[1] = global_state + (long)E * AO; x.word[1] = state16_valid;
+    x.rows[1] = (long)(T - 1) * E; x.ld[1] = AO; x.w[1] = AO;
+    most = x.rows[1] > most ? x.rows[1] : most;
+  }
+  const long tiles = mava_cdiv(most, (long)EXPAND_ROWS);
+  hipLaunchKernelGGL(rollout_expand_kernel, dim3((unsigned)(tiles > 2048 ? 2048 : tiles), 2), dim3(256), 0, s, x);
+  MAVA_LAUNCH_CHECK();
+  return MAVA_OK;
 }
 
 namespace {
diff --git a/mava_amd/learner.py b/mava_amd/learner.py
--- a/mava_amd/learner.py
+++ b/mava_amd/learner.py
@@ -9,13 +9,13 @@
 
 from . import ops, parallel, ppo_learner
 from .networks import FeedForwardActor, FeedForwardValueNet, MLPTorso
-from .ppo_learner import PPOLearner
+from .ppo_learner import LeanReplica, PPOLearner
 from .types import LearnerState, TimeStep
 
 
 class FFLearner(PPOLearner):
     def __init__(self, env, config, centralised_critic: bool, device: Optional[torch.device] = None):
-        super().__init__(env, config, centralised_critic, device,
+        super().__init__(env, config, centralised_critic, device, replica=LeanReplica,
                          ctx_kwargs={"critic_aggregation": os.environ.get("MAVA_CRITIC_AGGREGATION", "1") != "0"})
         s, env0, action_head = config.system, self.reps[0].env, self.action_head
 
@@ -69,6 +69,7 @@
         for rep in self.reps:
             rep.view16 = torch.zeros((self.T + 1, self.E, self.A, rp), dtype=torch.float16, device=d) if self.view16 else None
             rep.view16_valid = torch.zeros((1,), dtype=torch.int32, device=d) if self.view16 else None
+        self.lean = os.environ.get("MAVA_ROLLOUT_LEAN", "1") != "0"
         self.fused_tail = (self.world == 1 and not self.generic and os.environ.get("MAVA_FUSED_TAIL", "1") != "0")
         self._finish_ws = ops.ppo_finish_workspace(self.Pa, self.Pc, d) if self.fused_tail else None
         self._finish_ws_mr = (ops.ppo_finish_workspace(self.Pa, self.Pc, d)
@@ -162,19 +163,26 @@
                 st.wait_stream(main)
         for u, rep in enumerate(self.reps):
             env = rep.env
+            skip_av, skip_gs = self._reads_records(rep) if self.lean else (False, False)
             with (torch.cuda.stream(self._roll_streams[u - 1]) if (side and u > 0) else contextlib.nullcontext()):
               ok = self._timed(
                 "rollout_fused", ops.rollout_ff, pa, pc, n_actions=self.nA, critic_shared=self.centralised, E=self.E,
                 A=self.A, O=env.raw_obs_dim, T=self.T, time_limit=env.time_limit, policy_seed=self.seed,
                 env_seed=env.seed, t0=self.t_global, row_offset=(self.rank * self.U + u) * EA, env_offset=env.env_offset,
-                reward_mode=1 if env.reward_mode == "match" else 0, env_state=rep.state, agents_view=rep.agents_view,
-                global_state=rep.global_state, action_mask=rep.action_mask, obs_step_count=rep.step_count,
+                reward_mode=1 if env.reward_mode == "match" else 0, env_state=rep.state, agents_view=rep.av_raw,
+                global_state=rep.gs_raw, action_mask=rep.action_mask, obs_step_count=rep.step_count,
                 action=rep.action, value=rep.value, reward=rep.reward, log_prob=rep.log_prob, done=rep.done,
                 last_val=rep.last_val, info_return=rep.info_return[n], info_length=rep.info_length[n],
                 info_terminal=rep.info_terminal[n], adv=rep.adv, tgt=rep.tgt, gamma=float(s.gamma),
                 gae_lambda=float(s.gae_lambda), last_reward=rep.last_reward, last_done=rep.last_done,
                 step_counter=self.step_dev if u == 0 else None,
-                state16=rep.state16, state16_valid=rep.state16_valid, view16=rep.view16, view16_valid=rep.view16_valid)
+                state16=rep.state16, state16_valid=rep.state16_valid, view16=rep.view16, view16_valid=rep.view16_valid,
+                skip_agents_view=skip_av, skip_global_state=skip_gs)
+              if ok and (skip_av or skip_gs):
+                self._timed("rollout_expand", ops.rollout_expand, rep.av_raw if skip_av else None, rep.view16 if skip_av else None,
+                            rep.view16_valid if skip_av else None, rep.gs_raw if skip_gs else None, rep.state16 if skip_gs else None,
+                            rep.state16_valid if skip_gs else None, force=False)
+                rep.stale_av, rep.stale_gs = rep.stale_av or skip_av, rep.stale_gs or skip_gs
               if not ok:
                 assert u == 0
                 self.fused_rollout = self.x16 = self.view16 = False
@@ -185,6 +193,24 @@
             for st in self._roll_streams:
                 main.wait_stream(st)
         return True
+
+    def _reads_records(self, rep) -> Tuple[bool, bool]:
+        T, TEA = self.T, self.T * self.E * self.A
+        av = rep.av_raw[:T].view(TEA, self.Oa)
+        v16 = rep.view16[:T].view(TEA, -1) if self.view16 else None
+        reads_av = v16 is not None and ops.ppo_actor_grad_reads_input16(self.ctx, av, self.nA, self.A, v16)
+        reads_gs = False
+        if self.centralised:
+            reads_gs = self.x16 and ops.ppo_critic_grad_reads_input16(
+                self.ctx, rep.gs_raw[:T].view(-1, self.Oc), self.critic_share, self.A, rep.state16[:T].view(-1, self.Oc))
+        elif reads_av:
+            reads_av = self.critic_share == 1 and ops.ppo_critic_grad_reads_input16(self.ctx, av, 1, self.A, v16)
+        return bool(reads_av), bool(reads_gs)
+
+    def _lean_guard(self, rep) -> None:
+        if rep.stale_av or rep.stale_gs:
+            now = self._reads_records(rep)
+            rep.materialise(av=not now[0], gs=not now[1])
 
     def _rollout_body(self) -> None:
         pa, pc = self.p[: self.Pa], self.p[self.Pa :]
@@ -250,7 +276,8 @@
         per_rep = self.fused_tail and self.U > 1
         for u, rep in enumerate(self.reps):
             slab_a = self.slab_a[u * ns : (u + 1) * ns] if per_rep else self.slab_a
-            av = rep.agents_view[:T].view(TEA, self.Oa)
+            self._lean_guard(rep)
+            av = rep.av_raw[:T].view(TEA, self.Oa)
             if getattr(self, "_stats_batched", False) and perm is self._perm_bufs[k]:
                 stats = self._stats_all[u, k * self.M + mb]
             else:
@@ -270,8 +297,8 @@
                 ops.slab_reduce2(self.slab_a, self.Pa, self.g[: self.Pa], 2, self.g[self.P : self.P + 2], accumulate=u > 0)
         w_actor = parallel.allreduce_sum_async(self.g[: self.Pa])
         for u, rep in enumerate(self.reps):
-            av = rep.agents_view[:T].view(TEA, self.Oa)
-            cx = rep.global_state[:T].view(-1, self.Oc) if self.centralised else av
+            av = rep.av_raw[:T].view(TEA, self.Oa)
+            cx = rep.gs_raw[:T].view(-1, self.Oc) if self.centralised else av
             in16 = in16_valid = None
             if self.x16:
                 in16, in16_valid = rep.state16[:T].view(-1, self.Oc), rep.state16_valid
@@ -406,7 +433,7 @@
 
     def _carry_observation(self) -> None:
         for rep in self.reps:
-            ops.rollout_carry(rep.agents_view, rep.global_state, rep.action_mask, rep.step_count)
+            ops.rollout_carry(rep.av_raw, rep.gs_raw, rep.action_mask, rep.step_count)
 
 
 def learner_setup(env, keys, config, centralised_critic: bool, device=None):
diff --git a/mava_amd/ops.py b/mava_amd/ops.py
--- a/mava_amd/ops.py
+++ b/mava_amd/ops.py
@@ -481,7 +481,8 @@
                reward_mode: int, env_state, agents_view, global_state, action_mask, obs_step_count, action, value,
                reward, log_prob, done, last_val, info_return, info_length, info_terminal, adv=None, tgt=None,
                gamma: float = 0.99, gae_lambda: float = 0.95, last_reward=None, last_done=None, step_counter=None,
-               state16=None, state16_valid=None, view16=None, view16_valid=None) -> bool:
+               state16=None, state16_valid=None, view16=None, view16_valid=None, skip_agents_view: bool = False,
+               skip_global_state: bool = False) -> bool:
     W = A + O
     _req(actor_params, torch.float32, "actor_params")
     _req(critic_params, torch.float32, "critic_params")
@@ -534,9 +535,56 @@
         _req(last_done, torch.uint8, "last_done", (E, A))
         if step_counter is not None:
             _req(step_counter, torch.int32, "step_counter", (1,))
-    rc = lib().mava_rollout_ff_f32(*args, ptr(last_reward), ptr(last_done), ptr(step_counter), ptr(state16), ptr(state16_valid),
-                                   ptr(view16), ptr(view16_valid), stream_ptr())
+    flags = (ROLLOUT_SKIP_AGENTS_VIEW if skip_agents_view else 0) | (ROLLOUT_SKIP_GLOBAL_STATE if skip_global_state else 0)
+    rc = lib().mava_rollout_ff_flags_f32(*args, ptr(last_reward), ptr(last_done), ptr(step_counter), ptr(state16),
+                                         ptr(state16_valid), ptr(view16), ptr(view16_valid), flags, stream_ptr())
     if rc == 1:
         return False
-    check(rc, "mava_rollout_ff_f32")
+    check(rc, "mava_rollout_ff_flags_f32")
     return True
+
+
+ROLLOUT_SKIP_AGENTS_VIEW, ROLLOUT_SKIP_GLOBAL_STATE = 1, 2
+
+
+def rollout_expand(agents_view, view16, view16_valid, global_state, state16, state16_valid, *, force: bool) -> None:
+    if (agents_view is None) != (view16 is None) or (view16 is None) != (view16_valid is None):
+        raise ValueError("agents_view, view16 and view16_valid go together")
+    if (global_state is None) != (state16 is None) or (state16 is None) != (state16_valid is None):
+        raise ValueError("global_state, state16 and state16_valid go together")
+    if view16 is None and state16 is None:
+        raise ValueError("rollout_expand: no record given")
+    if view16 is not None:
+        _req(agents_view, torch.float32, "agents_view")
+        T1, E, A, W = agents_view.shape
+        O = W - A
+        _req(view16, torch.float16, "view16", (T1, E, A, 8 * ((W + 8) // 8)))
+        _req(view16_valid, torch.int32, "view16_valid", (1,))
+    if state16 is not None:
+        _req(global_state, torch.float32, "global_state")
+        if view16 is None:
+            T1, E, AO = global_state.shape[0], global_state.shape[1], global_state.shape[-1]
+            A, O = 1, AO
+        _req(global_state, torch.float32, "global_state", (T1, E, 1, A * O))
+        _req(state16, torch.float16, "state16", (T1, E, 1, A * O))
+        _req(state16_valid, torch.int32, "state16_valid", (1,))
+    check(lib().mava_rollout_expand_f32(T1 - 1, E, A, O, ptr(agents_view), ptr(view16), ptr(view16_valid), ptr(global_state),
+                                        ptr(state16), ptr(state16_valid), int(bool(force)), stream_ptr()), "mava_rollout_expand_f32")
+
+
+def ppo_actor_grad_reads_input16(ctx: Optional[Ctx], agents_view: torch.Tensor, n_actions: int, A: int,
+                                 input16: Optional[torch.Tensor]) -> bool:
+    rc = lib().mava_ppo_actor_grad_reads_input16(ctx_ptr(ctx), agents_view.shape[1], n_actions, ptr(agents_view), A, ptr(input16),
+                                                 0 if input16 is None else input16.shape[1])
+    if rc < 0:
+        check(rc, "mava_ppo_actor_grad_reads_input16")
+    return rc == 1
+
+
+def ppo_critic_grad_reads_input16(ctx: Optional[Ctx], critic_input: torch.Tensor, x_share: int, A: int,
+                                  input16: Optional[torch.Tensor]) -> bool:
+    rc = lib().mava_ppo_critic_grad_reads_input16(ctx_ptr(ctx), critic_input.shape[1], ptr(critic_input), x_share, A, ptr(input16),
+                                                  0 if input16 is None else input16.shape[1])
+    if rc < 0:
+        check(rc, "mava_ppo_critic_grad_reads_input16")
+    return rc == 1
diff --git a/mava_amd/ppo_learner.py b/mava_amd/ppo_learner.py
--- a/mava_amd/ppo_learner.py
+++ b/mava_amd/ppo_learner.py
@@ -47,6 +47,50 @@
     def obs_slot(self, t: int) -> Dict[str, torch.Tensor]:
         return {"agents_view": self.agents_view[t], "global_state": self.global_state[t],
                 "action_mask": self.action_mask[t], "step_count": self.step_count[t]}
+
+    @property
+    def av_raw(self) -> torch.Tensor:
+        return self.agents_view
+
+    @property
+    def gs_raw(self) -> torch.Tensor:
+        return self.global_state
+
+
+class LeanReplica(_Replica):
+
+    def __init__(self, *args, **kwargs):
+        self.stale_av = self.stale_gs = False
+        self.state16 = self.state16_valid = self.view16 = self.view16_valid = None
+        super().__init__(*args, **kwargs)
+
+    def materialise(self, av: bool = True, gs: bool = True) -> None:
+        av, gs = av and self.stale_av, gs and self.stale_gs
+        if av or gs:
+            ops.rollout_expand(self.av_raw if av else None, self.view16 if av else None, self.view16_valid if av else None,
+                               self.gs_raw if gs else None, self.state16 if gs else None, self.state16_valid if gs else None,
+                               force=True)
+            self.stale_av, self.stale_gs = self.stale_av and not av, self.stale_gs and not gs
+
+    av_raw = gs_raw = None
+
+    @property
+    def agents_view(self) -> torch.Tensor:
+        self.materialise(gs=False)
+        return self.av_raw
+
+    @agents_view.setter
+    def agents_view(self, t: torch.Tensor) -> None:
+        self.av_raw = t
+
+    @property
+    def global_state(self) -> torch.Tensor:
+        self.materialise(av=False)
+        return self.gs_raw
+
+    @global_state.setter
+    def global_state(self, t: torch.Tensor) -> None:
+        self.gs_raw = t
 
 
 class PPOLearner:
@@ -163,12 +207,12 @@
         return torch.stack([f(r) for r in self.reps], 0).unsqueeze(0)
 
     def _observation(self, slot: int = 0):
-        av = self._stack(lambda r: r.agents_view[slot])
+        av = self._stack(lambda r: r.av_raw[slot])
         mask = self._stack(lambda r: r.action_mask[slot]).bool()
         sc = self._stack(lambda r: r.step_count[slot])
         if not self.centralised:
             return Observation(av, mask, sc)
-        gs = self._stack(lambda r: r.global_state[slot].expand(-1, self.A, -1) if r.env.gs_tiles == 1 else r.global_state[slot])
+        gs = self._stack(lambda r: r.gs_raw[slot].expand(-1, self.A, -1) if r.env.gs_tiles == 1 else r.gs_raw[slot])
         return ObservationGlobalState(av, mask, gs, sc)
 
     def _key(self) -> torch.Tensor:
@@ -211,7 +255,7 @@
         self._carry_observation()
 
     def _guard_tensors(self) -> Tuple[torch.Tensor, List[Optional[torch.Tensor]]]:
-        return self.p, [t for r in self.reps for t in (r.agents_view[0], r.global_state[0] if self.centralised else None)]
+        return self.p, [t for r in self.reps for t in (r.av_raw[0], r.gs_raw[0] if self.centralised else None)]
 
     def learn(self, learner_state) -> ExperimentOutput:
         self.adopt(learner_state)
```
